# SenseBrain/JPD-SE

Hardware: AMD Instinct MI355X
Metric: training images/sec at 1024x512 (G+D+VGG step) (higher is better)
Workload: dtype bf16; 1 GPU; JPD-SE train step 1024x512, netG=global ngf=64 (39-ch input), num_D=2, VGG19+feat+L1, Adam x2, batch 4/GPU; global_batch=4, parallelism=dp1

## Files before the change

include/jpdse.h:

```cpp
#ifndef JPDSE_H_
#define JPDSE_H_

#include <stddef.h>
#include <stdint.h>

#ifdef __cplusplus
extern "C" {
#endif

#define JPDSE_ABI_VERSION 2

enum { JPDSE_F32 = 0, JPDSE_BF16 = 1 };
enum { JPDSE_PAD_ZERO = 0, JPDSE_PAD_REFLECT = 1 };
enum { JPDSE_ACT_NONE = 0, JPDSE_ACT_RELU = 1, JPDSE_ACT_LRELU = 2, JPDSE_ACT_TANH = 3 };
enum {
  JPDSE_OK = 0,
  JPDSE_EINVAL = -1,
  JPDSE_EWORKSPACE = -2,
  JPDSE_ELAUNCH = -3,
  JPDSE_EARCH = -4
};

#define JPDSE_CPAD(c) (((c) + 7) & ~7)

// ... 9 lines not shown
#define JPDSE_HBM_ADAM 2
int jpdse_prof_hbm_select(int32_t enable, int32_t max_regions);
int jpdse_prof_hbm_collect(int32_t cls, double* total_ms, double* total_bytes, int64_t* regions);

typedef struct jpdse_conv_desc {
  int32_t dtype;
  int32_t N, H, W, C;
  int32_t K;
  int32_t R, S;
  int32_t stride;
  int32_t pad;
  int32_t pad_mode;
  int32_t act;
  float slope;
} jpdse_conv_desc;

int jpdse_conv_out_shape(const jpdse_conv_desc* d, int32_t* OH, int32_t* OW);
int jpdse_conv_plan_query(const jpdse_conv_desc* d, int32_t* out, int32_t n);
size_t jpdse_conv_fwd_pack_size(const jpdse_conv_desc* d);
size_t jpdse_conv_dgrad_pack_size(const jpdse_conv_desc* d);
int jpdse_conv_pack_weights(const jpdse_conv_desc* d, const float* w_krsc, void* fwd_pack,
                            void* dgrad_pack, void* stream);
typedef struct jpdse_pack_entry {
  const float* w;
  void* out;
  int32_t K, Ks, C, Cs, R, S, st, qh, qw, Uh, Uw, Lk, gx, gy;
  int32_t out_f32;
  int32_t reserved_;
  int64_t blocks;
  int64_t block0;
} jpdse_pack_entry;
int jpdse_conv_pack_entries(const jpdse_conv_desc* d, const float* w_krsc, void* dgrad_pack,
                            jpdse_pack_entry* out, int32_t max_entries);
int jpdse_conv_pack_run(const jpdse_pack_entry* table_dev, int32_t n_entries, int64_t total_blocks,
                        void* stream);
size_t jpdse_conv_workspace_size(const jpdse_conv_desc* d);
int jpdse_conv_fwd(const jpdse_conv_desc* d, const void* x, const void* fwd_pack,
                   const float* bias, void* y, void* ws, size_t ws_bytes, void* stream);
int32_t jpdse_conv_moment_slots(const jpdse_conv_desc* d);
int jpdse_conv_fwd_moments(const jpdse_conv_desc* d, const void* x, const void* fwd_pack, void* y, float* moments,
                           void* ws, size_t ws_bytes, void* stream);
int jpdse_conv_fwd_pool(const jpdse_conv_desc* d, const void* x, const void* fwd_pack, const float* bias,
                        void* y, void* y_pool, void* ws, size_t ws_bytes, void* stream);
int jpdse_conv_dgrad(const jpdse_conv_desc* d, const void* dy, const void* dgrad_pack, void* dx,
                     void* ws, size_t ws_bytes, void* stream);
int jpdse_conv_dgrad_relu(const jpdse_conv_desc* d, const void* dy, const void* dgrad_pack,
                          const void* x, void* dx, void* ws, size_t ws_bytes, void* stream);
int jpdse_conv_dgrad_fused(const jpdse_conv_desc* d, const void* dy, const void* dgrad_pack,
                           const void* x, const void* addend, void* dx, void* ws, size_t ws_bytes,
                           void* stream);
int jpdse_conv_dgrad_fused_lrelu(const jpdse_conv_desc* d, const void* dy, const void* dgrad_pack,
                                 const void* x, float slope, const void* addend, void* dx, void* ws,
                                 size_t ws_bytes, void* stream);
int32_t jpdse_conv_dgrad_nsum_slots(const jpdse_conv_desc* d);
int jpdse_conv_dgrad_fused_nsums(const jpdse_conv_desc* d, const void* dy, const void* dgrad_pack, const void* x,
                                 const void* addend, void* dx, const void* norm_x, const float* norm_stats,
                                 int32_t norm_act, float norm_slope, float* sums, void* ws, size_t ws_bytes, void* stream);
int jpdse_conv_wgrad(const jpdse_conv_desc* d, const void* x, const void* dy, float* dw_krsc,
                     void* ws, size_t ws_bytes, void* stream);

int jpdse_convT_fwd(const jpdse_conv_desc* d, const void* x, const void* dgrad_pack, void* y,
                    void* ws, size_t ws_bytes, void* stream);
int32_t jpdse_convT_moment_slots(const jpdse_conv_desc* d);
int jpdse_convT_fwd_moments(const jpdse_conv_desc* d, const void* x, const void* dgrad_pack, void* y, float* moments,
                            void* ws, size_t ws_bytes, void* stream);
int jpdse_convT_dgrad(const jpdse_conv_desc* d, const void* dy, const void* fwd_pack, void* dx,
                      void* ws, size_t ws_bytes, void* stream);
int jpdse_convT_wgrad(const jpdse_conv_desc* d, const void* x, const void* dy, float* dw,
                      void* ws, size_t ws_bytes, void* stream);

typedef struct jpdse_inorm_desc {
  int32_t dtype;
  int32_t N, H, W, C;
  int32_t act;
  float slope;
  float eps;
  int32_t has_residual;
} jpdse_inorm_desc;
size_t jpdse_inorm_workspace_size(const jpdse_inorm_desc* d);
int jpdse_inorm_fwd(const jpdse_inorm_desc* d, const void* x, const void* residual, void* y,
                    float* stats, void* ws, size_t ws_bytes, void* stream);
int jpdse_inorm_fwd_from_moments(const jpdse_inorm_desc* d, const void* x, const float* moments, int32_t slots,
                                 const void* residual, void* y, float* stats, void* stream);
int jpdse_inorm_bwd_from_sums(const jpdse_inorm_desc* d, const void* x, const float* stats, const void* dy,
                              const float* sums, int32_t slots, void* dx, void* ws, size_t ws_bytes, void* stream);
int jpdse_inorm_bwd(const jpdse_inorm_desc* d, const void* x, const float* stats, const void* dy,
                    void* dx, void* ws, size_t ws_bytes, void* stream);

int jpdse_avgpool3s2_fwd(int32_t dtype, int32_t N, int32_t H, int32_t W, int32_t C, const void* x,
                         void* y, void* stream);
int jpdse_avgpool3s2_bwd(int32_t dtype, int32_t N, int32_t H, int32_t W, int32_t C, const void* dy,
                         void* dx, void* stream);
int jpdse_maxpool2_fwd(int32_t dtype, int32_t N, int32_t H, int32_t W, int32_t C, const void* x,
                       void* y, void* stream);
int jpdse_maxpool2_bwd(int32_t dtype, int32_t N, int32_t H, int32_t W, int32_t C, const void* x,
                       const void* dy, void* dx, void* stream);

int jpdse_act_bwd(int32_t dtype, int64_t n, int32_t act, float slope, const void* y, const void* dy,
                  void* dz, void* stream);
int jpdse_add(int32_t dtype, int64_t n, const void* a, const void* b, void* out, void* stream);
size_t jpdse_channel_sum_workspace_size(int64_t npix, int32_t C);
int jpdse_channel_sum(int32_t dtype, int64_t npix, int32_t C, const void* dy, float* out, void* ws,
                      size_t ws_bytes, void* stream);
int jpdse_channel_copy(int32_t dtype, int64_t npix, const void* src, int32_t src_cs, int32_t src_c0,
                       void* dst, int32_t dst_cs, int32_t dst_c0, int32_t nch, void* stream);
int jpdse_concat_channels(int32_t dtype, int64_t npix, const void* base, int32_t cs, const void* img,
                          int32_t img_cs, int32_t c0, int32_t nch, void* out, void* stream);
int jpdse_copy(int64_t nbytes, const void* src, void* dst, void* stream);
int jpdse_zero(int32_t dtype, int64_t n, void* p, void* stream);
int jpdse_cast(int32_t src_dtype, int32_t dst_dtype, int64_t n, const void* src, void* dst, void* stream);

int jpdse_nchw_to_nhwc(int32_t dtype, int32_t N, int32_t C, int32_t H, int32_t W, const float* src,
                       void* dst, void* stream);
int jpdse_nhwc_to_nchw(int32_t dtype, int32_t N, int32_t C, int32_t H, int32_t W, const void* src,
                       float* dst, void* stream);
int jpdse_onehot_edge(int32_t dtype, int32_t N, int32_t H, int32_t W, int32_t num_labels,
                      const float* label, const int64_t* instance, void* dst, int32_t cs,
                      void* stream);

int jpdse_input_builder(int32_t dtype, int32_t N, int32_t H, int32_t W, int32_t num_labels, const float* label,
                        const int64_t* instance, int32_t n_dst, void* const* dst, const void* const* img, int32_t cs,
                        int32_t img_cs, int32_t c0, int32_t nch, void* stream);
int jpdse_input_builder_wide(int32_t dtype, int32_t N, int32_t H, int32_t W, int32_t num_labels, const float* label,
                             const int64_t* instance, int32_t n_dst, void* const* dst, const void* const* img, int32_t cs,
                             int32_t img_cs, int32_t c0, int32_t nch, void*  stream);
int jpdse_insert_channels(int32_t dtype, int64_t npix, void* dst, int32_t cs, const void* img, int32_t img_cs, int32_t c0,
                          int32_t nch, void* stream);

size_t jpdse_loss_workspace_size(int64_t n);
typedef struct jpdse_loss_term {
// ... 426 lines not shown
```

jpd-se_amd/csrc/conv_dispatch_dgrad.h:

```cpp
#pragma once

namespace jpdse {

struct RingFoldArgs {
  bf16_t* dx;
  const float* top; const float* bot; const float* left; const float* right;
  int splits_tb, splits_lr;
  int N, H, W, Cs;
};
__device__ __forceinline__ void ring_acc(float (&acc)[8], const float* slab, int splits, long long slab_elems,
                                         long long row, int Cs, int c0) {
  const float* base = slab + row * Cs + c0;
  int sp = 0;
  for (; sp + 4 <= splits; sp += 4) {
    float4 lo[4], hi[4];
#pragma unroll
    for (int u = 0; u < 4; ++u) {
      const float4* src = reinterpret_cast<const float4*>(base + (sp + u) * slab_elems);
      lo[u] = src[0];
      hi[u] = src[1];
    }
#pragma unroll
    for (int u = 0; u < 4; ++u) {
      acc[0] += lo[u].x; acc[1] += lo[u].y; acc[2] += lo[u].z; acc[3] += lo[u].w;
// ... 80 lines not shown
    cols[1] = left ? 2 : W - 1;
    nc = 2;
  }
  float acc[8];
#pragma unroll
  for (int i = 0; i < 8; ++i) acc[i] = 0.f;
  for (int r = 0; r < nr; ++r)
    for (int c = 0; c < nc; ++c) {
      float v[8];
      Vec16<bf16_t>::load(dy + (((long long)n * H + rows[r]) * W + cols[c]) * Cs + c0, v);
#pragma unroll
      for (int i = 0; i < 8; ++i) acc[i] += v[i];
    }
  Vec16<bf16_t>::store(V + ((long long)n * per_n + e) * Cs + c0, acc);
}

template <typename T>
__global__ void relu_mask_kernel(T* __restrict__ dx, const T* __restrict__ mask, long long total_vec,
                                 const T* __restrict__ addend = nullptr, float slope = 0.f) {
  constexpr int VE = Vec16<T>::N;
  for (long long i = blockIdx.x * (long long)blockDim.x + threadIdx.x; i < total_vec;
       i += (long long)gridDim.x * blockDim.x) {
    float v[VE], m[VE];
    Vec16<T>::load(dx + i * VE, v);
    if (addend != nullptr) {
      Vec16<T>::load(addend + i * VE, m);
#pragma unroll
      for (int e = 0; e < VE; ++e) v[e] += m[e];
    }
    if (mask != nullptr) {
      Vec16<T>::load(mask + i * VE, m);
#pragma unroll
      for (int e = 0; e < VE; ++e) {
        const float r = sizeof(T) == 2 ? bf16_round(v[e]) : v[e];
        v[e] = m[e] > 0.f ? v[e] : (slope == 0.f ? 0.f : r * slope);
      }
    }
    Vec16<T>::store(dx + i * VE, v);
  }
}

struct NormSink {
  const void* x;
  const float* stats;
  float* sums;
  int act;
  float slope;
};

struct DgradCall {
  const jpdse_conv_desc* d; const ConvPlan& p;
  const void* dy; const void* pack; void* dx; void* ws; hipStream_t s;
  const void* mask; const void* addend; float* mom; float mask_slope; const NormSink* sink;
};
static void* dgrad_dxp(const DgradCall& c) { return reinterpret_cast<char*>(c.ws) + c.p.dypad_bytes; }

static ConvView dgrad_view(const DgradCall& c) {
  ConvView v = view_dgrad_phase(c.d, c.p, 0, c.dy, c.pack, c.dx);
  v.mask = reinterpret_cast<const bf16_t*>(c.mask);
  v.addend = reinterpret_cast<const bf16_t*>(c.addend);
  return v;
}
static ConvView ring_view(const DgradCall& c) {
  ConvView r = dgrad_view(c);
  r.OH = c.d->H;
  r.OW = c.d->W;
  r.py = r.px = 1;
  r.out_base = 0;
  r.mask = nullptr;
  return r;
}

static int dgrad_ring_frame(const DgradCall& c, DgradRoute route) {
  const jpdse_conv_desc* d = c.d;
  const ConvPlan& p = c.p;
  const bool taps = route == DgradRoute::ring_taps9_frame;
  ConvView r = ring_view(c);
  bf16_t* frame = reinterpret_cast<bf16_t*>(c.ws);
  const long long fv = (long long)d->N * (2 * (d->W + 2) + 2 * d->H) * (p.Ks / 8);
  if (taps && (size_t)fv * 16 > p.splitk_off) return set_error(JPDSE_EWORKSPACE, "reflect data gradient: no room for the frame in front of the slabs");
  const int pslot = taps ? -1 : prof_begin(c.s, p.Cs, 9LL * p.Ks);
  hipLaunchKernelGGL(ring_frame_kernel, dim3(ew_blocks(fv)), dim3(256), 0, c.s, r.X, frame, d->N, d->H, d->W, p.Ks, fv);
  const int rc = check_launch("ring_frame_kernel");
  prof_end(pslot, 1, 0.0, c.s);
  if (rc) return rc;
  r.frame = frame;
  r.mask = reinterpret_cast<const bf16_t*>(c.mask);
  if (taps) return launch_taps9(r, splitk_slabs(p, c.ws), c.s);
  HaloArgs h = to_halo(r);
  if (c.sink != nullptr) {
    h.nx = reinterpret_cast<const bf16_t*>(c.sink->x);
    h.nstats = c.sink->stats;
    h.nsums = c.sink->sums;
    h.nact = c.sink->act;
    h.nslope = c.sink->slope;
    h.mom_slots = halo_slots(d->H, d->W);
  }
  return p.Cs > 64 ? launch_halo_cfg<2>(h, c.s) : launch_halo_cfg<1>(h, c.s);
}

static int dgrad_ring_strips(const DgradCall& c, DgradRoute route) {
  const jpdse_conv_desc* d = c.d;
  const ConvPlan& p = c.p;
  hipStream_t s = c.s;
  const ConvView r = ring_view(c);
  if (route == DgradRoute::ring_taps9_strips) {
    if (int rc = launch_taps9(r, splitk_slabs(p, c.ws), s)) return rc;
  } else if (int rc = p.Cs > 64 ? launch_halo_cfg<2>(to_halo(r), s) : launch_halo_cfg<1>(to_halo(r), s)) return rc;
  const int H = d->H, W = d->W, Ks = p.Ks, Lk = p.ph[0].Lk;
  const bf16_t* dyb = reinterpret_cast<const bf16_t*>(c.dy);
  const bf16_t* pk = reinterpret_cast<const bf16_t*>(c.pack);
  const int Mtb = d->N * (W + 2), Mlr = d->N * H;
  const int nt = (p.Cs + 127) / 128;
// ... 73 lines not shown
  h.Wp = reinterpret_cast<const bf16_t*>(c.pack);
  h.Y = reinterpret_cast<bf16_t*>(c.dx);
  h.N = d->N; h.H = p.OH; h.W = p.OW; h.OH = d->H; h.OW = d->W;
  h.K = d->C; h.Ks_out = p.Cs;
  h.R = h.S = 3;
  h.pad = 1;
  h.act = JPDSE_ACT_NONE;
  h.tiles_w = (d->W + 63) / 64;
  h.tiles_h = (d->H + kHeadTH - 1) / kHeadTH;
  if (head_rows_ok(64, h.R, h.K, h.Ks_out, h.H, h.W, h.OH, h.OW)) return launch_head_rows<3>(h, c.s);
  return launch_head_fwd<64, 3, 3, 3>(h, c.s);
}

template <typename Args>
static Args phases_rows_args(const DgradCall& c) {
  Args g = {};
  g.DY = reinterpret_cast<const bf16_t*>(c.dy);
  for (int i = 0; i < 4; ++i) g.P[i] = reinterpret_cast<const bf16_t*>(reinterpret_cast<const char*>(c.pack) + c.p.ph[i].pack_off);
  g.DX = reinterpret_cast<bf16_t*>(c.dx);
  g.N = c.d->N; g.OH = c.p.OH; g.OW = c.p.OW;
  return g;
}
static int dgrad_dgrad2_rows(const DgradCall& c) {
  Dgrad2Args g = phases_rows_args<Dgrad2Args>(c);
  g.mom = c.mom;
  return launch_dgrad2_rows(g, c.s);
}
static int dgrad_thin_dgrad2_rows(const DgradCall& c) {
  ThinDgrad2Args g = phases_rows_args<ThinDgrad2Args>(c);
  g.H = c.d->H; g.W = c.d->W; g.K = c.d->C;
  return launch_thin_dgrad2_rows(g, c.s);
}

static int dgrad_thin_in_rows(const DgradCall& c) {
  ThinInArgs g = {};
  g.DY = reinterpret_cast<const bf16_t*>(c.dy);
  g.P = reinterpret_cast<const bf16_t*>(reinterpret_cast<const char*>(c.pack) + c.p.ph[0].pack_off);
  g.DX = reinterpret_cast<bf16_t*>(c.dx);
  g.DXP = reinterpret_cast<bf16_t*>(dgrad_dxp(c));
  g.N = c.d->N; g.H = c.d->H; g.W = c.d->W; g.OH = c.d->H + 6; g.OW = c.d->W + 6;
  g.py = g.px = 6;
  g.act = JPDSE_ACT_NONE;
  return launch_thin_in_rows<7, true>(g, c.s);
}

static int dgrad_thin1(const DgradCall& c) {
  const Phase& f = c.p.ph[0];
  Thin1DgradArgs t = {};
  t.DY = reinterpret_cast<const bf16_t*>(c.dy);
  t.B = reinterpret_cast<const bf16_t*>(reinterpret_cast<const char*>(c.pack) + f.pack_off);
  t.taps = reinterpret_cast<float*>(c.ws);
  t.DX = reinterpret_cast<bf16_t*>(c.dx);
  t.addend = reinterpret_cast<const bf16_t*>(c.addend);
  t.N = c.d->N; t.H = c.d->H; t.W = c.d->W; t.Cs = c.p.Cs; t.OH = c.p.OH; t.OW = c.p.OW;
  t.py = (f.Uh - 1) - f.i0h;
  t.px = (f.Uw - 1) - f.i0w;
  t.Lk = f.Lk;
  t.b_stride = (long long)f.Uh * f.Lk;
  return launch_thin1_dgrad(t, c.s);
}

template <typename Args>
static void phase_out(Args* a, const DgradCall& c, const Phase& f) {
  const jpdse_conv_desc* d = c.d;
  const ConvPlan& p = c.p;
  const bool refl = d->pad_mode == JPDSE_PAD_REFLECT;
  const int st = d->stride, H = refl ? p.Hp : d->H, W = refl ? p.Wp : d->W, off = refl ? 0 : d->pad;
  a->Y = reinterpret_cast<decltype(a->Y)>(refl ? dgrad_dxp(c) : c.dx);
  a->out_sn = (long long)H * W * p.Cs;
  a->out_sh = (long long)st * W * p.Cs;
  a->out_sw = (long long)st * p.Cs;
  a->out_base = ((long long)(st * f.i0h + f.qh - off) * W + (st * f.i0w + f.qw - off)) * p.Cs;
}
template <typename T>
static int dgrad_finish(const DgradCall& c, bool in_epilogue) {
  const jpdse_conv_desc* d = c.d;
  const long long total_vec = (long long)d->N * d->H * d->W * (c.p.Cs / (16 / (int)sizeof(T)));
  int rc = JPDSE_OK;
  if (d->pad_mode == JPDSE_PAD_REFLECT) {
    hipLaunchKernelGGL((reflect_fold_kernel<T>), dim3(ew_blocks(total_vec)), dim3(256), 0, c.s, reinterpret_cast<const T*>(dgrad_dxp(c)),
                       reinterpret_cast<T*>(c.dx), d->N, d->H, d->W, c.p.Cs, d->pad, total_vec);
    rc = check_launch("reflect_fold_kernel");
  }
  if (rc == JPDSE_OK && (c.mask != nullptr || c.addend != nullptr) && !in_epilogue) {
    hipLaunchKernelGGL((relu_mask_kernel<T>), dim3(ew_blocks(total_vec)), dim3(256), 0, c.s, reinterpret_cast<T*>(c.dx),
                       reinterpret_cast<const T*>(c.mask), total_vec, reinterpret_cast<const T*>(c.addend), c.mask_slope);
    rc = check_launch("relu_mask_kernel");
  }
  return rc;
}

static int dgrad_fast(const DgradCall& c) {
  const jpdse_conv_desc* d = c.d;
  const ConvPlan& p = c.p;
  const bool refl = d->pad_mode == JPDSE_PAD_REFLECT;
  const int nlive = live_phases(p);
  FastBatch batch = {};
  for (int i = 0; i < p.nph; ++i) {
    const Phase& f = p.ph[i];
    if (f.cnth <= 0 || f.cntw <= 0) continue;
    FastArgs g = to_fast(view_dgrad_phase(d, p, i, c.dy, c.pack, c.dx));
    phase_out(&g, c, f);
    if (!refl) {
      g.mask = reinterpret_cast<const bf16_t*>(c.mask);
      g.addend = reinterpret_cast<const bf16_t*>(c.addend);
    }
    g.mask_slope = c.mask_slope;
    g.splits = nlive == 1 ? splitk_for(g.M, p.Cs, f.Uh * f.Uw * p.Ks / 64) : 1;
    g.partial = splitk_slabs(p, c.ws);
    batch.p[batch.n++] = g;
  }
  if (int rc = launch_fast_batch(batch, c.s)) return rc;
  return dgrad_finish<bf16_t>(c, !refl);
}

template <typename T>
static int dgrad_generic(const DgradCall& c) {
  const jpdse_conv_desc* d = c.d;
  const ConvPlan& p = c.p;
  if (int rc = launch_pad<T>(c.dy, c.ws, d->N, p.OH, p.OW, p.Ks, p.PT, p.PB, p.PL, p.PR, JPDSE_PAD_ZERO, c.s)) return rc;
  for (int i = 0; i < p.nph; ++i) {
    const Phase& f = p.ph[i];
    if (f.cnth <= 0 || f.cntw <= 0) continue;
    GemmFwdArgs a = {};
    a.A = c.ws;
    a.B = reinterpret_cast<const char*>(c.pack) + f.pack_off;
    a.M = d->N * f.cnth * f.cntw; a.OH = f.cnth; a.OW = f.cntw;
    a.Kout = d->C; a.Ks = a.b_rows = p.Cs;
    a.R = f.Uh; a.cpr = f.Lk / p.BKE; a.b_row_stride = (long long)f.Uh * f.Lk;
    a.in_sn = (long long)p.DH * p.DW * p.Ks; a.in_sh = a.in_sr = (long long)p.DW * p.Ks; a.in_sw = p.Ks;
    a.in_base = ((long long)(f.i0h + p.PT - (f.Uh - 1)) * p.DW + (f.i0w + p.PL - (f.Uw - 1))) * p.Ks;
    phase_out(&a, c, f);
    a.act = JPDSE_ACT_NONE;
    a.partial = splitk_slabs(p, c.ws);
    a.partial_cap = p.splitk_bytes;
    if (int rc = launch_fwd<T>(a, c.s)) return rc;
  }
  return dgrad_finish<T>(c, false);
}

static int convT_fwd_moment_slots(const jpdse_conv_desc* d, const ConvPlan& p) {
  if (!g_moments_fused || select_dgrad(d, p, {false, false, false, true, false}) != DgradRoute::dgrad2_rows) return 0;
  return dgrad2_rows_slots(dgrad2_rows_band(d->N, p.OH, p.OW), p.OH, p.OW);
}
static int dgrad_nsum_slots(const jpdse_conv_desc* d, const ConvPlan& p) {
  if (select_dgrad(d, p, {false, false, false, false, true}) != DgradRoute::ring_halo_frame) return 0;
  return p.Ks >= 128 && p.Cs % 128 == 0 && d->C == p.Cs ? halo_slots(d->H, d->W) : 0;
}

template <typename T>
static int conv_dgrad_t(const jpdse_conv_desc* d, const ConvPlan& p, const void* dy, const void* pack, void* dx,
                        void* ws, hipStream_t s, const void* mask = nullptr, const void* addend = nullptr, float* mom = nullptr,
                        float mask_slope = 0.f, const NormSink* sink = nullptr) {
  const bool lrelu = mask != nullptr && mask_slope != 0.f;
  if (sink != nullptr && (dgrad_nsum_slots(d, p) == 0 || lrelu))
    return set_error(JPDSE_EINVAL, "conv_dgrad: this layer's data-gradient kernel writes no norm-backward sums (jpdse_conv_dgrad_nsum_slots == 0)");
  const DgradCall c = {d, p, dy, pack, dx, ws, s, mask, addend, mom, mask_slope, sink};
  const DgradRoute route = select_dgrad(d, p, {mask != nullptr, addend != nullptr, lrelu, mom != nullptr, sink != nullptr});
  if constexpr (sizeof(T) == 2) {
    switch (route) {
      case DgradRoute::rows: return launch_rows(to_rows(dgrad_view(c)), 1, s);
      case DgradRoute::halo: return p.Cs > 64 ? launch_halo_cfg<2>(to_halo(dgrad_view(c)), s) : launch_halo_cfg<1>(to_halo(dgrad_view(c)), s);
      case DgradRoute::taps9: return launch_taps9(dgrad_view(c), splitk_slabs(p, ws), s);
      case DgradRoute::ring_taps9_frame:
      case DgradRoute::ring_halo_frame: return dgrad_ring_frame(c, route);
      case DgradRoute::ring_taps9_strips:
      case DgradRoute::ring_halo_strips: return dgrad_ring_strips(c, route);
      case DgradRoute::head: return dgrad_head(c);
      case DgradRoute::dgrad2_rows: return dgrad_dgrad2_rows(c);
      case DgradRoute::thin_dgrad2_rows: return dgrad_thin_dgrad2_rows(c);
      case DgradRoute::thin_in_rows: return dgrad_thin_in_rows(c);
      case DgradRoute::taps_dgrad2: return launch_taps_dgrad2(d, p, dy, pack, dx, s, mask, addend, mask_slope);
      case DgradRoute::taps4: return launch_taps4(dgrad_view(c), ws, s);
      case DgradRoute::thin1: return dgrad_thin1(c);
      case DgradRoute::fast: return dgrad_fast(c);
      default: break;
    }
  }
  return dgrad_generic<T>(c);
}

}
```

jpd-se_amd/csrc/conv_gemm.hip:

```cpp
#include "common.h"

#include <vector>


namespace jpdse {

struct GemmFwdArgs {
  const void* A;
  const void* B;
  const float* bias;
  void* Y;
  int M, OH, OW;
  int Kout, Ks;
  int R, cpr;
  int b_rows;
  long long b_row_stride;
  long long in_sn, in_sh, in_sw, in_sr, in_base;
  long long out_sn, out_sh, out_sw, out_base;
  int act;
  float slope;
  int col_mod, k_real;
  int splits;
  float* partial;
  size_t partial_cap;
// ... 443 lines not shown
                           size_t ws_bytes, void* stream) {
  ConvPlan p;
  if (int rc = conv_enter("conv_fwd_moments", d, x && fwd_pack && y && moments, ws, ws_bytes, &p, [d](const ConvPlan& q) {
        JPDSE_REQUIRE(conv_fwd_moment_slots(d, q) > 0, "conv_fwd_moments: this layer has no moment epilogue (jpdse_conv_moment_slots == 0)");
        return (int)JPDSE_OK;
      })) return rc;
  return conv_fwd_t<bf16_t>(d, p, x, fwd_pack, nullptr, y, ws, as_stream(stream), moments);
}

int jpdse_convT_fwd_moments(const jpdse_conv_desc* d, const void* x, const void* dgrad_pack, void* y, float* moments, void* ws,
                            size_t ws_bytes, void* stream) {
  ConvPlan p;
  if (int rc = conv_enter("convT_fwd_moments", d, x && dgrad_pack && y && moments, ws, ws_bytes, &p, [d](const ConvPlan& q) {
        JPDSE_REQUIRE(convT_fwd_moment_slots(d, q) > 0, "convT_fwd_moments: this layer has no moment epilogue (jpdse_convT_moment_slots == 0)");
        return (int)JPDSE_OK;
      })) return rc;
  return conv_dgrad_t<bf16_t>(d, p, x, dgrad_pack, y, ws, as_stream(stream), nullptr, nullptr, moments);
}

int jpdse_conv_dgrad(const jpdse_conv_desc* d, const void* dy, const void* dgrad_pack, void* dx, void* ws,
                     size_t ws_bytes, void* stream) {
  ConvPlan p;
  if (int rc = conv_enter("conv_dgrad", d, dy && dgrad_pack && dx, ws, ws_bytes, &p)) return rc;
  return d->dtype == JPDSE_BF16 ? conv_dgrad_t<bf16_t>(d, p, dy, dgrad_pack, dx, ws, as_stream(stream))
                                : conv_dgrad_t<float>(d, p, dy, dgrad_pack, dx, ws, as_stream(stream));
}

int jpdse_conv_dgrad_relu(const jpdse_conv_desc* d, const void* dy, const void* dgrad_pack, const void* x, void* dx,
                          void* ws, size_t ws_bytes, void* stream) {
  JPDSE_REQUIRE(x != nullptr, "conv_dgrad_relu: null mask tensor");
  return jpdse_conv_dgrad_fused(d, dy, dgrad_pack, x, nullptr, dx, ws, ws_bytes, stream);
}

int jpdse_conv_dgrad_fused(const jpdse_conv_desc* d, const void* dy, const void* dgrad_pack, const void* x,
                           const void* addend, void* dx, void* ws, size_t ws_bytes, void* stream) {
  ConvPlan p;
  if (int rc = conv_enter("conv_dgrad_fused", d, dy && dgrad_pack && dx, ws, ws_bytes, &p)) return rc;
  return d->dtype == JPDSE_BF16 ? conv_dgrad_t<bf16_t>(d, p, dy, dgrad_pack, dx, ws, as_stream(stream), x, addend)
                                : conv_dgrad_t<float>(d, p, dy, dgrad_pack, dx, ws, as_stream(stream), x, addend);
}

int jpdse_conv_dgrad_fused_lrelu(const jpdse_conv_desc* d, const void* dy, const void* dgrad_pack, const void* x,
                                 float slope, const void* addend, void* dx, void* ws, size_t ws_bytes, void* stream) {
  ConvPlan p;
  if (int rc = conv_enter("conv_dgrad_fused_lrelu", d, dy && dgrad_pack && dx && x, ws, ws_bytes, &p, [slope](const ConvPlan&) {
        JPDSE_REQUIRE(slope >= 0.f && slope < 1.f, "conv_dgrad_fused_lrelu: slope %g outside [0, 1)", (double)slope);
        return (int)JPDSE_OK;
      })) return rc;
  return d->dtype == JPDSE_BF16
             ? conv_dgrad_t<bf16_t>(d, p, dy, dgrad_pack, dx, ws, as_stream(stream), x, addend, nullptr, slope)
             : conv_dgrad_t<float>(d, p, dy, dgrad_pack, dx, ws, as_stream(stream), x, addend, nullptr, slope);
}

int32_t jpdse_conv_dgrad_nsum_slots(const jpdse_conv_desc* d) {
  if (validate(d)) return 0;
  ConvPlan p;
  make_plan(d, &p);
  return dgrad_nsum_slots(d, p);
}

int jpdse_conv_dgrad_fused_nsums(const jpdse_conv_desc* d, const void* dy, const void* dgrad_pack, const void* x,
                                 const void* addend, void* dx, const void* norm_x, const float* norm_stats, int32_t norm_act,
                                 float norm_slope, float* sums, void* ws, size_t ws_bytes, void* stream) {
  ConvPlan p;
  if (int rc = conv_enter("conv_dgrad_fused_nsums", d, dy && dgrad_pack && dx && norm_x && norm_stats && sums, ws, ws_bytes, &p,
                          [d, norm_act](const ConvPlan& q) {
        JPDSE_REQUIRE(norm_act == JPDSE_ACT_NONE || norm_act == JPDSE_ACT_RELU || norm_act == JPDSE_ACT_LRELU,
                      "conv_dgrad_fused_nsums: activation %d", norm_act);
        JPDSE_REQUIRE(d->dtype == JPDSE_BF16 && dgrad_nsum_slots(d, q) > 0,
                      "conv_dgrad_fused_nsums: this layer has no norm-backward-sum epilogue (jpdse_conv_dgrad_nsum_slots == 0)");
        return (int)JPDSE_OK;
      })) return rc;
  const NormSink sink = {norm_x, norm_stats, sums, norm_act, norm_slope};
  return conv_dgrad_t<bf16_t>(d, p, dy, dgrad_pack, dx, ws, as_stream(stream), x, addend, nullptr, 0.f, &sink);
}

int jpdse_conv_wgrad(const jpdse_conv_desc* d, const void* x, const void* dy, float* dw, void* ws, size_t ws_bytes,
                     void* stream) {
  ConvPlan p;
  if (int rc = conv_enter("conv_wgrad", d, x && dy && dw, ws, ws_bytes, &p)) return rc;
  return d->dtype == JPDSE_BF16 ? conv_wgrad_t<bf16_t>(d, p, x, dy, dw, ws, as_stream(stream))
                                : conv_wgrad_t<float>(d, p, x, dy, dw, ws, as_stream(stream));
}

int jpdse_convT_fwd(const jpdse_conv_desc* d, const void* x, const void* dgrad_pack, void* y, void* ws,
                    size_t ws_bytes, void* stream) {
  return jpdse_conv_dgrad(d, x, dgrad_pack, y, ws, ws_bytes, stream);
}
int jpdse_convT_dgrad(const jpdse_conv_desc* d, const void* dy, const void* fwd_pack, void* dx, void* ws,
                      size_t ws_bytes, void* stream) {
  return jpdse_conv_fwd(d, dy, fwd_pack, nullptr, dx, ws, ws_bytes, stream);
}
int jpdse_convT_wgrad(const jpdse_conv_desc* d, const void* x, const void* dy, float* dw, void* ws,
                      size_t ws_bytes, void* stream) {
  return jpdse_conv_wgrad(d, dy, x, dw, ws, ws_bytes, stream);
}

}
```

jpd-se_amd/csrc/conv_launch.h:

```cpp
#pragma once

namespace jpdse {

struct GemmProf {
  bool on = false;
  int Ks = 0;
  long long kdim = 0;
  int used = 0;
  std::vector<hipEvent_t> ev;
  std::vector<double> flops;
  std::vector<int> cls;
};
static GemmProf g_prof;
static int check_tile_grid(const char* who, int N, int OH, int OW, int th, int tw, int Cs_in, long long in_elems, long long out_elems) {
  if (N <= 0 || OH <= 0 || OW <= 0 || OH % th != 0 || OW % tw != 0)
    return set_error(JPDSE_EINVAL, "%s: output grid %d x %d x %d does not tile into %d x %d patches", who, N, OH, OW, th, tw);
  if (Cs_in <= 0 || Cs_in % 64 != 0) return set_error(JPDSE_EINVAL, "%s: %d input channels (a multiple of 64 is required)", who, Cs_in);
  if (in_elems >= (1LL << 31) || out_elems >= (1LL << 40))
    return set_error(JPDSE_EINVAL, "%s: tensor too large for the kernel's offsets (%lld input elements)", who, in_elems);
  return JPDSE_OK;
}

template <auto Kernel>
static int opt_in_lds(const char* who, int bytes) {
  static bool configured = false;
  if (configured) return JPDSE_OK;
  const hipError_t e = hipFuncSetAttribute(reinterpret_cast<const void*>(Kernel), hipFuncAttributeMaxDynamicSharedMemorySize, bytes);
  if (e != hipSuccess) return set_error(JPDSE_ELAUNCH, "%s: hipFuncSetAttribute(%d B LDS): %s", who, bytes, hipGetErrorString(e));
  configured = true;
  return JPDSE_OK;
}

static int prof_begin(hipStream_t s, int Ks, long long kdim) {
  if (!g_prof.on || Ks != g_prof.Ks || kdim != g_prof.kdim || (size_t)(2 * g_prof.used + 2) > g_prof.ev.size()) return -1;
  (void)hipEventRecord(g_prof.ev[2 * g_prof.used], s);
  return g_prof.used;
}
static void prof_end(int slot, int cls, double flops, hipStream_t s) {
  if (slot < 0) return;
  (void)hipEventRecord(g_prof.ev[2 * slot + 1], s);
  g_prof.flops[slot] = flops;
  g_prof.cls[slot] = cls;
  g_prof.used = slot + 1;
}

struct ConvView : ConvShape {
  const bf16_t* X; const bf16_t* B; const float* bias; bf16_t* Y;
  int py, px, Kout;
  long long ktot;
  int tap_s;
  long long out_sn, out_sh, out_sw, out_base;
  float slope;
  const bf16_t* mask; float mask_slope; const bf16_t* addend;
  float* mom;
  const bf16_t* frame;
};

static ConvView view_fwd(const jpdse_conv_desc* d, const ConvPlan& p, const void* x, const void* pack, const float* bias, void* y) {
  ConvView v = {};
  static_cast<ConvShape&>(v) = shape_fwd(d, p);
  v.X = reinterpret_cast<const bf16_t*>(x);
  v.B = reinterpret_cast<const bf16_t*>(pack);
  v.bias = bias;
  v.Y = reinterpret_cast<bf16_t*>(y);
  v.py = v.px = d->pad;
  v.Kout = d->K;
  v.ktot = (long long)d->R * p.Lk_fwd; v.tap_s = p.Cs;
  v.out_sn = (long long)p.OH * p.OW * p.Ks; v.out_sh = (long long)p.OW * p.Ks; v.out_sw = p.Ks;
  v.slope = d->slope;
  return v;
}

static ConvView view_dgrad_phase(const jpdse_conv_desc* d, const ConvPlan& p, int i, const void* dy, const void* pack, void* dx) {
  const Phase& f = p.ph[i];
  const int st = d->stride;
  ConvView v = {};
  static_cast<ConvShape&>(v) = shape_dgrad_phase(d, p, i);
  v.X = reinterpret_cast<const bf16_t*>(dy);
  v.B = reinterpret_cast<const bf16_t*>(reinterpret_cast<const char*>(pack) + f.pack_off);
  v.Y = reinterpret_cast<bf16_t*>(dx);
  v.py = (f.Uh - 1) - f.i0h; v.px = (f.Uw - 1) - f.i0w;
  v.Kout = d->C;
  v.ktot = (long long)f.Uh * f.Lk; v.tap_s = p.Ks;
  v.out_sn = (long long)d->H * d->W * p.Cs; v.out_sh = (long long)st * d->W * p.Cs; v.out_sw = (long long)st * p.Cs;
  v.out_base = ((long long)(st * f.i0h + f.qh - d->pad) * d->W + (st * f.i0w + f.qw - d->pad)) * p.Cs;
  return v;
}

template <typename Args>
static Args view_to(const ConvView& v) {
  Args a = {};
  a.X = v.X; a.B = v.B; a.bias = v.bias; a.Y = v.Y;
  a.OH = v.OH; a.OW = v.OW; a.IH = v.IH; a.IW = v.IW; a.py = v.py; a.px = v.px;
  a.Kout = v.Kout; a.Ks = v.Ks_out; a.b_rows = v.Ks_out;
  a.out_sn = v.out_sn; a.out_sh = v.out_sh; a.out_sw = v.out_sw; a.out_base = v.out_base;
  a.act = v.act; a.slope = v.slope;
  a.mask = v.mask; a.addend = v.addend;
  return a;
}
static RowsArgs to_rows(const ConvView& v) {
  RowsArgs r = view_to<RowsArgs>(v);
  r.N = v.N;
  r.mom = v.mom;
  return r;
}
static int halo_slots(int OH, int OW) { return (OH / 4) * (OW / 64); }
static HaloArgs to_halo(const ConvView& v) {
  HaloArgs h = view_to<HaloArgs>(v);
  h.N = v.N; h.Cs = v.Cin_s; h.reflect = v.reflect;
  h.V = v.frame;
  h.mom = v.mom;
  h.mom_slots = v.mom != nullptr ? halo_slots(v.OH, v.OW) : 0;
  return h;
}
static FastArgs to_fast(const ConvView& v) {
  FastArgs f = view_to<FastArgs>(v);
  f.M = v.N * v.OH * v.OW; f.Cs = v.Cin_s;
  f.R = v.R; f.S = v.S; f.sy = f.sx = v.stride; f.reflect = v.reflect;
  f.mask_slope = v.mask_slope;
  return f;
}

template <typename T, int BM, int BN, int WM, int WN>
static int launch_fwd_cfg(const GemmFwdArgs& a_in, hipStream_t s) {
  GemmFwdArgs a = a_in;
  const int tiles_m = (a.M + BM - 1) / BM, tiles_n = (a.Ks + BN - 1) / BN;
  const size_t lds = 2 * (BM + BN) * 64;
  a.splits = (a.col_mod == 0 && a.partial != nullptr) ? generic_splitk_for((int)sizeof(T), a.M, a.Ks, a.R * a.cpr, a.M / (a.OH * a.OW)) : 1;
  if (a.splits > 1 && (size_t)a.splits * a.M * a.Ks * sizeof(float) > a.partial_cap) a.splits = 1;
  const long long kdim = (long long)a.R * a.cpr * (64 / (int)sizeof(T));
  const int pslot = prof_begin(s, a.Ks, kdim);
  hipLaunchKernelGGL((gemm_fwd_kernel<T, BM, BN, WM, WN>), dim3(tiles_m * tiles_n, a.splits > 1 ? a.splits : 1), dim3(64 * WM * WN), lds, s, a);
  int rc = check_launch("gemm_fwd_kernel");
  if (rc == JPDSE_OK && a.splits > 1) {
    const long long total_vec = (long long)a.M * (a.Ks / 4);
    hipLaunchKernelGGL((gemm_splitk_finish_kernel<T>), dim3((unsigned)((total_vec + 255) / 256)), dim3(256), 0, s, a, total_vec);
    rc = check_launch("gemm_splitk_finish_kernel");
  }
  prof_end(pslot, 0, 2.0 * (double)a.M * (double)a.Ks * (double)kdim, s);
  return rc;
}

template <typename T>
static int launch_fwd(const GemmFwdArgs& a, hipStream_t s) {
  if (a.M <= 0) return JPDSE_OK;
  if (a.Ks > 64) return launch_fwd_cfg<T, 128, 128, 2, 2>(a, s);
  if (a.Ks > 32) return launch_fwd_cfg<T, 128, 64, 2, 2>(a, s);
  return launch_fwd_cfg<T, 256, 32, 4, 1>(a, s);
}

template <typename T, int BM, int BN>
static int generic_wgrad_splits(const GemmWgradArgs& a, int* chunks_per_split) {
  const int PIX = WgStage<T>::PIX;
  const int col_tiles = (a.run + BN - 1) / BN, chunks_total = (a.M + PIX - 1) / PIX;
  const int tiles = ((a.K + BM - 1) / BM) * a.R * col_tiles;
  int splits = 1;
  if (tiles < 512) {
    splits = (768 + tiles - 1) / tiles;
    const int max_splits = (chunks_total + 7) / 8;
    if (splits > max_splits) splits = max_splits;
    if (splits > 64) splits = 64;
    if (splits < 1) splits = 1;
  }
  const int cps = (chunks_total + splits - 1) / splits;
  if (chunks_per_split) *chunks_per_split = cps;
  return (chunks_total + cps - 1) / cps;
}

template <typename T, int BM, int BN, int WM, int WN>
static int launch_wgrad_cfg(GemmWgradArgs a, float* slabs, hipStream_t s) {
  const int PIX = WgStage<T>::PIX;
  a.col_tiles_per_r = (a.run + BN - 1) / BN;
  a.chunks_total = (a.M + PIX - 1) / PIX;
  const int tiles = ((a.K + BM - 1) / BM) * a.R * a.col_tiles_per_r;
  const int splits = generic_wgrad_splits<T, BM, BN>(a, &a.chunks_per_split);
  const long long n = (long long)a.K * a.R * a.S * a.C;
  a.partial = splits > 1 ? slabs : nullptr;
  a.slab_stride = (n + 3) / 4 * 4;
  const size_t lds = 2 * (BM + BN) * 64;
  hipLaunchKernelGGL((gemm_wgrad_kernel<T, BM, BN, WM, WN>), dim3(tiles, splits), dim3(64 * WM * WN), lds, s, a);
  if (int rc = check_launch("gemm_wgrad_kernel")) return rc;
  return splits > 1 ? launch_slab_reduce(slabs, a.DW, n, a.slab_stride, splits, s) : JPDSE_OK;
}

template <typename T>
static size_t generic_wgrad_slab_bytes(const GemmWgradArgs& a) {
  const int splits = a.K > 64 ? generic_wgrad_splits<T, 128, 128>(a, nullptr)
                              : (a.K > 32 ? generic_wgrad_splits<T, 64, 128>(a, nullptr) : generic_wgrad_splits<T, 32, 256>(a, nullptr));
  const long long n = (long long)a.K * a.R * a.S * a.C;
  return splits > 1 ? (size_t)splits * ((n + 3) / 4 * 4) * sizeof(float) : 0;
}

template <typename T>
static int launch_wgrad(const GemmWgradArgs& a, float* slabs, hipStream_t s) {
  if (a.K > 64) return launch_wgrad_cfg<T, 128, 128, 2, 2>(a, slabs, s);
  if (a.K > 32) return launch_wgrad_cfg<T, 64, 128, 2, 2>(a, slabs, s);
  return launch_wgrad_cfg<T, 32, 256, 1, 4>(a, slabs, s);
}

template <int WM, int WN, int TM, int TN, int STAGES = 3>
static int launch_fast_cfg(FastBatch& b, hipStream_t s) {
  constexpr int BM = WM * TM * 32, BN = WN * TN * 32;
  constexpr int lds = STAGES * (BM + BN) * 128;
  if (int rc = opt_in_lds<&gemm_fast_kernel<WM, WN, TM, TN, STAGES>>("gemm_fast", lds)) return rc;
  int total = 0;
  for (int i = 0; i < b.n; ++i) {
    const FastArgs& a = b.p[i];
    if ((a.Y == nullptr && !a.no_finish) || ((a.splits > 1 || a.no_finish) && a.partial == nullptr))
      return set_error(JPDSE_EINVAL, "gemm_fast: problem %d has no output buffer", i);
    if ((a.x_sh ? a.x_sh : (long long)a.IW * a.Cs) * a.IH >= (1LL << 31))
      return set_error(JPDSE_EINVAL, "gemm_fast: one image spans >= 2^31 elements (in-image offsets are 32-bit)");
    if (a.x_extent > 0 && a.OH > 0 && a.OW > 0) {
      const long long n_img = a.M / ((long long)a.OH * a.OW);
      const long long sn = a.x_sn ? a.x_sn : (long long)a.IH * a.IW * a.Cs, sh = a.x_sh ? a.x_sh : (long long)a.IW * a.Cs;
      const long long last = (n_img - 1) * sn + (long long)(a.IH - 1) * sh + (long long)(a.IW - 1) * a.Cs + a.Cs;
      if (n_img < 1 || last > a.x_extent)
        return set_error(JPDSE_EINVAL, "gemm_fast: problem %d addresses element %lld of a %lld-element input", i, last, a.x_extent);
    }
    b.first_tile[i] = total;
    b.p[i].xcd_map = 0;
    total += ((a.M + BM - 1) / BM) * ((a.Ks + BN - 1) / BN) * (a.splits > 1 ? a.splits : 1);
  }
  for (int i = b.n; i < 5; ++i) b.first_tile[i] = total;
  const long long kdim = (long long)b.p[0].R * b.p[0].S * b.p[0].Cs;
  const int pslot = b.n == 1 ? prof_begin(s, b.p[0].Ks, kdim) : -1;
  hipLaunchKernelGGL((gemm_fast_kernel<WM, WN, TM, TN, STAGES>), dim3(total), dim3(64 * WM * WN), lds, s, b);
  if (b.n == 1 && b.p[0].splits > 1 && !b.p[0].no_finish) {
    const long long total_vec = (long long)b.p[0].M * (b.p[0].Ks / 8);
    hipLaunchKernelGGL(splitk_finish_kernel, dim3(ew_blocks(total_vec)), dim3(256), 0, s, b.p[0], total_vec);
  }
  prof_end(pslot, 0, 2.0 * (double)b.p[0].M * (double)b.p[0].Ks * (double)kdim, s);
  return check_launch("gemm_fast_kernel");
}

JPDSE_SWITCH(int, g_fast_small, 20);
JPDSE_SWITCH(int, g_fast_fill, 1);
static int launch_fast_batch(FastBatch& b, hipStream_t s) {
  if (b.n <= 0) return JPDSE_OK;
  const int Ks = b.p[0].Ks;
  if (b.n == 1 && b.p[0].splits > 1) {
    if (Ks > 64) return launch_fast_cfg<4, 2, 2, 2>(b, s);
    if (Ks > 32) return launch_fast_cfg<4, 2, 2, 1>(b, s);
    return launch_fast_cfg<8, 1, 1, 1>(b, s);
  }
  for (int i = 0; i < b.n; ++i)
    if (b.n > 1 && !b.p[i].no_finish) b.p[i].splits = 1;
  if (b.small_m) {
    if (Ks > 64) return launch_fast_cfg<2, 2, 2, 2, 2>(b, s);
    if (Ks > 32) return launch_fast_cfg<2, 2, 2, 1, 2>(b, s);
  }
  int kt = 0;
  for (int i = 0; i < b.n; ++i) {
    const int k = b.p[i].R * b.p[i].S * (b.p[i].Cs / 64);
    kt = k > kt ? k : kt;
  }
  if (g_fast_small && kt <= g_fast_small && b.p[0].splits <= 1) {
    if (Ks > 64 && kt <= 16) return launch_fast_cfg<2, 2, 1, 2, 2>(b, s);
    if (Ks > 64) return launch_fast_cfg<2, 2, 2, 2, 2>(b, s);
    if (Ks > 32) return launch_fast_cfg<2, 2, 2, 1, 2>(b, s);
  }
  if (g_fast_fill && Ks > 64 && kt <= 64 && b.p[0].splits <= 1) {
    long long t256 = 0;
    for (int i = 0; i < b.n; ++i) t256 += (long long)((b.p[i].M + 255) / 256) * ((Ks + 127) / 128);
    if (t256 < 224) {
      if (t256 < 160) return launch_fast_cfg<2, 2, 1, 2, 2>(b, s);
      return launch_fast_cfg<2, 2, 2, 2, 2>(b, s);
    }
  }
  if (b.n == 1 && prefer_320(b.p[0].M, Ks)) return launch_fast_cfg<2, 4, 5, 1, 2>(b, s);
  if (Ks > 64) return launch_fast_cfg<4, 2, 2, 2>(b, s);
  if (Ks > 32) return launch_fast_cfg<4, 2, 2, 1>(b, s);
  return launch_fast_cfg<8, 1, 1, 1>(b, s);
}

static int launch_fast(const FastArgs& a, hipStream_t s) {
  if (a.M <= 0) return JPDSE_OK;
// ... 239 lines not shown
          ++t;
        }
    }
  }
  const int bn = p.Cs % 128 == 0 ? 128 : 64;
  a.nblk0 = d->N * (a.OH / 4) * (a.OW / 64) * ((p.Cs + bn - 1) / bn);
  return bn == 128 ? launch_taps_dgrad2_cfg<2>(a, 2 * a.nblk0, s) : launch_taps_dgrad2_cfg<1>(a, 2 * a.nblk0, s);
}

static int taps4_fringe_splits(int N, int OH, int OW, int Ks_out, int k_tiles) {
  const int OHc = OH / 8 * 8, OWc = OW / 32 * 32;
  const long long m_bot = (long long)N * (OH - OHc) * OW, m_right = (long long)N * OHc * (OW - OWc);
  const long long nt = (Ks_out + 127) / 128;
  const long long tiles = ((m_bot + 255) / 256 + (m_right + 255) / 256) * nt;
  if (tiles <= 0) return 0;
  long long sp = 256 / tiles;
  if (sp > k_tiles / 8) sp = k_tiles / 8;
  if (sp > 8) sp = 8;
  return sp < 1 ? 1 : (int)sp;
}

static size_t taps4_fringe_bytes(int N, int OH, int OW, int Ks_out, int k_tiles) {
  const int OHc = OH / 8 * 8, OWc = OW / 32 * 32;
  const long long m = (long long)N * (OH - OHc) * OW + (long long)N * OHc * (OW - OWc);
  return (size_t)taps4_fringe_splits(N, OH, OW, Ks_out, k_tiles) * m * Ks_out * sizeof(float);
}

template <int TN>
static int launch_taps4_cfg(const TapsArgs& a, int total, hipStream_t s) {
  constexpr int PH = 11, PW = 35;
  constexpr int lds = 2 * ((PH * PW + 7) / 8) * 1024 + 3 * (2 * TN * 32) * 128;
  if (int rc = opt_in_lds<&gemm_taps_kernel<TN, 16, 0, 0, 0, 2, PH, PW>>("gemm_taps(4x4)", lds)) return rc;
  if (int rc = check_tile_grid("gemm_taps(4x4)", a.N, a.OH, a.OW, 8, 32, a.Cs, (long long)a.N * a.IH * a.IW * a.Cs,
                               (long long)a.N * a.OH * a.OW * a.Ks)) return rc;
  if (total != a.N * (a.OH / 8) * (a.OW / 32) * ((a.Ks + 2 * TN * 32 - 1) / (2 * TN * 32)))
    return set_error(JPDSE_EINVAL, "gemm_taps(4x4): %d blocks do not match the tile grid", total);
  hipLaunchKernelGGL((gemm_taps_kernel<TN, 16, 0, 0, 0, 2, PH, PW>), dim3(total), dim3(512), lds, s, a);
  return check_launch("gemm_taps_kernel(4x4)");
}

static TapsArgs to_taps(const ConvView& v, int patch_w) {
  TapsArgs a = {};
  a.X = v.X;
  a.Y = v.Y;
  a.bias = v.bias;
  a.N = v.N; a.OH = v.OH; a.OW = v.OW; a.IH = v.IH; a.IW = v.IW; a.Cs = v.Cin_s;
  a.py = v.py; a.px = v.px;
  a.Kout = v.Kout; a.Ks = v.Ks_out; a.b_rows = v.Ks_out;
  a.out_sn = v.out_sn; a.out_sh = v.out_sh; a.out_sw = v.out_sw;
  a.act = v.act;
  a.slope = v.slope;
  a.addend = v.addend;
  a.mask = v.mask;
  a.prog[0].B[0] = v.B;
  a.prog[0].ktot[0] = v.ktot;
  a.prog[0].out_base[0] = v.out_base;
  for (int r = 0; r < v.R; ++r)
    for (int c = 0; c < v.S; ++c) {
      a.prog[0].tap_off[r * v.S + c] = r * patch_w + c;
      a.prog[0].tap_koff[r * v.S + c] = r * v.tap_r + c * v.tap_s;
    }
  return a;
}

static int launch_taps4(const ConvView& v, void* ws, hipStream_t s) {
  const int OHc = v.OH / 8 * 8, OWc = v.OW / 32 * 32;
  TapsArgs a = to_taps(v, 35);
  a.OH = OHc;
  a.OW = OWc;
  const int bn = v.Ks_out % 128 == 0 ? 128 : 64;
  a.nblk0 = v.N * (OHc / 8) * (OWc / 32) * ((v.Ks_out + bn - 1) / bn);
  if (int rc = bn == 128 ? launch_taps4_cfg<2>(a, a.nblk0, s) : launch_taps4_cfg<1>(a, a.nblk0, s)) return rc;
  const int k_tiles = 16 * v.Cin_s / 64;
  const int sp = taps4_fringe_splits(v.N, v.OH, v.OW, v.Ks_out, k_tiles);
  if (sp == 0) return JPDSE_OK;
  FastBatch fb = {};
  float* slab = reinterpret_cast<float*>(ws);
  const int rect[2][4] = {{OHc, 0, v.OH - OHc, v.OW}, {0, OWc, OHc, v.OW - OWc}};
  for (int q = 0; q < 2; ++q) {
    const int oh0 = rect[q][0], ow0 = rect[q][1], rows = rect[q][2], cols = rect[q][3];
    if (rows <= 0 || cols <= 0) continue;
    FastArgs g = to_fast(v);
    g.M = v.N * rows * cols;
    g.OH = rows;
    g.OW = cols;
    g.py = v.py - oh0;
    g.px = v.px - ow0;
    g.out_base = v.out_base + oh0 * v.out_sh + ow0 * v.out_sw;
    g.splits = sp;
    g.no_finish = 1;
    g.partial = slab;
    g.b_stride = v.ktot;
    g.b_tap_r = v.tap_r;
    g.b_tap_s = v.tap_s;
    slab += (size_t)sp * g.M * v.Ks_out;
    fb.p[fb.n++] = g;
  }
  if (int rc = launch_fast_batch(fb, s)) return rc;
  for (int q = 0; q < fb.n; ++q) {
    const long long total_vec = (long long)fb.p[q].M * (fb.p[q].Ks / 8);
    hipLaunchKernelGGL(splitk_finish_kernel, dim3(ew_blocks(total_vec)), dim3(256), 0, s, fb.p[q], total_vec);
  }
  return check_launch("taps4 fringe finish");
}

static int taps9_splits(int N, int OH, int OW, int Cin_s, int Ks_out) {
// ... 105 lines not shown
```

jpd-se_amd/csrc/gemm_fast.h:

```cpp
#pragma once
#include "common.h"
#include "lds_ops.h"

namespace jpdse {

__device__ __attribute__((aligned(256))) uint32_t g_zero_page[64];

struct FastArgs {
  const bf16_t* X;
  const bf16_t* B;
  const float* bias;
  bf16_t* Y;
  int M, OH, OW;
  int IH, IW, Cs;
  int R, S;
  int sy, sx;
  int py, px;
  int reflect;
  int Kout, Ks, b_rows;
  long long out_sn, out_sh, out_sw, out_base;
  int act;
  float slope;
  int splits;
  float* partial;
  const bf16_t* mask;
  const bf16_t* addend;
  float mask_slope;
  long long x_sn, x_sh;
  long long b_stride;
  int b_tap_r, b_tap_s;
  int no_finish;
  long long x_extent;
  int xcd_map;
};

struct FastBatch {
  FastArgs p[4];
  int first_tile[5];
  int n;
  int small_m;
};

__device__ __forceinline__ int swz128(int row, int slot) { return (row << 7) + (((slot ^ (row >> 1)) & 7) << 4); }

__device__ __forceinline__ float pair_swap(float v) {
  return __builtin_bit_cast(float, __builtin_amdgcn_update_dpp(0, __builtin_bit_cast(int, v), 0xB1, 0xF, 0xF, false));
}

template <int TM, int TN, int ACT>
__device__ __forceinline__ void acc_tile_to_lds_ct(char* tile, int pitch, int wrow0, int wcol0, int n0, int lane,
                                                   const f32x16 (&acc)[TM][TN], const float* bias, int Kout, float slope) {
  const int odd = lane & 1;
#pragma unroll
  for (int j = 0; j < TN; ++j) {
    const int lcol = wcol0 + j * 32 + (lane & 31);
    const int col = n0 + lcol;
    const bool live = col < Kout;
    const float bv = (bias != nullptr && live) ? bias[col] : 0.f;
#pragma unroll
    for (int i = 0; i < TM; ++i) {
#pragma unroll
      for (int ep = 0; ep < 8; ++ep) {
        const int e = 2 * ep;
        const float v0 = live ? act_ct<ACT>(acc[i][j][e] + bv, slope) : 0.f;
        const float v1 = live ? act_ct<ACT>(acc[i][j][e + 1] + bv, slope) : 0.f;
        const float recv = pair_swap(odd ? v0 : v1);
        const float lo = odd ? recv : v0, hi = odd ? v1 : recv;
        const uint32_t word = (uint32_t)f2bf(lo) | ((uint32_t)f2bf(hi) << 16);
        const int row = wrow0 + i * 32 + (e & 3) + 8 * (e >> 2) + 4 * (lane >> 5) + odd;
        *reinterpret_cast<uint32_t*>(tile + row * pitch + (lcol - odd) * 2) = word;
      }
    }
  }
}
template <int TM, int TN>
__device__ __forceinline__ void acc_tile_to_lds(char* tile, int pitch, int wrow0, int wcol0, int n0, int lane,
                                                const f32x16 (&acc)[TM][TN], const float* bias, int Kout, int act,
                                                float slope) {
  if (act == JPDSE_ACT_RELU) acc_tile_to_lds_ct<TM, TN, JPDSE_ACT_RELU>(tile, pitch, wrow0, wcol0, n0, lane, acc, bias, Kout, slope);
  else if (act == JPDSE_ACT_LRELU) acc_tile_to_lds_ct<TM, TN, JPDSE_ACT_LRELU>(tile, pitch, wrow0, wcol0, n0, lane, acc, bias, Kout, slope);
  else if (act == JPDSE_ACT_TANH) acc_tile_to_lds_ct<TM, TN, JPDSE_ACT_TANH>(tile, pitch, wrow0, wcol0, n0, lane, acc, bias, Kout, slope);
  else acc_tile_to_lds_ct<TM, TN, JPDSE_ACT_NONE>(tile, pitch, wrow0, wcol0, n0, lane, acc, bias, Kout, slope);
}

__device__ __forceinline__ u32x4 add_bf16x8(u32x4 v, u32x4 w) {
#pragma unroll
  for (int i = 0; i < 4; ++i) {
    const float lo = __uint_as_float(v[i] << 16) + __uint_as_float(w[i] << 16);
    const float hi = __uint_as_float(v[i] & 0xffff0000u) + __uint_as_float(w[i] & 0xffff0000u);
    v[i] = (uint32_t)f2bf(lo) | ((uint32_t)f2bf(hi) << 16);
  }
  return v;
}

__device__ __forceinline__ u32x4 max_bf16x8(u32x4 a, u32x4 b) {
#pragma unroll
  for (int i = 0; i < 4; ++i) {
    const float alo = __uint_as_float(a[i] << 16), blo = __uint_as_float(b[i] << 16);
    const float ahi = __uint_as_float(a[i] & 0xffff0000u), bhi = __uint_as_float(b[i] & 0xffff0000u);
    a[i] = (__float_as_uint(fmaxf(alo, blo)) >> 16) | (__float_as_uint(fmaxf(ahi, bhi)) & 0xffff0000u);
  }
  return a;
}

__device__ __forceinline__ u32x4 relu_mask8(u32x4 v, u32x4 m) {
#pragma unroll
  for (int i = 0; i < 4; ++i) {
    const uint32_t lo = m[i] & 0xffffu, hi = m[i] >> 16;
    const uint32_t klo = (lo - 1u) < 0x7f80u ? 0xffffu : 0u;
    const uint32_t khi = (hi - 1u) < 0x7f80u ? 0xffff0000u : 0u;
    v[i] &= (klo | khi);
  }
  return v;
}

__device__ __forceinline__ u32x4 lrelu_mask8(u32x4 v, u32x4 m, float slope) {
  if (slope == 0.f) return relu_mask8(v, m);
#pragma unroll
  for (int i = 0; i < 4; ++i) {
    const uint32_t lo = m[i] & 0xffffu, hi = m[i] >> 16;
    const uint32_t slo = f2bf(__uint_as_float(v[i] << 16) * slope);
    const uint32_t shi = f2bf(__uint_as_float(v[i] & 0xffff0000u) * slope);
    const uint32_t rlo = (lo - 1u) < 0x7f80u ? (v[i] & 0xffffu) : slo;
    const uint32_t rhi = (hi - 1u) < 0x7f80u ? (v[i] >> 16) : shi;
    v[i] = rlo | (rhi << 16);
  }
  return v;
}

template <int WM, int WN, int TM, int TN, int STAGES>
__global__ __launch_bounds__(64 * WM * WN) void gemm_fast_kernel(const FastBatch batch) {
  int q = 0;
#pragma unroll
  for (int i = 1; i < 4; ++i)
    if (i < batch.n && (int)blockIdx.x >= batch.first_tile[i]) q = i;
  const FastArgs& a = batch.p[q];
  const int block_id = (int)blockIdx.x - batch.first_tile[q];
  constexpr int NW = WM * WN;
  constexpr int BM = WM * TM * 32, BN = WN * TN * 32;
  constexpr int A_TILE = BM * 128, B_TILE = BN * 128;
  constexpr int STAGE_BYTES = A_TILE + B_TILE;
  constexpr int A_UNITS = BM / 8, B_UNITS = BN / 8;
  constexpr int AU = (A_UNITS + NW - 1) / NW, BU = (B_UNITS + NW - 1) / NW;
  static_assert(A_UNITS % NW == 0, "every wave stages the same number of A units");
  extern __shared__ __attribute__((aligned(16))) char smem[];

  const int tid = threadIdx.x, lane = tid & 63;
  const int wid = __builtin_amdgcn_readfirstlane(tid >> 6);
  const int wm = wid / WN, wn = wid % WN;
  const int tiles_m = (a.M + BM - 1) / BM;
  const int ntiles = tiles_m * ((a.Ks + BN - 1) / BN);
  const int split = a.splits > 1 ? block_id / ntiles : 0;
  const int tile_id = a.splits > 1 ? block_id - split * ntiles : block_id;
  int tile_m = tile_id % tiles_m, tile_n = tile_id / tiles_m;
  if (a.xcd_map) {
    const int tiles_n = ntiles / tiles_m;
    const int m8 = tiles_m & ~7, head = m8 * tiles_n;
    if (tile_id < head) {
      const int x = tile_id & 7, j = tile_id >> 3;
      tile_n = j % tiles_n;
      tile_m = (j / tiles_n) * 8 + x;
    } else {
      const int rem = tiles_m - m8, t = tile_id - head;
      tile_m = m8 + t % rem;
      tile_n = t / rem;
    }
  }
  const int m0 = tile_m * BM, n0 = tile_n * BN;
  const int lrow = lane >> 3, lslot = lane & 7;

  const bf16_t* a_xb[AU];
  int a_oh[AU], a_ow[AU], a_lds[AU];
#pragma unroll
  for (int i = 0; i < AU; ++i) {
    const int u = wid + i * NW;
    const int row = u * 8 + lrow;
    int m = m0 + row;
    m = m < a.M ? m : a.M - 1;
    const int ow = m % a.OW, t = m / a.OW, oh = t % a.OH, n = t / a.OH;
    a_xb[i] = a.X + (long long)n * (a.x_sn ? a.x_sn : (long long)a.IH * a.IW * a.Cs) + ((lslot ^ (row >> 1)) & 7) * 8;
    a_oh[i] = oh * a.sy - a.py;
    a_ow[i] = ow * a.sx - a.px;
    a_lds[i] = u * 1024;
  }
  const bf16_t* b_ptr[BU];
  int b_lds[BU];
  bool b_on[BU];
// ... 193 lines not shown
      }
    }
    return;
  }
  for (int idx = tid; idx < BM * VPR; idx += 64 * NW) {
    const int row = idx / VPR, v = idx - row * VPR;
    const long long off = row_off[row];
    if (off < 0 || n0 + v * 8 >= a.Ks) continue;
    *reinterpret_cast<u32x4*>(a.Y + off + n0 + v * 8) = *reinterpret_cast<const u32x4*>(tile + row * PITCH + v * 16);
  }
}

__global__ __launch_bounds__(256) void splitk_finish_kernel(const FastArgs a, long long total_vec) {
  const long long v = (long long)blockIdx.x * 256 + threadIdx.x;
  if (v >= total_vec) return;
  const int vpr = a.Ks >> 3;
  const int m = (int)(v / vpr), c0 = (int)(v % vpr) * 8;
  float acc[8];
#pragma unroll
  for (int e = 0; e < 8; ++e) acc[e] = 0.f;
  const float* const base = a.partial + (long long)m * a.Ks + c0;
  const long long slab_elems = (long long)a.M * a.Ks;
  int sidx = 0;
  for (; sidx + 4 <= a.splits; sidx += 4) {
    float4 lo[4], hi[4];
#pragma unroll
    for (int u = 0; u < 4; ++u) {
      const float4* src = reinterpret_cast<const float4*>(base + (sidx + u) * slab_elems);
      lo[u] = src[0];
      hi[u] = src[1];
    }
#pragma unroll
    for (int u = 0; u < 4; ++u) {
      acc[0] += lo[u].x; acc[1] += lo[u].y; acc[2] += lo[u].z; acc[3] += lo[u].w;
      acc[4] += hi[u].x; acc[5] += hi[u].y; acc[6] += hi[u].z; acc[7] += hi[u].w;
    }
  }
  for (; sidx < a.splits; ++sidx) {
    const float4* src = reinterpret_cast<const float4*>(base + sidx * slab_elems);
    const float4 lo = src[0], hi = src[1];
    acc[0] += lo.x; acc[1] += lo.y; acc[2] += lo.z; acc[3] += lo.w;
    acc[4] += hi.x; acc[5] += hi.y; acc[6] += hi.z; acc[7] += hi.w;
  }
  const int ow = m % a.OW, t = m / a.OW, oh = t % a.OH, n = t / a.OH;
  const long long off = a.out_base + n * a.out_sn + oh * a.out_sh + ow * a.out_sw;
  float o[8];
#pragma unroll
  for (int e = 0; e < 8; ++e) {
    const int col = c0 + e;
    const bool live = col < a.Kout;
    const float bv = (a.bias != nullptr && live) ? a.bias[col] : 0.f;
    o[e] = live ? apply_act(acc[e] + bv, a.act, a.slope) : 0.f;
  }
  if (a.addend != nullptr) {
    float ad[8];
    Vec16<bf16_t>::load(a.addend + off + c0, ad);
#pragma unroll
    for (int e = 0; e < 8; ++e) o[e] += ad[e];
  }
  if (a.mask != nullptr) {
    float mk[8];
    Vec16<bf16_t>::load(a.mask + off + c0, mk);
#pragma unroll
    for (int e = 0; e < 8; ++e) o[e] = mk[e] > 0.f ? o[e] : (a.mask_slope == 0.f ? 0.f : bf16_round(o[e]) * a.mask_slope);
  }
  Vec16<bf16_t>::store(a.Y + off + c0, o);
}

}
```

jpd-se_amd/csrc/gemm_taps.h:

```cpp
#pragma once
#include "common.h"
#include "gemm_fast.h"
#include "gemm_halo.h"

namespace jpdse {

constexpr int kTapsMax = 16;

struct TapsProg {
  const bf16_t* B[2];
  long long ktot[2];
  long long out_base[2];
  int tap_off[kTapsMax];
  int tap_koff[kTapsMax];
};

struct TapsArgs {
  const bf16_t* X;
  bf16_t* Y;
  const float* bias;
  int N, OH, OW;
  int IH, IW, Cs;
  int py, px;
  int Kout, Ks, b_rows;
  long long out_sn, out_sh, out_sw;
  int act;
  float slope;
  const bf16_t* addend;
  const bf16_t* mask;
  float mask_slope;
  int reflect;
  int splits;
  float* partial;
  const bf16_t* V;
  int nblk0;
  TapsProg prog[2];
};

template <int TN, int T0, int T1, int WROWS, int PH, int PW, bool VIRT = false>
__device__ __forceinline__ void gemm_taps_body(const TapsArgs& a, const TapsProg& pr, int bid, char* smem) {
  constexpr int NT = T0 + T1, NSETS = T1 > 0 ? 2 : 1;
  constexpr int NW = 8, WN = 2;
  constexpr int TH = 4 * WROWS, TW = 64 / WROWS;
  constexpr int BN = WN * TN * 32;
  constexpr int NP = PH * PW;
  constexpr int UH = (NP + 7) / 8;
  constexpr int HALO = UH * 1024;
  constexpr int B_STAGE = BN * 128;
  constexpr int B_UNITS = BN / 8, BU = B_UNITS / NW;
  static_assert(B_UNITS % NW == 0, "every wave issues exactly BU weight pieces per tile");
  constexpr int HU = (UH + NW - 1) / NW;
  constexpr int UPT = (HU + NT - 1) / NT;
  static_assert(NT <= kTapsMax && NT >= 2, "tap program length");
  constexpr int PZ = UH * 8 - 1;
  static_assert(!VIRT || (T0 == 9 && T1 == 0 && PZ - 1 >= NP && (PZ & 1) == 1 && (PW & 1) == 0 && PH == TH + 2 && PW == TW + 2), "VIRT: nine taps, one set, two slack pixels");
  char* const bring = smem;
  char* const halo0 = smem + 3 * B_STAGE;

  const int tid = threadIdx.x, lane = tid & 63;
  const int wid = __builtin_amdgcn_readfirstlane(tid >> 6);
  const int wm = wid / WN, wn = wid % WN;
  const int tiles_w = a.OW / TW, tiles_h = a.OH / TH;
  const int tiles_m = a.N * tiles_h * tiles_w;
  const int ntiles = tiles_m * ((a.Ks + BN - 1) / BN);
  const int split = a.splits > 1 ? bid / ntiles : 0;
  if (a.splits > 1) bid -= split * ntiles;
  const int tile_m = bid % tiles_m, tile_n = bid / tiles_m;
  const int tw_i = tile_m % tiles_w, t1 = tile_m / tiles_w;
  const int th_i = t1 % tiles_h, n = t1 / tiles_h;
  const int oh0 = th_i * TH, ow0 = tw_i * TW, n0 = tile_n * BN;
  const int lrow = lane >> 3, lslot = lane & 7;
  const bf16_t* const zero = reinterpret_cast<const bf16_t*>(g_zero_page);

  int h_off[HU];
  int h_lds[HU];
  int n_hu = 0;
#pragma unroll
  for (int i = 0; i < HU; ++i) {
    const int u = wid + i * NW;
    const bool on = u < UH;
    n_hu += on ? 1 : 0;
    const int ug = on ? u : 0;
    int p = ug * 8 + lrow;
    const int swz_p = p;
    const bool slack = p >= NP;
    p = p < NP ? p : NP - 1;
    const int hr = p / PW, wc = p - hr * PW;
    int ih = oh0 - a.py + hr, iw = ow0 - a.px + wc;
// ... 131 lines not shown
    }
    __builtin_amdgcn_s_setprio(1);
#pragma unroll
    for (int ks = 0; ks < 4; ++ks) {
      s16x8 af[2], bf[TN];
#pragma unroll
      for (int i = 0; i < 2; ++i)
        af[i] = *reinterpret_cast<const s16x8*>(hb + a_base[i] + (((2 * ks + hsel) << 4) ^ a_sw[i]));
#pragma unroll
      for (int j = 0; j < TN; ++j) bf[j] = *reinterpret_cast<const s16x8*>(st + b_rd[j][ks]);
#pragma unroll
      for (int i = 0; i < 2; ++i)
#pragma unroll
        for (int j = 0; j < TN; ++j)
          acc[q][i][j] = __builtin_amdgcn_mfma_f32_32x32x16_bf16(af[i], bf[j], acc[q][i][j], 0, 0, 0);
    }
    __builtin_amdgcn_s_setprio(0);
  };

  for (int slab0 = s_begin; slab0 < CC; slab0 += 3) {
#pragma unroll
    for (int sm = 0; sm < 3; ++sm) {
      const int slab = slab0 + sm;
      if (slab >= CC) break;
      const bool more = slab + 1 < CC;
      const char* const hb = halo0 + (slab & 1) * HALO;
#pragma unroll
      for (int tap = 0; tap < NT; ++tap) step(sm, tap, slab, more, hb);
    }
  }

  if (a.splits > 1) {
    float* const slab = a.partial + (long long)split * ((long long)a.N * a.OH * a.OW) * a.Ks;
#pragma unroll
    for (int j = 0; j < TN; ++j) {
      const int col = n0 + wn * TN * 32 + j * 32 + (lane & 31);
      if (col >= a.Ks) continue;
#pragma unroll
      for (int i = 0; i < 2; ++i) {
#pragma unroll
        for (int e = 0; e < 16; ++e) {
          const int rl = i * 32 + (e & 3) + 8 * (e >> 2) + 4 * (lane >> 5);
          const int r = WROWS == 1 ? wm : 2 * wm + (rl >> 5), c = WROWS == 1 ? rl : (rl & 31);
          const long long m = ((long long)n * a.OH + oh0 + r) * a.OW + ow0 + c;
          slab[m * a.Ks + col] = acc[0][i][j][e];
        }
      }
    }
    return;
  }
  constexpr int PITCH = BN * 2 + 64;
  static_assert(TH * TW * PITCH <= 2 * HALO + 3 * B_STAGE, "epilogue tile fits the pipeline LDS");
  constexpr int VPR = BN / 8;
#pragma unroll
  for (int q = 0; q < NSETS; ++q) {
    __syncthreads();
    acc_tile_to_lds<2, TN>(smem, PITCH, WROWS == 1 ? wm * 64 : wm * 64, wn * TN * 32, n0, lane, acc[q], a.bias, a.Kout, a.act, a.slope);
    __syncthreads();
    const long long blk_base = pr.out_base[q] + n * a.out_sn + (long long)oh0 * a.out_sh + (long long)ow0 * a.out_sw;
    if (a.addend != nullptr || a.mask != nullptr) {
      constexpr int NV = TH * TW * VPR / 512;
      static_assert(TH * TW * VPR % 512 == 0, "every thread owns the same number of output vectors");
      u32x4 addv[NV], mskv[NV];
#pragma unroll
      for (int it = 0; it < NV; ++it) {
        const int idx = tid + 512 * it;
        const int row = idx / VPR, v = idx - row * VPR;
        const int r = row / TW, c = row - r * TW;
        const long long off = blk_base + (long long)r * a.out_sh + (long long)c * a.out_sw + n0 + v * 8;
        const bool on = n0 + v * 8 < a.Ks;
        if (on && a.addend != nullptr) addv[it] = *reinterpret_cast<const u32x4*>(a.addend + off);
        if (on && a.mask != nullptr) mskv[it] = *reinterpret_cast<const u32x4*>(a.mask + off);
      }
#pragma unroll
      for (int it = 0; it < NV; ++it) {
        const int idx = tid + 512 * it;
        const int row = idx / VPR, v = idx - row * VPR;
        if (n0 + v * 8 >= a.Ks) continue;
        const int r = row / TW, c = row - r * TW;
        const long long off = blk_base + (long long)r * a.out_sh + (long long)c * a.out_sw + n0 + v * 8;
        u32x4 val = *reinterpret_cast<const u32x4*>(smem + row * PITCH + v * 16);
        if (a.addend != nullptr) val = add_bf16x8(val, addv[it]);
        if (a.mask != nullptr) val = lrelu_mask8(val, mskv[it], a.mask_slope);
        *reinterpret_cast<u32x4*>(a.Y + off) = val;
      }
      continue;
    }
    for (int idx = tid; idx < TH * TW * VPR; idx += 512) {
      const int row = idx / VPR, v = idx - row * VPR;
      if (n0 + v * 8 >= a.Ks) continue;
      const int r = row / TW, c = row - r * TW;
      const long long off = blk_base + (long long)r * a.out_sh + (long long)c * a.out_sw;
      *reinterpret_cast<u32x4*>(a.Y + off + n0 + v * 8) = *reinterpret_cast<const u32x4*>(smem + row * PITCH + v * 16);
    }
  }
}

template <int TN, int T0A, int T1A, int T0B, int T1B, int WROWS, int PH, int PW, bool VIRT = false>
__global__ __launch_bounds__(512) void gemm_taps_kernel(const TapsArgs a) {
  extern __shared__ __attribute__((aligned(16))) char smem[];
  if constexpr (T0B > 0) {
    const int b = (int)blockIdx.x;
    int prog, local;
    if ((a.nblk0 & 7) == 0) {
      prog = (b >> 3) & 1;
      local = ((b >> 4) << 3) | (b & 7);
    } else {
      prog = b >= a.nblk0 ? 1 : 0;
      local = prog ? b - a.nblk0 : b;
    }
    if (prog) {
      gemm_taps_body<TN, T0B, T1B, WROWS, PH, PW>(a, a.prog[1], local, smem);
      return;
    }
    gemm_taps_body<TN, T0A, T1A, WROWS, PH, PW>(a, a.prog[0], local, smem);
  } else {
    gemm_taps_body<TN, T0A, T1A, WROWS, PH, PW, VIRT>(a, a.prog[0], (int)blockIdx.x, smem);
  }
}

}
```

jpd-se_amd/csrc/norm.hip:

```cpp
#include "common.h"

namespace jpdse {

struct MomentGeom {
  int N, HW, Cs, cv;
  int TX, TY;
  int tx_shift;
  int splits, pix_per_split;
};

static MomentGeom moment_geom(int N, int HW, int Cs, int VE) {
  MomentGeom g;
  g.N = N; g.HW = HW; g.Cs = Cs; g.cv = Cs / VE;
  int tx = 1;
  while (tx < g.cv && tx < 256) tx <<= 1;
  g.TX = tx; g.TY = 256 / tx;
  g.tx_shift = 0;
  while ((1 << g.tx_shift) < tx) ++g.tx_shift;
  const int col_blocks = (g.cv + g.TX - 1) / g.TX;
  long long want = 2048 / ((long long)N * col_blocks);
  if (want < 1) want = 1;
  long long max_splits = HW / ((long long)g.TY * 8);
  if (max_splits < 1) max_splits = 1;
  if (want > max_splits) want = max_splits;
  if (want > 256) want = 256;
  g.splits = (int)want;
  g.pix_per_split = (HW + g.splits - 1) / g.splits;
  g.splits = (HW + g.pix_per_split - 1) / g.pix_per_split;
  return g;
}

#ifndef JPDSE_NORM_ILP
#define JPDSE_NORM_ILP 2
#endif

template <typename T> struct FwdMoments {
  const T* x;
  __device__ __forceinline__ void prep(int n, int HW, int Cs, int c0, float (&aux)[8]) const {
    float v[Vec16<T>::N];
    Vec16<T>::load(x + (long long)n * HW * Cs + c0, v);
#pragma unroll
    for (int e = 0; e < Vec16<T>::N; ++e) aux[e] = v[e];
  }
  __device__ __forceinline__ void acc(const float (&v)[Vec16<T>::N], const float (&aux)[8], float (&s1)[8], float (&s2)[8]) const {
#pragma unroll
    for (int e = 0; e < Vec16<T>::N; ++e) {
      const float d = v[e] - aux[e];
      s1[e] += d;
      s2[e] += d * d;
    }
  }
  __device__ __forceinline__ void at(long long off, const float (&aux)[8], float (&s1)[8], float (&s2)[8]) const {
    float v[Vec16<T>::N];
    Vec16<T>::load(x + off, v);
    acc(v, aux, s1, s2);
  }
};

__device__ __forceinline__ float act_grad(float yhat, int act, float slope) {
  if (act == JPDSE_ACT_RELU) return yhat > 0.f ? 1.f : 0.f;
  if (act == JPDSE_ACT_LRELU) return yhat > 0.f ? 1.f : slope;
  return 1.f;
}

template <typename T> struct BwdMoments {
  const T* x;
  const T* dy;
  const float* stats;
  int act;
  float slope;
  __device__ __forceinline__ void acc2(const float (&v)[Vec16<T>::N], const float (&g)[Vec16<T>::N], const float (&mean)[Vec16<T>::N],
                                       const float (&rstd)[Vec16<T>::N], float (&s1)[8], float (&s2)[8]) const {
#pragma unroll
    for (int e = 0; e < Vec16<T>::N; ++e) {
      const float yh = (v[e] - mean[e]) * rstd[e];
      const float dz = g[e] * act_grad(yh, act, slope);
      s1[e] += dz;
      s2[e] += dz * yh;
    }
  }
};

template <typename T, bool BWD>
__global__ __launch_bounds__(256) void moment_kernel(const T* __restrict__ x, const T* __restrict__ dy,
                                                    const float* __restrict__ stats, int act, float slope,
                                                    float* __restrict__ partial, MomentGeom g) {
  constexpr int VE = Vec16<T>::N;
  __shared__ float red[256 * 2 * VE];
  const int tx = threadIdx.x & (g.TX - 1), ty = threadIdx.x >> g.tx_shift;
  const int col_blocks = (g.cv + g.TX - 1) / g.TX;
  const int cb = blockIdx.x % col_blocks;
  const int split = (blockIdx.x / col_blocks) % g.splits;
  const int n = blockIdx.x / (col_blocks * g.splits);
  const int col = cb * g.TX + tx;
  const bool on = col < g.cv;
  const int c0 = col * VE;
  float s1[8], s2[8], aux[8];
#pragma unroll
  for (int e = 0; e < 8; ++e) { s1[e] = 0.f; s2[e] = 0.f; aux[e] = 0.f; }
  if (on) {
    const int p0 = split * g.pix_per_split;
    int p1 = p0 + g.pix_per_split;
    p1 = p1 < g.HW ? p1 : g.HW;
    const long long base = (long long)n * g.HW * g.Cs + c0;
    if (!BWD) {
      FwdMoments<T> f{x};
      f.prep(n, g.HW, g.Cs, c0, aux);
      int p = p0 + ty;
      for (; p + (JPDSE_NORM_ILP - 1) * g.TY < p1; p += JPDSE_NORM_ILP * g.TY) {
        float v[JPDSE_NORM_ILP][VE];
#pragma unroll
        for (int u = 0; u < JPDSE_NORM_ILP; ++u) Vec16<T>::load(x + base + (long long)(p + u * g.TY) * g.Cs, v[u]);
#pragma unroll
        for (int u = 0; u < JPDSE_NORM_ILP; ++u) f.acc(v[u], aux, s1, s2);
      }
      for (; p < p1; p += g.TY) f.at(base + (long long)p * g.Cs, aux, s1, s2);
    } else {
      BwdMoments<T> f{x, dy, stats, act, slope};
      float mean[VE], rstd[VE];
      {
        const float* st = stats + ((long long)n * g.Cs + c0) * 2;
#pragma unroll
        for (int e = 0; e < VE; ++e) { mean[e] = st[2 * e]; rstd[e] = st[2 * e + 1]; }
      }
      int p = p0 + ty;
      for (; p + (JPDSE_NORM_ILP - 1) * g.TY < p1; p += JPDSE_NORM_ILP * g.TY) {
        float v[JPDSE_NORM_ILP][VE], gr[JPDSE_NORM_ILP][VE];
#pragma unroll
        for (int u = 0; u < JPDSE_NORM_ILP; ++u) {
          const long long off = base + (long long)(p + u * g.TY) * g.Cs;
          Vec16<T>::load(x + off, v[u]);
          Vec16<T>::load(dy + off, gr[u]);
        }
#pragma unroll
        for (int u = 0; u < JPDSE_NORM_ILP; ++u) f.acc2(v[u], gr[u], mean, rstd, s1, s2);
      }
      for (; p < p1; p += g.TY) {
        float v[VE], gr[VE];
        Vec16<T>::load(x + base + (long long)p * g.Cs, v);
        Vec16<T>::load(dy + base + (long long)p * g.Cs, gr);
        f.acc2(v, gr, mean, rstd, s1, s2);
      }
    }
  }
#pragma unroll
  for (int e = 0; e < VE; ++e) {
    red[(threadIdx.x * VE + e) * 2] = s1[e];
    red[(threadIdx.x * VE + e) * 2 + 1] = s2[e];
  }
  __syncthreads();
  if (ty == 0 && on) {
    float* out = partial + (((long long)n * g.splits + split) * g.Cs + c0) * 2;
#pragma unroll
    for (int e = 0; e < VE; ++e) {
      float a = 0.f, b = 0.f;
      for (int y = 0; y < g.TY; ++y) {
        a += red[((y * g.TX + tx) * VE + e) * 2];
        b += red[((y * g.TX + tx) * VE + e) * 2 + 1];
      }
      out[2 * e] = a;
      out[2 * e + 1] = b;
    }
  }
}

__device__ __forceinline__ void reduce_splits(const float* __restrict__ partial, int n, int c, int Cs, int splits,
                                              int sub, float& a, float& b) {
  a = 0.f;
  b = 0.f;
  const long long stride = (long long)Cs * 2;
  const float* p = partial + (((long long)n * splits + sub) * Cs + c) * 2;
  int s = sub;
  for (; s + 24 < splits; s += 32, p += 32 * stride) {
    const float2 v0 = *reinterpret_cast<const float2*>(p);
    const float2 v1 = *reinterpret_cast<const float2*>(p + 8 * stride);
    const float2 v2 = *reinterpret_cast<const float2*>(p + 16 * stride);
    const float2 v3 = *reinterpret_cast<const float2*>(p + 24 * stride);
    a += v0.x; b += v0.y;
    a += v1.x; b += v1.y;
    a += v2.x; b += v2.y;
    a += v3.x; b += v3.y;
  }
  for (; s < splits; s += 8, p += 8 * stride) {
    const float2 v = *reinterpret_cast<const float2*>(p);
    a += v.x;
    b += v.y;
  }
#pragma unroll
  for (int off = 4; off > 0; off >>= 1) {
    a += __shfl_xor(a, off, 64);
    b += __shfl_xor(b, off, 64);
  }
// ... 51 lines not shown
  const int n = blockIdx.x / (col_blocks * g.splits);
  const int col = cb * g.TX + tx;
  if (col >= g.cv) return;
  const int c0 = col * VE;
  float mean[VE], rstd[VE];
  const float* st = stats + ((long long)n * g.Cs + c0) * 2;
#pragma unroll
  for (int e = 0; e < VE; ++e) { mean[e] = st[2 * e]; rstd[e] = st[2 * e + 1]; }
  const int p0 = split * g.pix_per_split;
  int p1 = p0 + g.pix_per_split;
  p1 = p1 < g.HW ? p1 : g.HW;
  const long long base = (long long)n * g.HW * g.Cs + c0;
  for (int p = p0 + ty; p < p1; p += JPDSE_NORM_ILP * g.TY) {
    float v[JPDSE_NORM_ILP][VE], r[JPDSE_NORM_ILP][VE];
#pragma unroll
    for (int u = 0; u < JPDSE_NORM_ILP; ++u) {
      const int pu = p + u * g.TY;
      if (pu < p1) {
        const long long off = base + (long long)pu * g.Cs;
        JPDSE_LOAD_LAST(T, x + off, v[u]);
        if (res != nullptr) Vec16<T>::load(res + off, r[u]);
      }
    }
#pragma unroll
    for (int u = 0; u < JPDSE_NORM_ILP; ++u) {
      const int pu = p + u * g.TY;
      if (pu >= p1) break;
#pragma unroll
      for (int e = 0; e < VE; ++e) {
        float t = norm_act(v[u][e], mean[e], rstd[e], act, slope);
        if (res != nullptr) t += r[u][e];
        v[u][e] = t;
      }
      Vec16<T>::store(y + base + (long long)pu * g.Cs, v[u]);
    }
  }
}

template <typename T>
__global__ __launch_bounds__(256) void inorm_apply_bwd_kernel(const T* __restrict__ x, const T* __restrict__ dy,
                                                            T* __restrict__ dx, const float* __restrict__ stats,
                                                            const float* __restrict__ sums, int act, float slope,
                                                            MomentGeom g) {
  constexpr int VE = Vec16<T>::N;
  const int tx = threadIdx.x & (g.TX - 1), ty = threadIdx.x >> g.tx_shift;
  const int col_blocks = (g.cv + g.TX - 1) / g.TX;
  const int cb = blockIdx.x % col_blocks;
  const int split = (blockIdx.x / col_blocks) % g.splits;
  const int n = blockIdx.x / (col_blocks * g.splits);
  const int col = cb * g.TX + tx;
  if (col >= g.cv) return;
  const int c0 = col * VE;
  float mean[VE], rstd[VE], s1[VE], s2[VE];
  const long long sidx = ((long long)n * g.Cs + c0) * 2;
#pragma unroll
  for (int e = 0; e < VE; ++e) {
    mean[e] = stats[sidx + 2 * e];
    rstd[e] = stats[sidx + 2 * e + 1];
    s1[e] = sums[sidx + 2 * e];
    s2[e] = sums[sidx + 2 * e + 1];
  }
  const int p0 = split * g.pix_per_split;
  int p1 = p0 + g.pix_per_split;
  p1 = p1 < g.HW ? p1 : g.HW;
  const long long base = (long long)n * g.HW * g.Cs + c0;
  for (int p = p0 + ty; p < p1; p += JPDSE_NORM_ILP * g.TY) {
    float v[JPDSE_NORM_ILP][VE], gr[JPDSE_NORM_ILP][VE];
#pragma unroll
    for (int u = 0; u < JPDSE_NORM_ILP; ++u) {
      const int pu = p + u * g.TY;
      if (pu < p1) {
        const long long off = base + (long long)pu * g.Cs;
        JPDSE_LOAD_LAST(T, x + off, v[u]);
        JPDSE_LOAD_LAST(T, dy + off, gr[u]);
      }
    }
#pragma unroll
    for (int u = 0; u < JPDSE_NORM_ILP; ++u) {
      const int pu = p + u * g.TY;
      if (pu >= p1) break;
#pragma unroll
      for (int e = 0; e < VE; ++e) {
        const float yh = (v[u][e] - mean[e]) * rstd[e];
        const float dz = gr[u][e] * act_grad(yh, act, slope);
        v[u][e] = rstd[e] * (dz - s1[e] - yh * s2[e]);
      }
      Vec16<T>::store(dx + base + (long long)pu * g.Cs, v[u]);
    }
  }
}


static inline int norm_form() {
#ifdef JPDSE_DEV
  return g_norm_fused;
#else
  return 1;
#endif
}
#ifdef JPDSE_DEV
int g_norm_fused = 1;
#endif

struct FusedGeom {
  int N, HW, Cs, cv;
  int TX, TY, tx_shift;
  int col_blocks, splits, span;
  int nv;
};

static FusedGeom fused_geom(int N, int HW, int Cs, int VE, int P) {
  FusedGeom g;
  g.N = N; g.HW = HW; g.Cs = Cs; g.cv = Cs / VE;
  int tx = 1;
  while (tx < g.cv && tx < 16) tx <<= 1;
  g.TX = tx; g.TY = 256 / tx;
  g.tx_shift = 0;
  while ((1 << g.tx_shift) < tx) ++g.tx_shift;
  g.col_blocks = (g.cv + g.TX - 1) / g.TX;
  g.span = g.TY * P;
  g.splits = (HW + g.span - 1) / g.span;
  g.nv = g.TX * VE * 2;
  return g;
}

template <int VE>
__device__ __forceinline__ float block_row(float* red, const float (&s1)[8], const float (&s2)[8], const FusedGeom& g) {
  const int tid = threadIdx.x;
  const int tx = tid & (g.TX - 1), ty = tid >> g.tx_shift;
#pragma unroll
  for (int e = 0; e < VE; ++e) {
    red[ty * g.nv + (tx * VE + e) * 2] = s1[e];
    red[ty * g.nv + (tx * VE + e) * 2 + 1] = s2[e];
  }
  __syncthreads();
  float tsum = 0.f;
  if (tid < g.nv)
    for (int yy = 0; yy < g.TY; ++yy) tsum += red[yy * g.nv + tid];
  __syncthreads();
  return tsum;
}

__device__ __forceinline__ float sum_rows(const float* rows, int splits, int nv) {
  float total = 0.f;
  for (int s0 = 0; s0 < splits; s0 += 16) {
    float v[16];
#pragma unroll
    for (int k = 0; k < 16; ++k) {
      const float* q = rows + (long long)(s0 + k) * nv;
      v[k] = 0.f;
      if (s0 + k < splits) v[k] = *q;
    }
#pragma unroll
    for (int k = 0; k < 16; ++k) total += v[k];
  }
  return total;
}

__device__ __forceinline__ void group_totals(float* red, const float* partial, int grp, const FusedGeom& g) {
  const int tid = threadIdx.x;
  const float* rows = partial + (long long)grp * g.splits * g.nv;
  const float total = tid < g.nv ? sum_rows(rows + tid, g.splits, g.nv) : 0.f;
  if (tid < g.nv) red[tid] = total;
  __syncthreads();
}

// ... 79 lines not shown
#pragma unroll
  for (int e = 0; e < VE; ++e) {
    if constexpr (PHASE == 3) {
      mean[e] = red[(tx * VE + e) * 2];
      rstd[e] = rsqrtf(red[(tx * VE + e) * 2 + 1] + eps);
    } else {
      const float dm = red[(tx * VE + e) * 2] * inv;
      float var = red[(tx * VE + e) * 2 + 1] * inv - dm * dm;
      var = var > 0.f ? var : 0.f;
      mean[e] = aux[e] + dm;
      rstd[e] = rsqrtf(var + eps);
    }
  }
  if (on && split == 0 && ty == 0) {
    float* st = stats + ((long long)n * g.Cs + c0) * 2;
#pragma unroll
    for (int e = 0; e < VE; ++e) { st[2 * e] = mean[e]; st[2 * e + 1] = rstd[e]; }
  }
#pragma unroll
  for (int i = 0; i < P; ++i) {
    const int p = p0 + i * g.TY;
    if (on && p < g.HW) {
      const long long off = base + (long long)p * g.Cs;
      float v[VE], r[VE];
      Vec16<T>::unpack(xv[i], v);
      if (res != nullptr) Vec16<T>::load(res + off, r);
#pragma unroll
      for (int e = 0; e < VE; ++e) {
        float t = norm_act(v[e], mean[e], rstd[e], act, slope);
        if (res != nullptr) t += r[e];
        v[e] = t;
      }
      Vec16<T>::store(y + off, v);
    }
  }
}

template <typename T, int P, int PHASE>
__global__ __launch_bounds__(256, (P == 8 ? 3 : 2)) void inorm_reg_bwd_kernel(const T* __restrict__ x, const T* __restrict__ dy,
                                                                             T* __restrict__ dx,
                                                                             const float* __restrict__ stats, float* partial,
                                                                             unsigned* unused, int act, float slope,
                                                                             FusedGeom g, int mslots = 0) {
  static_assert(PHASE >= 1 && PHASE <= 3, "PHASE 0 (in-launch exchange) is retired");
  constexpr int VE = Vec16<T>::N;
  __shared__ float red[256 * VE * 2];
  const int tid = threadIdx.x;
  const int tx = tid & (g.TX - 1), ty = tid >> g.tx_shift;
  const int split = blockIdx.x % g.splits, grp = blockIdx.x / g.splits;
  const int cb = grp % g.col_blocks, n = grp / g.col_blocks;
  const int col = cb * g.TX + tx;
  const bool on = col < g.cv;
  const int c0 = (on ? col : 0) * VE;
  const long long base = (long long)n * g.HW * g.Cs + c0;
  const int p0 = split * g.span + ty;
  u32x4 xv[P], gv[P];
#pragma unroll
  for (int i = 0; i < P; ++i) {
    const int p = p0 + i * g.TY;
    if (on && p < g.HW) {
      xv[i] = *reinterpret_cast<const u32x4*>(x + base + (long long)p * g.Cs);
      gv[i] = *reinterpret_cast<const u32x4*>(dy + base + (long long)p * g.Cs);
    }
  }
  float mean[VE], rstd[VE], s1[8], s2[8];
#pragma unroll
  for (int e = 0; e < 8; ++e) { s1[e] = 0.f; s2[e] = 0.f; }
  {
    const float* st = stats + ((long long)n * g.Cs + c0) * 2;
#pragma unroll
    for (int e = 0; e < VE; ++e) { mean[e] = st[2 * e]; rstd[e] = st[2 * e + 1]; }
  }
  if constexpr (PHASE == 3) {
    const int nch = g.TX * VE;
    if (tid < nch) {
      const int ch = cb * nch + tid;
      float a = 0.f, b = 0.f;
      if (ch < g.Cs) {
        const float2* const src = reinterpret_cast<const float2*>(partial) + ((long long)n * g.Cs + ch) * mslots;
        for (int q = 0; q < mslots; ++q) {
          const float2 v = src[q];
          a += v.x;
          b += v.y;
        }
      }
      red[tid * 2] = a;
      red[tid * 2 + 1] = b;
    }
    __syncthreads();
  } else if constexpr (PHASE == 2) {
    group_totals(red, partial, grp, g);
  } else {
#pragma unroll
    for (int i = 0; i < P; ++i) {
      const int p = p0 + i * g.TY;
      if (on && p < g.HW) {
        float v[VE], gr[VE];
        Vec16<T>::unpack(xv[i], v);
        Vec16<T>::unpack(gv[i], gr);
#pragma unroll
        for (int e = 0; e < VE; ++e) {
          const float yh = (v[e] - mean[e]) * rstd[e];
          const float dz = gr[e] * act_grad(yh, act, slope);
          s1[e] += dz;
          s2[e] += dz * yh;
        }
      }
    }
    const float tsum = block_row<VE>(red, s1, s2, g);
    if (tid < g.nv) partial[((long long)grp * g.splits + split) * g.nv + tid] = tsum;
    return;
  }
  float m1[VE], m2[VE];
  const float inv = 1.f / (float)g.HW;
#pragma unroll
  for (int e = 0; e < VE; ++e) {
    m1[e] = red[(tx * VE + e) * 2] * inv;
    m2[e] = red[(tx * VE + e) * 2 + 1] * inv;
  }
#pragma unroll
  for (int i = 0; i < P; ++i) {
    const int p = p0 + i * g.TY;
// ... 38 lines not shown
    a += v1.x;
    a += v2.x;
    a += v3.x;
  }
  for (; s < slots; s += 64) a += src[s].x;
  const float mean = wave_sum(a) / (float)slots;
  const float ns = (float)HW / (float)slots;
  float b = 0.f;
  for (s = lane; s < slots; s += 64) {
    const float2 v = src[s];
    const float dm = v.x - mean;
    b += v.y + ns * dm * dm;
  }
  b = wave_sum(b);
  if (lane == 0) {
    float var = b / (float)HW;
    var = var > 0.f ? var : 0.f;
    stats[2 * pair] = mean;
    stats[2 * pair + 1] = rsqrtf(var + eps);
  }
}

__global__ __launch_bounds__(256) void finalize_bwd_slots_kernel(const float* __restrict__ slots_in, float* __restrict__ sums, int NC,
                                                                int slots, int HW) {
  const int gid = blockIdx.x * blockDim.x + threadIdx.x;
  const int idx = gid >> 3, sub = gid & 7;
  float a = 0.f, b = 0.f;
  if (idx < NC) {
    const float2* const src = reinterpret_cast<const float2*>(slots_in) + (long long)idx * slots;
    for (int q = sub; q < slots; q += 8) {
      const float2 v = src[q];
      a += v.x;
      b += v.y;
    }
  }
#pragma unroll
  for (int off = 1; off < 8; off <<= 1) {
    a += __shfl_xor(a, off, 64);
    b += __shfl_xor(b, off, 64);
  }
  if (idx >= NC || sub != 0) return;
  const float inv = 1.f / (float)HW;
  sums[2 * idx] = a * inv;
  sums[2 * idx + 1] = b * inv;
}

struct NormCall {
  const jpdse_inorm_desc* d;
  const void* x;
  const void* in2;
  void* out;
  float* stats;
  void* stream;
};

static MomentGeom moment_geom(const jpdse_inorm_desc* d) {
  return moment_geom(d->N, d->H * d->W, cpad(d->C), vec_elems(d->dtype));
}
static dim3 moment_grid(const MomentGeom& g) { return dim3(g.N * g.splits * ((g.cv + g.TX - 1) / g.TX)); }
static dim3 lanes8_grid(const jpdse_inorm_desc* d) { return dim3((d->N * cpad(d->C) * 8 + 255) / 256); }
static dim3 fused_grid(const FusedGeom& g) { return dim3((unsigned)((size_t)g.N * g.col_blocks * g.splits)); }

static size_t ws_sums_bytes(const jpdse_inorm_desc* d) { return align_up((size_t)d->N * cpad(d->C) * 2 * sizeof(float), 256); }
static size_t ws_sums_offset(const jpdse_inorm_desc* d, const MomentGeom& g) {
  return align_up((size_t)d->N * g.splits * g.Cs * 2 * sizeof(float), 256);
}
static size_t ws_bytes_for(const jpdse_inorm_desc* d) {
  const size_t three = ws_sums_offset(d, moment_geom(d)) + ws_sums_bytes(d), reg = reg_ws_bytes(d);
  return three > reg ? three : reg;
}

template <typename T, int PHASE, bool BWD>
static int launch_reg(const NormCall& c, const FusedGeom& fg, float* part, int mslots = 0) {
  static const char* const what[2][3] = {{"inorm rows fwd", "inorm apply-from-rows fwd", "inorm apply-from-slots fwd"},
                                         {"inorm rows bwd", "inorm apply-from-rows bwd", "inorm apply-from-slots bwd"}};
  const jpdse_inorm_desc* d = c.d;
  if constexpr (BWD)
    return launch256(what[1][PHASE - 1], inorm_reg_bwd_kernel<T, 8, PHASE>, fused_grid(fg), c.stream, cptr<T>(c.x), cptr<T>(c.in2),
                     mptr<T>(c.out), c.stats, part, (unsigned*)nullptr, d->act, d->slope, fg, mslots);
  else
    return launch256(what[0][PHASE - 1], inorm_reg_fwd_kernel<T, 8, PHASE>, fused_grid(fg), c.stream, cptr<T>(c.x), cptr<T>(c.in2),
                     mptr<T>(c.out), c.stats, part, (unsigned*)nullptr, d->act, d->slope, d->eps, fg, mslots);
}

constexpr int kNoRegForm = 1;

template <typename T, bool BWD> static int try_reg(const NormCall& c, void* ws) {
  FusedGeom fg;
  if (norm_form() == 0 || !reg_geom<T>(c.d, &fg)) return kNoRegForm;
  float* part = mptr<float>(ws);
  if (int rc = launch_reg<T, 1, BWD>(c, fg, part)) return rc;
  return launch_reg<T, 2, BWD>(c, fg, part);
}

template <typename T, bool BWD> static int try_reg_from_slots(const NormCall& c, const float* slots_in, int slots) {
  FusedGeom fg;
  if (norm_form() == 0 || slots > 64 || !reg_geom<T>(c.d, &fg)) return kNoRegForm;
  return launch_reg<T, 3, BWD>(c, fg, const_cast<float*>(slots_in), slots);
}

template <typename T, bool BWD> static int launch_apply(const NormCall& c, const MomentGeom& g, const float* sums = nullptr) {
  if constexpr (BWD)
    return launch256("inorm apply bwd", inorm_apply_bwd_kernel<T>, moment_grid(g), c.stream, cptr<T>(c.x), cptr<T>(c.in2),
                     mptr<T>(c.out), c.stats, sums, c.d->act, c.d->slope, g);
  else
    return launch256("inorm apply fwd", inorm_apply_fwd_kernel<T>, moment_grid(g), c.stream, cptr<T>(c.x), cptr<T>(c.in2),
                     mptr<T>(c.out), c.stats, c.d->act, c.d->slope, g);
}

template <typename T> static int inorm_fwd_t(const NormCall& c, void* ws) {
  if (const int r = try_reg<T, false>(c, ws); r != kNoRegForm) return r;
  const jpdse_inorm_desc* d = c.d;
  const MomentGeom g = moment_geom(d);
  float* partial = mptr<float>(ws);
  if (int rc = launch256("inorm moment fwd", moment_kernel<T, false>, moment_grid(g), c.stream, cptr<T>(c.x), nullptr, nullptr, 0,
                         0.f, partial, g))
    return rc;
  if (int rc = launch256("inorm finalize fwd", finalize_fwd_kernel<T>, lanes8_grid(d), c.stream, cptr<T>(c.x), partial, c.stats,
                         d->N, g.HW, g.Cs, g.splits, d->eps))
    return rc;
  return launch_apply<T, false>(c, g);
}

template <typename T> static int inorm_bwd_t(const NormCall& c, void* ws) {
  if (const int r = try_reg<T, true>(c, ws); r != kNoRegForm) return r;
  const jpdse_inorm_desc* d = c.d;
  const MomentGeom g = moment_geom(d);
  float* partial = mptr<float>(ws);
  float* sums = reinterpret_cast<float*>(mptr<char>(ws) + ws_sums_offset(d, g));
  if (int rc = launch256("inorm moment bwd", moment_kernel<T, true>, moment_grid(g), c.stream, cptr<T>(c.x), cptr<T>(c.in2),
                         c.stats, d->act, d->slope, partial, g))
    return rc;
  if (int rc = launch256("inorm finalize bwd", finalize_bwd_kernel, lanes8_grid(d), c.stream, partial, sums, d->N, g.HW, g.Cs,
                         g.splits))
    return rc;
  return launch_apply<T, true>(c, g, sums);
}

template <typename T> static int inorm_bwd_from_sums_t(const NormCall& c, const float* slot_sums, int slots, void* ws) {
  if (const int r = try_reg_from_slots<T, true>(c, slot_sums, slots); r != kNoRegForm) return r;
  const jpdse_inorm_desc* d = c.d;
  float* const sums = mptr<float>(ws);
  if (int rc = launch256("inorm finalize bwd from slots", finalize_bwd_slots_kernel, lanes8_grid(d), c.stream, slot_sums, sums,
                         d->N * cpad(d->C), slots, d->H * d->W))
    return rc;
  return launch_apply<T, true>(c, moment_geom(d), sums);
}

template <typename T> static int inorm_from_moments_t(const NormCall& c, const float* mom, int slots) {
  if (const int r = try_reg_from_slots<T, false>(c, mom, slots); r != kNoRegForm) return r;
  const jpdse_inorm_desc* d = c.d;
  const int NC = d->N * cpad(d->C);
  if (int rc = launch256("inorm finalize from moments", finalize_slots_kernel, dim3((NC + 3) / 4), c.stream, mom, c.stats, NC,
                         slots, d->H * d->W, d->eps))
    return rc;
  return launch_apply<T, false>(c, moment_geom(d));
}

static int validate(const jpdse_inorm_desc* d) {
  JPDSE_REQUIRE(d != nullptr, "inorm: null descriptor");
  JPDSE_REQUIRE(d->dtype == JPDSE_F32 || d->dtype == JPDSE_BF16, "inorm: bad dtype");
  JPDSE_REQUIRE(d->N > 0 && d->H > 0 && d->W > 0 && d->C > 0, "inorm: non-positive shape");
  JPDSE_REQUIRE(d->act == JPDSE_ACT_NONE || d->act == JPDSE_ACT_RELU || d->act == JPDSE_ACT_LRELU,
                "inorm: unsupported activation %d", d->act);
  return JPDSE_OK;
}

enum NormWs { WS_NONE, WS_FULL, WS_SUMS };
static int inorm_enter(const char* name, const jpdse_inorm_desc* d, bool args_ok, const char* args_what, const void** residual,
                       NormWs kind, const void* ws, size_t ws_bytes) {
  if (int rc = validate(d)) return rc;
  JPDSE_REQUIRE(args_ok, "%s: %s", name, args_what);
  if (residual != nullptr) {
    JPDSE_REQUIRE(!d->has_residual || *residual, "%s: has_residual set but residual is null", name);
    if (!d->has_residual) *residual = nullptr;
  }
  if (kind != WS_NONE) {
    const size_t need = kind == WS_FULL ? ws_bytes_for(d) : ws_sums_bytes(d);
    if (ws == nullptr || ws_bytes < need) return set_error(JPDSE_EWORKSPACE, "%s: workspace %zu < %zu", name, ws_bytes, need);
  }
  return JPDSE_OK;
}

template <typename F> static int timed_by_dtype(const jpdse_inorm_desc* d, void* stream, int cls, double tensors, F&& run) {
  const int pslot = hbm_prof_begin(as_stream(stream));
  const int rc = by_dtype(d->dtype, run);
  hbm_prof_end(pslot, cls, (double)d->N * d->H * d->W * cpad(d->C) * (double)esize(d->dtype) * tensors, as_stream(stream));
  return rc;
}

}

using namespace jpdse;

extern "C" {

size_t jpdse_inorm_workspace_size(const jpdse_inorm_desc* d) {
  if (jpdse::validate(d)) return 0;
  return ws_bytes_for(d);
}

int jpdse_inorm_fwd(const jpdse_inorm_desc* d, const void* x, const void* residual, void* y, float* stats, void* ws,
                    size_t ws_bytes, void* stream) {
  if (int rc = inorm_enter("inorm_fwd", d, x && y && stats, "null pointer", &residual, WS_FULL, ws, ws_bytes)) return rc;
  const NormCall c = {d, x, residual, y, stats, stream};
  return timed_by_dtype(d, stream, JPDSE_HBM_INORM_FWD, d->has_residual ? 4.0 : 3.0,
                        [&](auto tag) { return inorm_fwd_t<decltype(tag)>(c, ws); });
}

int jpdse_inorm_bwd(const jpdse_inorm_desc* d, const void* x, const float* stats, const void* dy, void* dx, void* ws,
                    size_t ws_bytes, void* stream) {
  if (int rc = inorm_enter("inorm_bwd", d, x && stats && dy && dx, "null pointer", nullptr, WS_FULL, ws, ws_bytes)) return rc;
  const NormCall c = {d, x, dy, dx, const_cast<float*>(stats), stream};
  return timed_by_dtype(d, stream, JPDSE_HBM_INORM_BWD, 5.0, [&](auto tag) { return inorm_bwd_t<decltype(tag)>(c, ws); });
}

int jpdse_inorm_bwd_from_sums(const jpdse_inorm_desc* d, const void* x, const float* stats, const void* dy, const float* sums,
                              int32_t slots, void* dx, void* ws, size_t ws_bytes, void* stream) {
  if (int rc = inorm_enter("inorm_bwd_from_sums", d, x && stats && dy && dx && sums && slots > 0, "null pointer / no slots",
                           nullptr, WS_SUMS, ws, ws_bytes))
    return rc;
  const NormCall c = {d, x, dy, dx, const_cast<float*>(stats), stream};
  return timed_by_dtype(d, stream, JPDSE_HBM_INORM_BWD, 3.0,
                        [&](auto tag) { return inorm_bwd_from_sums_t<decltype(tag)>(c, sums, slots, ws); });
}

int jpdse_inorm_fwd_from_moments(const jpdse_inorm_desc* d, const void* x, const float* moments, int32_t slots,
                                 const void* residual, void* y, float* stats, void* stream) {
  if (int rc = inorm_enter("inorm_fwd_from_moments", d, x && y && stats && moments && slots > 0, "null pointer / no slots",
                           &residual, WS_NONE, nullptr, 0))
    return rc;
  const NormCall c = {d, x, residual, y, stats, stream};
  return timed_by_dtype(d, stream, JPDSE_HBM_INORM_FWD, d->has_residual ? 3.0 : 2.0,
                        [&](auto tag) { return inorm_from_moments_t<decltype(tag)>(c, moments, slots); });
}

}
```

jpd-se_amd/csrc/thin_out1.h:

```cpp
#pragma once
#include "common.h"

namespace jpdse {

struct Thin1DgradArgs {
  const bf16_t* DY;
  const bf16_t* B;
  float* taps;
  bf16_t* DX;
  const bf16_t* addend;
  int N, H, W, Cs, OH, OW;
  int py, px;
  long long b_stride;
  int Lk;
  int nseg, segw;
};

typedef float f32x2 __attribute__((ext_vector_type(2)));

constexpr int kThin1Run = 64;

__global__ __launch_bounds__(256) void thin1_taps_kernel(const bf16_t* __restrict__ B, float* __restrict__ taps, int Cs, long long b_stride,
                                                         int Lk, int S, int ntaps) {
  const int i = blockIdx.x * 256 + threadIdx.x;
  if (i >= ntaps * Cs) return;
  const int t = i / Cs, c = i - t * Cs;
  taps[i] = bf2f(B[(long long)c * b_stride + (t / S) * Lk + (t % S) * 8]);
}

template <int R, int S>
__global__ __launch_bounds__(256) void thin1_dgrad_kernel(const Thin1DgradArgs a) {
  __shared__ float dyw[32][R][kThin1Run + S];
  const int cv = a.Cs >> 3;
  const int cg = threadIdx.x & (cv - 1);
  const int pl = threadIdx.x / cv, PL = 256 / cv;
  f32x2 w[R * S][4];
#pragma unroll
  for (int t = 0; t < R * S; ++t) {
    const float4 lo = *reinterpret_cast<const float4*>(a.taps + t * a.Cs + cg * 8);
    const float4 hi = *reinterpret_cast<const float4*>(a.taps + t * a.Cs + cg * 8 + 4);
    w[t][0] = (f32x2){lo.x, lo.y};
    w[t][1] = (f32x2){lo.z, lo.w};
    w[t][2] = (f32x2){hi.x, hi.y};
    w[t][3] = (f32x2){hi.z, hi.w};
  }
  const int items = a.N * a.H * a.nseg;
  const int rounds = (items + gridDim.x * PL - 1) / (gridDim.x * PL);
  for (int k = 0; k < rounds; ++k) {
    const int it = (k * gridDim.x + blockIdx.x) * PL + pl;
    const bool live = it < items;
    const int itc = live ? it : 0;
    const int seg = itc % a.nseg, row = itc / a.nseg;
    const int ih = row % a.H, n = row / a.H;
    const int w0 = seg * a.segw;
    int wn = a.W - w0;
    wn = wn < a.segw ? wn : a.segw;
    wn = live ? wn : 0;
    __syncthreads();
    for (int j = cg; j < R * (kThin1Run + S); j += cv) {
      const int u = j / (kThin1Run + S), c = j - u * (kThin1Run + S);
      const int oh = ih - a.py + u, ow = w0 - a.px + c;
      const bool ok = live && c < wn + S - 1 && ((unsigned)oh < (unsigned)a.OH) & ((unsigned)ow < (unsigned)a.OW);
      dyw[pl][u][c] = ok ? bf2f(a.DY[(((long long)n * a.OH + oh) * a.OW + ow) * 8]) : 0.f;
    }
    __syncthreads();
    float win[S][R];
#pragma unroll
    for (int v = 1; v < S; ++v)
#pragma unroll
      for (int u = 0; u < R; ++u) win[v][u] = dyw[pl][u][v - 1];
    bf16_t* __restrict__ out = a.DX + (((long long)n * a.H + ih) * a.W + w0) * a.Cs + cg * 8;
    const bf16_t* __restrict__ add = a.addend != nullptr ? a.addend + (out - a.DX) : nullptr;
    for (int i0 = 0; i0 < wn; i0 += 4) {
      u32x4 adv[4];
      if (add != nullptr) {
#pragma unroll
        for (int q = 0; q < 4; ++q)
          if (i0 + q < wn) adv[q] = *reinterpret_cast<const u32x4*>(add + (long long)(i0 + q) * a.Cs);
      }
#pragma unroll
      for (int q = 0; q < 4; ++q) {
        const int i = i0 + q;
        if (i >= wn) break;
#pragma unroll
        for (int v = 0; v + 1 < S; ++v)
#pragma unroll
          for (int u = 0; u < R; ++u) win[v][u] = win[v + 1][u];
#pragma unroll
        for (int u = 0; u < R; ++u) win[S - 1][u] = dyw[pl][u][i + S - 1];
        f32x2 acc[4];
#pragma unroll
        for (int e = 0; e < 4; ++e) acc[e] = (f32x2){0.f, 0.f};
#pragma unroll
        for (int u = 0; u < R; ++u)
#pragma unroll
          for (int v = 0; v < S; ++v) {
            const f32x2 g = {win[v][u], win[v][u]};
#pragma unroll
            for (int e = 0; e < 4; ++e) acc[e] += g * w[u * S + v][e];
          }
        float o[8];
#pragma unroll
        for (int e = 0; e < 4; ++e) { o[2 * e] = acc[e].x; o[2 * e + 1] = acc[e].y; }
        if (add != nullptr) {
          float ad[8];
          Vec16<bf16_t>::unpack(adv[q], ad);
#pragma unroll
          for (int e = 0; e < 8; ++e) o[e] = bf16_round(o[e]) + ad[e];
        }
        Vec16<bf16_t>::store(out + (long long)i * a.Cs, o);
      }
    }
  }
}

struct Thin1WgradArgs {
  const bf16_t* X;
  const bf16_t* DY;
  float* partial;
  int N, H, W, Cs, OH, OW, pad;
  int nseg, segw;
  int items_per_strip;
};

constexpr int kThin1SegW = 32;
// ... 170 lines not shown
```

jpd-se_amd/ctu/models/pix2pixHD_model.py:

```python
import contextlib
import os

import torch
import torch.distributed as dist

from jpdse_hip import F32, JpdseError, require_gpu
from jpdse_hip import ops
from jpdse_hip.ops import Act
from jpdse_hip.optim import FusedAdam
from jpdse_hip.layers import PackBatcher
from ctu.utils.image_pool import ImagePool
from ctu.models.codec import CODECS
from ctu.models.coded_calls import CodedCalls
from ctu.models.model_options import add_model_options, parse_class_distortion_weights, resolve_model_options
from ctu.models.pix2pixHD_networks.base_model import BaseModel
from ctu.models.pix2pixHD_networks import networks

LOSS_NAMES = ('G_GAN', 'G_GAN_Feat', 'G_VGG', 'G_Distortion', 'D_real', 'D_fake')
FORWARD_MODES = {m: (m, {}) for m in ('get_img', 'get_train_loss', 'get_eval_loss', 'get_code', 'get_eval_rate',
                                      'get_eval_metrics', 'get_rate_map', 'get_class_rates')}
FORWARD_MODES['get_eval_metrics_per_class'] = ('get_eval_metrics', dict(per_class=True))


class Pix2PixHDModel(CodedCalls, BaseModel):
# ... 307 lines not shown
    s = lambda i: slots[i:i + 1]
    gw = grad_w or {}
    d_feat, d_vgg, d_dist = None, None, None
    with ops.deferred_loss_finals():
      for i in range(nD if run_d else 0):
        p = pred[i][-1]
        ops.mse_const_fwd(p.batch_slice(0, B), 0.0, s(layout['D_fake'][i]))
        ops.mse_const_fwd(p.batch_slice(B, 2 * B), 1.0, s(layout['D_real'][i]))
        ops.mse_const_fwd(p.batch_slice(0, B), 1.0, s(layout['G_GAN'][i]))
        for j in range(nF):
          f = pred[i][j]
          ff, fr = f.batch_slice(0, B), f.batch_slice(B, 2 * B)
          if gw.get('feat') and j < nF - 1:
            d_feat = d_feat if d_feat is not None else [[None] * nF for _ in range(nD)]
            d_feat[i][j] = ops.l1_fwd_bwd(ff, fr, s(layout['feat'][i][j]), gw['feat'] / nD)
          else:
            ops.l1_fwd(ff, fr, s(layout['feat'][i][j]))
      wk = networks.VGGLoss.weights
      for k in range(len(vf)):
        if gw.get('vgg') and v_ctx is not None:
          d_vgg = d_vgg if d_vgg is not None else [None] * len(vf)
          d_vgg[k] = ops.l1_fwd_bwd(vf[k], vr[k], s(layout['vgg'][k]), gw['vgg'] * wk[k], relu_a=True)
        else:
          ops.l1_fwd(vf[k], vr[k], s(layout['vgg'][k]))
      d_dist = self._distortion(fake, real, label, pre['inst_raw'], s(layout['dist']), gw.get('dist'))
    state = dict(B=B, fake=fake, real=real, g_ctx=g_ctx, e_ctx=e_ctx, pred=pred, d_ctx=d_ctx, vf=vf, vr=vr, v_ctx=v_ctx,
                 d_feat=d_feat, d_vgg=d_vgg, d_dist=d_dist, label=label, inst_raw=pre['inst_raw'])
    return state, slots, layout

  def _reduce_losses(self, vals, layout):
    nD = self.opt.num_D
    w = networks.VGGLoss.weights
    L = dict(
        G_GAN=sum(vals[i] for i in layout['G_GAN']),
        G_GAN_Feat=sum((1.0 / nD) * vals[i] for row in layout['feat'] for i in row),
        G_VGG=sum(w[k] * vals[i] for k, i in enumerate(layout['vgg'])),
        G_Distortion=vals[layout['dist']],
        D_real=sum(vals[i] for i in layout['D_real']),
        D_fake=sum(vals[i] for i in layout['D_fake']))
    if 'rate' in layout:
      L['G_Rate'] = vals[layout['rate']]
    return L

  def get_train_loss(self, x_dict):
    state, slots, layout = self._forward_losses(x_dict)
    L = self._reduce_losses(slots.cpu().tolist(), layout)
    return tuple(torch.tensor(L[k], device=slots.device) for k in LOSS_NAMES)

  def _ones(self, dev):
    if self._one is None or self._one.device != dev:
      self._one = torch.ones(1, dtype=torch.float32, device=dev)
    return self._one

  def backward_G(self, state, w_gan, w_feat, w_vgg, w_dist):
    opt, B = self.opt, state['B']
    one = self._ones(state['fake'].t.device)
    fake, real = state['fake'], state['real']
    d_fake = None
    if (w_gan != 0.0 or w_feat != 0.0) and state['pred'] is not None:
      dres = []
      for i in range(opt.num_D):
        row = []
        for j, f in enumerate(state['pred'][i]):
          ff, fr = f.batch_slice(0, B), f.batch_slice(B, 2 * B)
          if j == len(state['pred'][i]) - 1:
            row.append(ops.mse_const_bwd(ff, 1.0, one, w_gan) if w_gan != 0.0 else None)
          elif w_feat == 0.0:
            row.append(None)
          elif state.get('d_feat') is not None and state['d_feat'][i][j] is not None:
            row.append(state['d_feat'][i][j])
          else:
            row.append(ops.l1_bwd(ff, fr, one, w_feat / opt.num_D))
        dres.append(row)
      d_fake = self.netD.bwd(state['d_ctx'], dres, need_dx=True, need_dw=False, batch=(0, B),
                             dx_channels=(self.label_nc, self.label_nc + fake.C))
    if w_vgg != 0.0 and state['v_ctx'] is not None:
      wk = networks.VGGLoss.weights
      dmaps = state.get('d_vgg') or [ops.l1_bwd(state['vf'][k], state['vr'][k], one, w_vgg * wk[k], relu_a=True)
                                     for k in range(len(wk))]
      dv = self.criterionVGG.vgg.bwd(state['v_ctx'], dmaps)
      d_fake = dv if d_fake is None else ops.add_(d_fake, dv)
    if w_dist != 0.0:
      if state.get('d_dist') is not None:
        dd = state['d_dist']
      elif opt.distortion_loss_fn == 'ms_ssim' or self.sem_weights is not None:
        dd = self._distortion(fake, real, state['label'], state['inst_raw'],
                              torch.empty(1, dtype=torch.float32, device=fake.t.device), w_dist)
      else:
        fn = ops.l1_bwd if opt.distortion_loss_fn == 'l1' else ops.mse_bwd
        dd = fn(fake, real, one, w_dist)
      d_fake = dd if d_fake is None else ops.add_(d_fake, dd)
    if d_fake is None:
      return False
    if state['e_ctx'] is None:
      self.netG.bwd(state['g_ctx'], d_fake, need_dx=False, need_dw=True)
      return True
    d_feat_map = self.netG.bwd(state['g_ctx'], d_fake, need_dx=True, need_dw=True,
                               dx_channels=(self.label_nc, self.label_nc + self.feat_nc))
    self.netE.bwd(state['e_ctx'], d_feat_map)
    return True

  def g_nets(self):
    if self.netE is None:
      return self.netG
    if getattr(self, '_g_nets', None) is None:
      self.__dict__['_g_nets'] = torch.nn.ModuleList([self.netG, self.netE])
    return self._g_nets

  def _repack(self, which):
    if not hasattr(self, '_pack_batchers'):
      self._pack_batchers = {}
    b = self._pack_batchers.get(which)
    if b is None:
      b = self._pack_batchers[which] = PackBatcher(self.g_nets() if which == 'G' else self.netD)
    b.run()

  def backward_D(self, state, w_d):
    if w_d == 0.0 or state['pred'] is None:
      return False
    opt, B = self.opt, state['B']
    one = self._ones(state['fake'].t.device)
    dres = []
    for i in range(opt.num_D):
      p = state['pred'][i][-1]
      dp = p.empty_like()
      ops.mse_const_bwd(p.batch_slice(0, B), 0.0, one, w_d, out=dp.batch_slice(0, B))
      ops.mse_const_bwd(p.batch_slice(B, 2 * B), 1.0, one, w_d, out=dp.batch_slice(B, 2 * B))
      dres.append([None] * (len(state['pred'][i]) - 1) + [dp])
    self.netD.bwd(state['d_ctx'], dres, need_dx=False, need_dw=True)
    return True

  def train_step(self, x_dict, optimizer_G, optimizer_D, lambda_distortion_weight=1.0):
    opt = self.opt
    w_gan = 0.0 if opt.no_g_gan_loss else 1.0
    w_feat = 0.0 if opt.no_gan_feat_loss else opt.lambda_feat
    w_vgg = 0.0 if opt.no_vgg_loss else opt.lambda_feat
    w_dist = 0.0 if opt.no_distortion_loss else opt.lambda_distortion * lambda_distortion_weight
    state, slots, layout = self._forward_losses(x_dict, grad_w=dict(feat=w_feat, vgg=w_vgg, dist=w_dist))
    early = getattr(self, 'early_loss_readback', True)
    if early:
      loss_host, loss_ready = self._queue_loss_readback(slots)
    bg, bd = self.grad_buckets.get('G'), self.grad_buckets.get('D')
    tl = getattr(self, 'ddp_timeline', None)
    marks = {} if tl is not None else None

    def mark(name):
      if marks is not None:
        ev = torch.cuda.Event(enable_timing=True)
        ev.record()
        marks[name] = ev

    did_G = self.backward_G(state, w_gan, w_feat, w_vgg, w_dist)
    mark('g_bwd_end')
    if did_G and bg is not None:
      bg.launch_all()
    did_D = self.backward_D(state, 0.0 if opt.no_d_gan_loss else 0.5)
    mark('d_bwd_end')
    if did_G:
      if bg is not None:
        bg.finish()
      mark('g_reduced')
      optimizer_G.step()
      self._repack('G')
      mark('adam_g_end')
    if did_D:
      if bd is not None:
        bd.finish()
      mark('d_reduced')
      optimizer_D.step()
      self._repack('D')
    mark('step_end')
    if tl is not None:
      marks['stats_G'] = dict(bg.stats) if bg is not None and bg.stats else None
      marks['stats_D'] = dict(bd.stats) if bd is not None and bd.stats else None
      tl.append(marks)
    if not early:
      loss_host, loss_ready = self._queue_loss_readback(slots)
    loss_ready.synchronize()
    return self._reduce_losses(loss_host.tolist(), layout)

  def _queue_loss_readback(self, slots):
    n = slots.numel()
    buf = getattr(self, '_loss_pinned', None)
    if buf is None or buf.numel() < n:
      buf = self._loss_pinned = torch.empty(max(n, 64), dtype=torch.float32).pin_memory()
    host = buf[:n]
    host.copy_(slots, non_blocking=True)
    ev = torch.cuda.Event()
    ev.record(torch.cuda.current_stream(slots.device))
    return host, ev

  def save(self):
    self.save_network(self.netG, 'G', self.opt)
    self.save_network(self.netD, 'D', self.opt)
    if self.netE is not None:
      self.save_network(self.netE, 'E', self.opt)

  def update_fixed_params(self, optimizer_G):
    for p in self.netG.parameters():
      p.requires_grad_(True)
    for m in self.netG.modules():
      if hasattr(m, 'ensure_grads'):
        m.ensure_grads()
    params = list(self.netG.parameters())
    if self.netE is not None:
      params += list(self.netE.parameters())
    return FusedAdam(params, lr=self.opt.lr, betas=(self.opt.beta1, 0.999),
                     grad_scale=getattr(optimizer_G, 'grad_scale', 1.0))
```

jpd-se_amd/ctu/models/pix2pixHD_networks/networks.py:

```python
import torch
import torch.nn as nn

from jpdse_hip import (ACT_NONE, ACT_RELU, ACT_LRELU, ACT_TANH, PAD_ZERO, PAD_REFLECT, F32, BF16, JpdseError,
                       require_gpu)
from jpdse_hip import ops
from jpdse_hip.ops import Act
from jpdse_hip.layers import (HipConv2d, HipResnetBlock, HipBinarizer, HipVQBottleneck, vq_bottleneck_check, InstNormAct,
                              ConvNormAct, Ctx, _Slot,
                              run_chain_fwd, run_chain_bwd)

ResnetBlock = HipResnetBlock

VGG_CFG = (64, 64, 'M', 128, 128, 'M', 256, 256, 256, 256, 'M', 512, 512, 512, 512, 'M', 512)
VGG_TAPS = (0, 2, 4, 8, 12)


def dtype_code(name):
  if name in (F32, BF16):
    return name
  table = {'fp32': F32, 'float32': F32, 'f32': F32, 'bf16': BF16, 'bfloat16': BF16}
  if name not in table:
    raise ValueError('compute dtype must be fp32 or bf16, got %r' % (name,))
  return table[name]

# ... 337 lines not shown
    nf = ndf
    for _ in range(1, n_layers):
      nf = min(nf * 2, 512)
      chans.append(nf)
    chans.append(min(nf * 2, 512))
    chans.append(1)
    self._stages = []
    for j in range(n_layers + 2):
      stride = 2 if j < n_layers else 1
      if j == 0:
        conv = HipConv2d(chans[0], chans[1], 4, stride, 2, PAD_ZERO, act=ACT_LRELU, slope=0.2, **kw)
        seq, stage = nn.Sequential(conv, _Slot()), conv
      elif j <= n_layers:
        conv = HipConv2d(chans[j], chans[j + 1], 4, stride, 2, PAD_ZERO, apply_bias=False, **kw)
        seq, stage = nn.Sequential(conv, _Slot(), _Slot()), ConvNormAct(conv, InstNormAct(ACT_LRELU, 0.2))
      else:
        conv = HipConv2d(chans[j], 1, 4, 1, 2, PAD_ZERO, **kw)
        seq, stage = nn.Sequential(conv), conv
      setattr(self, 'model' + str(j), seq)
      self._stages.append(stage)

  def fwd(self, x):
    feats, ctxs = [], []
    for st in self._stages:
      x, c = st.fwd(x)
      feats.append(x)
      ctxs.append(c)
    return feats, ctxs

  def bwd(self, ctxs, dfeats, need_dx=False, need_dw=True, dx_channels=None):
    d = None
    fused = False
    dz0 = False
    for j in range(len(self._stages) - 1, -1, -1):
      if dfeats[j] is not None and not fused:
        d = dfeats[j] if d is None else ops.add_(d, dfeats[j])
      fused = False
      if d is None:
        continue
      lrelu0 = dict(relu_input=True, input_slope=self._stages[0].slope) if (j == 1 and self.fuse_lrelu0) else {}
      if j == 0 and dx_channels is not None and need_dx and not need_dw:
        d = self._stages[0].bwd_input_slice(ctxs[0], d, dx_channels[0], dx_channels[1], dy_is_dz=dz0)
      elif j == 0:
        d = self._stages[0].bwd(ctxs[0], d, need_dx, need_dw, dy_is_dz=dz0)
      elif dfeats[j - 1] is not None:
        d = self._stages[j].bwd(ctxs[j], d, True, need_dw, addend=dfeats[j - 1], **lrelu0)
        fused = True
      else:
        d = self._stages[j].bwd(ctxs[j], d, True, need_dw, **lrelu0)
      dz0 = bool(lrelu0)
    return d


class MultiscaleDiscriminator(nn.Module):

  def __init__(self, input_nc, ndf=64, n_layers=3, norm_layer=None, use_sigmoid=False, num_D=3,
               getIntermFeat=True, compute_dtype='fp32', device=None):
    super(MultiscaleDiscriminator, self).__init__()
    if not getIntermFeat:
      raise NotImplementedError('the JPD-SE model always requests intermediate features')
    self.num_D, self.n_layers, self.getIntermFeat = num_D, n_layers, True
    self.cdtype = dtype_code(compute_dtype)
    self._scales = []
    for i in range(num_D):
      netD = NLayerDiscriminator(input_nc, ndf, n_layers, norm_layer, use_sigmoid, True, compute_dtype, device)
      for j in range(n_layers + 2):
        setattr(self, 'scale' + str(i) + '_layer' + str(j), getattr(netD, 'model' + str(j)))
      self._scales.append(netD)

  def fwd(self, x):
    result, ctxs, h = [], [], x
    for i in range(self.num_D):
      feats, c = self._scales[self.num_D - 1 - i].fwd(h)
      result.append(feats)
      ctxs.append((c, h.H, h.W))
      if i != self.num_D - 1:
        h = ops.avgpool3s2_fwd(h)
    return result, ctxs

  def bwd(self, ctxs, dresult, need_dx=False, need_dw=True, batch=None, dx_channels=None):
    dx = None
    for i in range(self.num_D - 1, -1, -1):
      c, H, W = ctxs[i]
      if batch is not None:
        c = [ci.slice(batch[0], batch[1]) for ci in c]
      d = self._scales[self.num_D - 1 - i].bwd(c, dresult[i], need_dx, need_dw, dx_channels)
      if need_dx:
        if dx is not None:
          d = ops.add_(d, ops.avgpool3s2_bwd(dx, H, W))
        dx = d
    return dx

  def forward(self, input, keep_input=False):
    if keep_input:
      raise NotImplementedError('--match_raw_feat is outside the JPD-SE hot path')
    result, _ = self.fwd(_to_act(input, self.cdtype))
    return [[ops.nhwc_to_nchw(f) for f in scale] for scale in result]


def define_D(input_nc, ndf, n_layers_D, norm='instance', use_sigmoid=False, num_D=1, getIntermFeat=False,
             gpu_ids=[], compute_dtype='fp32'):
  get_norm_layer(norm)
  device = torch.device('cuda', gpu_ids[0]) if len(gpu_ids) > 0 else None
  if device is not None:
    require_gpu(gpu_ids[0])
  return MultiscaleDiscriminator(input_nc, ndf, n_layers_D, None, use_sigmoid, num_D, getIntermFeat,
                                 compute_dtype, device)


class Vgg19(nn.Module):

  def __init__(self, requires_grad=False, compute_dtype='fp32', device=None, seed=20):
    super(Vgg19, self).__init__()
    self.cdtype = dtype_code(compute_dtype)
    convs, cin = [], 3
    g = torch.Generator().manual_seed(seed)
    for item in VGG_CFG:
      if item == 'M':
        continue
      conv = HipConv2d(cin, item, 3, 1, 1, PAD_ZERO, act=ACT_RELU, dtype=self.cdtype, device=device)
      std = (2.0 / (cin * 9)) ** 0.5
      with torch.no_grad():
        conv.weight.copy_(torch.randn(item, cin, 3, 3, generator=g) * std)
        conv.bias.copy_(torch.randn(item, generator=g) * 0.01)
      convs.append(conv)
      cin = item
    self.convs = nn.ModuleList(convs)
    for p in self.parameters():
      p.requires_grad = requires_grad

  def load_torchvision_state_dict(self, sd):
    idx, ci = 0, 0
    with torch.no_grad():
      for item in VGG_CFG:
        if item == 'M':
          idx += 1
          continue
        self.convs[ci].weight.copy_(sd['features.%d.weight' % idx])
        self.convs[ci].bias.copy_(sd['features.%d.bias' % idx])
        idx, ci = idx + 2, ci + 1

  def fwd(self, x, save=True):
    maps, ctxs, ci = [], [], 0
    pooled = None
# ... 80 lines not shown
```

jpd-se_amd/jpdse_hip/__init__.py:

```python
import ctypes
import os

_HERE = os.path.dirname(os.path.abspath(__file__))
LIB_PATH = os.environ.get('JPDSE_HIP_LIB') or os.path.join(_HERE, 'libjpdse_hip.so')

F32, BF16 = 0, 1
PAD_ZERO, PAD_REFLECT = 0, 1
ACT_NONE, ACT_RELU, ACT_LRELU, ACT_TANH = 0, 1, 2, 3


class JpdseError(RuntimeError):
  pass


class ConvDesc(ctypes.Structure):
  _fields_ = [('dtype', ctypes.c_int32), ('N', ctypes.c_int32), ('H', ctypes.c_int32),
              ('W', ctypes.c_int32), ('C', ctypes.c_int32), ('K', ctypes.c_int32),
              ('R', ctypes.c_int32), ('S', ctypes.c_int32), ('stride', ctypes.c_int32),
              ('pad', ctypes.c_int32), ('pad_mode', ctypes.c_int32), ('act', ctypes.c_int32),
              ('slope', ctypes.c_float)]


class InormDesc(ctypes.Structure):
  _fields_ = [('dtype', ctypes.c_int32), ('N', ctypes.c_int32), ('H', ctypes.c_int32),
              ('W', ctypes.c_int32), ('C', ctypes.c_int32), ('act', ctypes.c_int32),
              ('slope', ctypes.c_float), ('eps', ctypes.c_float), ('has_residual', ctypes.c_int32)]


class PackEntry(ctypes.Structure):
  _fields_ = [('w', ctypes.c_void_p), ('out', ctypes.c_void_p)] + \
             [(n, ctypes.c_int32) for n in ('K', 'Ks', 'C', 'Cs', 'R', 'S', 'st', 'qh', 'qw', 'Uh', 'Uw', 'Lk', 'gx', 'gy',
                                            'out_f32', 'reserved_')] + \
             [('blocks', ctypes.c_int64), ('block0', ctypes.c_int64)]


class LossTerm(ctypes.Structure):
  _fields_ = [('partial', ctypes.c_void_p), ('n', ctypes.c_int32), ('inv_count', ctypes.c_float), ('out', ctypes.c_void_p)]


class AdamEntry(ctypes.Structure):
  _fields_ = [('p', ctypes.c_void_p), ('g', ctypes.c_void_p), ('m', ctypes.c_void_p),
              ('v', ctypes.c_void_p), ('n', ctypes.c_int64), ('block0', ctypes.c_int64),
              ('cast_bf16', ctypes.c_void_p)]


class EvalMetricsSemArgs(ctypes.Structure):
  _fields_ = [(n, ctypes.c_int32) for n in ('dtype_fake', 'dtype_real', 'N', 'H', 'W', 'C')] + \
             [('fake', ctypes.c_void_p), ('real', ctypes.c_void_p), ('label', ctypes.c_void_p), ('n_classes', ctypes.c_int32),
              ('mean', ctypes.POINTER(ctypes.c_double)), ('std', ctypes.POINTER(ctypes.c_double)), ('out', ctypes.c_void_p),
              ('cls', ctypes.c_void_p), ('ws', ctypes.c_void_p), ('ws_bytes', ctypes.c_size_t), ('stream', ctypes.c_void_p)]


class MsssimLossArgs(ctypes.Structure):
  _fields_ = [(n, ctypes.c_int32) for n in ('dtype', 'N', 'H', 'W', 'C')] + \
             [('fake', ctypes.c_void_p), ('real', ctypes.c_void_p), ('mean', ctypes.POINTER(ctypes.c_double)),
              ('std', ctypes.POINTER(ctypes.c_double)), ('out', ctypes.c_void_p), ('stats', ctypes.c_void_p),
              ('dfake', ctypes.c_void_p), ('scale', ctypes.c_float), ('ws', ctypes.c_void_p), ('ws_bytes', ctypes.c_size_t),
              ('stream', ctypes.c_void_p)]


class CodeRateArgs(ctypes.Structure):
  _fields_ = [(n, ctypes.c_int32) for n in ('dtype', 'N', 'H', 'W', 'C')] + \
             [('pixels', ctypes.c_int64), ('b', ctypes.c_void_p), ('t', ctypes.c_void_p), ('grad', ctypes.c_void_p),
              ('scale', ctypes.c_float), ('out', ctypes.c_void_p), ('per_image', ctypes.c_void_p), ('counts', ctypes.c_void_p),
              ('ws', ctypes.c_void_p), ('ws_bytes', ctypes.c_size_t), ('stream', ctypes.c_void_p)]


class SemLossArgs(ctypes.Structure):
  _fields_ = [(n, ctypes.c_int32) for n in ('dtype', 'N', 'H', 'W', 'C', 'kind')] + \
             [('fake', ctypes.c_void_p), ('real', ctypes.c_void_p), ('label', ctypes.c_void_p), ('inst', ctypes.c_void_p),
              ('table', ctypes.POINTER(ctypes.c_float)), ('n_table', ctypes.c_int32), ('edge_w', ctypes.c_float),
              ('scale', ctypes.c_float), ('out', ctypes.c_void_p), ('dfake', ctypes.c_void_p), ('ws', ctypes.c_void_p),
              ('ws_bytes', ctypes.c_size_t), ('stream', ctypes.c_void_p)]


class CodeCostArgs(ctypes.Structure):
  _fields_ = [(n, ctypes.c_int32) for n in ('dtype', 'N', 'h', 'w', 'C')] + \
             [('b', ctypes.c_void_p), ('H', ctypes.c_int32), ('W', ctypes.c_int32), ('label', ctypes.c_void_p),
              ('n_classes', ctypes.c_int32), ('symbol', ctypes.c_void_p), ('cell', ctypes.c_void_p), ('channel', ctypes.c_void_p),
# ... 103 lines not shown

class VqRateFwdArgs(ctypes.Structure):
  _fields_ = [(n, ctypes.c_int32) for n in ('dtype', 'M', 'D', 'L', 'G')] + \
             [('sigma', ctypes.c_float), ('hard', ctypes.c_int32), ('x', ctypes.c_void_p), ('code_book', ctypes.c_void_p),
              ('scale', ctypes.c_float), ('denom', ctypes.c_float), ('hist', ctypes.c_void_p), ('rate', ctypes.c_void_p),
              ('dhist', ctypes.c_void_p), ('ws', ctypes.c_void_p), ('ws_bytes', ctypes.c_size_t), ('stream', ctypes.c_void_p)]


class VqQuantizeBwdGroupedArgs(ctypes.Structure):
  _fields_ = [(n, ctypes.c_int32) for n in ('dtype', 'M', 'D', 'L', 'G')] + \
             [('sigma', ctypes.c_float), ('dy', ctypes.c_void_p), ('x', ctypes.c_void_p), ('code_book', ctypes.c_void_p),
              ('dhist', ctypes.c_void_p), ('dx', ctypes.c_void_p), ('dcode_book', ctypes.c_void_p), ('ws', ctypes.c_void_p),
              ('ws_bytes', ctypes.c_size_t), ('stream', ctypes.c_void_p)]


class VqLloydAccumArgs(ctypes.Structure):
  _fields_ = [(n, ctypes.c_int32) for n in ('dtype', 'M', 'D', 'L', 'first')] + \
             [(n, ctypes.c_void_p) for n in ('x', 'code_book', 'counts', 'sums', 'sse', 'far_dist', 'far_vec', 'ws')] + \
             [('ws_bytes', ctypes.c_size_t), ('stream', ctypes.c_void_p)]


class VqLloydUpdateArgs(ctypes.Structure):
  _fields_ = [(n, ctypes.c_int32) for n in ('D', 'L', 'reseed')] + \
             [(n, ctypes.c_void_p) for n in ('code_book', 'counts', 'sums', 'sse', 'far_dist', 'far_vec', 'report', 'stream')]


_P, _I32, _I64, _F, _SZ = (ctypes.c_void_p, ctypes.c_int32, ctypes.c_int64, ctypes.c_float,
                           ctypes.c_size_t)
_CD, _ND = ctypes.POINTER(ConvDesc), ctypes.POINTER(InormDesc)

SIGNATURES = {
    'jpdse_version': (_I32, []),
    'jpdse_last_error': (ctypes.c_char_p, []),
    'jpdse_arch_check': (_I32, [_I32]),
    'jpdse_prof_select': (_I32, [_I32, _I32, _I64, _I32]),
    'jpdse_prof_collect': (_I32, [ctypes.POINTER(ctypes.c_double), ctypes.POINTER(ctypes.c_double), ctypes.POINTER(_I64)]),
    'jpdse_prof_collect_class': (_I32, [_I32, ctypes.POINTER(ctypes.c_double), ctypes.POINTER(ctypes.c_double), ctypes.POINTER(_I64)]),
    'jpdse_prof_hbm_select': (_I32, [_I32, _I32]),
    'jpdse_prof_hbm_collect': (_I32, [_I32, ctypes.POINTER(ctypes.c_double), ctypes.POINTER(ctypes.c_double), ctypes.POINTER(_I64)]),
    'jpdse_conv_out_shape': (_I32, [_CD, ctypes.POINTER(_I32), ctypes.POINTER(_I32)]),
    'jpdse_conv_plan_query': (_I32, [_CD, ctypes.POINTER(_I32), _I32]),
    'jpdse_conv_fwd_pack_size': (_SZ, [_CD]),
    'jpdse_conv_dgrad_pack_size': (_SZ, [_CD]),
    'jpdse_conv_pack_entries': (_I32, [_CD, _P, _P, ctypes.POINTER(PackEntry), _I32]),
    'jpdse_conv_pack_run': (_I32, [_P, _I32, _I64, _P]),
    'jpdse_conv_pack_weights': (_I32, [_CD, _P, _P, _P, _P]),
    'jpdse_conv_workspace_size': (_SZ, [_CD]),
    'jpdse_conv_fwd': (_I32, [_CD, _P, _P, _P, _P, _P, _SZ, _P]),
    'jpdse_conv_fwd_pool': (_I32, [_CD, _P, _P, _P, _P, _P, _P, _SZ, _P]),
    'jpdse_conv_dgrad': (_I32, [_CD, _P, _P, _P, _P, _SZ, _P]),
    'jpdse_conv_dgrad_relu': (_I32, [_CD, _P, _P, _P, _P, _P, _SZ, _P]),
    'jpdse_conv_dgrad_fused': (_I32, [_CD, _P, _P, _P, _P, _P, _P, _SZ, _P]),
    'jpdse_conv_dgrad_fused_lrelu': (_I32, [_CD, _P, _P, _P, _F, _P, _P, _P, _SZ, _P]),
    'jpdse_conv_dgrad_nsum_slots': (_I32, [_CD]),
    'jpdse_conv_dgrad_fused_nsums': (_I32, [_CD, _P, _P, _P, _P, _P, _P, _P, _I32, _F, _P, _P, _SZ, _P]),
    'jpdse_conv_wgrad': (_I32, [_CD, _P, _P, _P, _P, _SZ, _P]),
    'jpdse_convT_fwd': (_I32, [_CD, _P, _P, _P, _P, _SZ, _P]),
    'jpdse_conv_moment_slots': (_I32, [_CD]),
    'jpdse_convT_moment_slots': (_I32, [_CD]),
    'jpdse_conv_fwd_moments': (_I32, [_CD, _P, _P, _P, _P, _P, _SZ, _P]),
    'jpdse_convT_fwd_moments': (_I32, [_CD, _P, _P, _P, _P, _P, _SZ, _P]),
    'jpdse_inorm_fwd_from_moments': (_I32, [_ND, _P, _P, _I32, _P, _P, _P, _P]),
    'jpdse_convT_dgrad': (_I32, [_CD, _P, _P, _P, _P, _SZ, _P]),
    'jpdse_convT_wgrad': (_I32, [_CD, _P, _P, _P, _P, _SZ, _P]),
    'jpdse_inorm_workspace_size': (_SZ, [_ND]),
    'jpdse_inorm_fwd': (_I32, [_ND, _P, _P, _P, _P, _P, _SZ, _P]),
    'jpdse_inorm_bwd': (_I32, [_ND, _P, _P, _P, _P, _P, _SZ, _P]),
    'jpdse_inorm_bwd_from_sums': (_I32, [_ND, _P, _P, _P, _P, _I32, _P, _P, _SZ, _P]),
    'jpdse_avgpool3s2_fwd': (_I32, [_I32, _I32, _I32, _I32, _I32, _P, _P, _P]),
    'jpdse_avgpool3s2_bwd': (_I32, [_I32, _I32, _I32, _I32, _I32, _P, _P, _P]),
    'jpdse_maxpool2_fwd': (_I32, [_I32, _I32, _I32, _I32, _I32, _P, _P, _P]),
    'jpdse_maxpool2_bwd': (_I32, [_I32, _I32, _I32, _I32, _I32, _P, _P, _P, _P]),
    'jpdse_act_bwd': (_I32, [_I32, _I64, _I32, _F, _P, _P, _P, _P]),
    'jpdse_add': (_I32, [_I32, _I64, _P, _P, _P, _P]),
    'jpdse_channel_sum_workspace_size': (_SZ, [_I64, _I32]),
    'jpdse_channel_sum': (_I32, [_I32, _I64, _I32, _P, _P, _P, _SZ, _P]),
    'jpdse_channel_copy': (_I32, [_I32, _I64, _P, _I32, _I32, _P, _I32, _I32, _I32, _P]),
    'jpdse_concat_channels': (_I32, [_I32, _I64, _P, _I32, _P, _I32, _I32, _I32, _P, _P]),
    'jpdse_copy': (_I32, [_I64, _P, _P, _P]),
    'jpdse_zero': (_I32, [_I32, _I64, _P, _P]),
    'jpdse_cast': (_I32, [_I32, _I32, _I64, _P, _P, _P]),
    'jpdse_quant_loss_workspace_size': (_SZ, []),
    'jpdse_quant_loss': (_I32, [_I32, _I32, _I64, _I32, _P, _P, ctypes.POINTER(ctypes.c_double),
                                ctypes.POINTER(ctypes.c_double), _I32, _P, _P, _SZ, _P]),
    'jpdse_nchw_to_nhwc': (_I32, [_I32, _I32, _I32, _I32, _I32, _P, _P, _P]),
    'jpdse_nhwc_to_nchw': (_I32, [_I32, _I32, _I32, _I32, _I32, _P, _P, _P]),
    'jpdse_onehot_edge': (_I32, [_I32, _I32, _I32, _I32, _I32, _P, _P, _P, _I32, _P]),
    'jpdse_input_builder': (_I32, [_I32, _I32, _I32, _I32, _I32, _P, _P, _I32, ctypes.POINTER(_P), ctypes.POINTER(_P), _I32, _I32,
                                   _I32, _I32, _P]),
    'jpdse_input_builder_wide': (_I32, [_I32, _I32, _I32, _I32, _I32, _P, _P, _I32, ctypes.POINTER(_P), ctypes.POINTER(_P), _I32,
                                        _I32, _I32, _I32, _P]),
    'jpdse_insert_channels': (_I32, [_I32, _I64, _P, _I32, _P, _I32, _I32, _I32, _P]),
    'jpdse_loss_workspace_size': (_SZ, [_I64]),
    'jpdse_loss_partial_count': (_I32, [_I64]),
    'jpdse_loss_finalize': (_I32, [_P, _I32, _P]),
    'jpdse_l1_fwd': (_I32, [_I32, _I64, _I64, _P, _P, _P, _P, _SZ, _P]),
    'jpdse_l1_bwd': (_I32, [_I32, _I64, _I64, _P, _P, _P, _F, _P, _P]),
    'jpdse_l1_bwd_relu': (_I32, [_I32, _I64, _I64, _P, _P, _P, _F, _P, _P]),
    'jpdse_l1_fwd_bwd': (_I32, [_I32, _I64, _I64, _P, _P, _P, _F, _I32, _P, _P, _SZ, _P]),
    'jpdse_mse_fwd': (_I32, [_I32, _I64, _I64, _P, _P, _P, _P, _SZ, _P]),
    'jpdse_mse_bwd': (_I32, [_I32, _I64, _I64, _P, _P, _P, _F, _P, _P]),
    'jpdse_mse_const_fwd': (_I32, [_I32, _I64, _I32, _F, _P, _P, _P, _SZ, _P]),
    'jpdse_mse_const_bwd': (_I32, [_I32, _I64, _I32, _F, _P, _P, _F, _P, _P]),
    'jpdse_adam_step': (_I32, [_P, _I32, _I64, _F, _F, _F, _F, _I32, _F, _P]),
    'jpdse_binarize_fwd': (_I32, [_I32, _I32, _I32, _I32, _I32, _P, _P, _I32, ctypes.c_uint64, ctypes.c_uint64, _I64, _P, _P]),
    'jpdse_code_stats_workspace_size': (_SZ, [_I32, _I32, _I32, _I32, _I32]),
# ... 139 lines not shown
```

jpd-se_amd/jpdse_hip/layers.py:

```python
import math

import torch
import torch.nn as nn

from . import ACT_NONE, ACT_RELU, ACT_LRELU, ACT_TANH, PAD_ZERO, PAD_REFLECT, F32, BF16, binding_epoch
from . import ops
from .ops import Act
from .panels import WeightPanels, ALIAS, CAST, PACKED, bump_weights_epoch


class Ctx(object):
  __slots__ = ('items',)

  def __init__(self, *items):
    self.items = items

  def slice(self, b0, b1):
    out = []
    for it in self.items:
      if isinstance(it, Act):
        out.append(it.batch_slice(b0, b1))
      elif torch.is_tensor(it):
        out.append(it[b0:b1])
      elif isinstance(it, Ctx):
# ... 105 lines not shown
    if self.apply_bias or self.act != ACT_NONE or self.cdtype != BF16:
      return None
    dims = (x.N, 2 * x.H, 2 * x.W) if self.transposed else (x.N, x.H, x.W)
    slots = self._route_answer(ops.conv_moment_slots, dims, self.transposed)
    if slots <= 0:
      return None
    fwd_pack, dgrad_pack = self.packs()
    y, mom = ops.conv_fwd_moments(self._desc(*dims), x, dgrad_pack if self.transposed else fwd_pack, slots, self.transposed)
    return y, (Ctx(x) if self.transposed else Ctx(x, None)), mom, slots

  def nsum_slots(self, N, H, W):
    if self.transposed or self.cdtype != BF16:
      return 0
    return self._route_answer(ops.conv_dgrad_nsum_slots, (N, H, W))

  def _route_answer(self, query, dims, *args):
    key = (query, binding_epoch(), dims)
    if key not in self._route_answers:
      self._route_answers[key] = query(self._desc(*dims), *args)
    return self._route_answers[key]

  def bwd(self, ctx, dy, need_dx=True, need_dw=True, dy_is_dz=False, relu_input=False, addend=None, input_slope=0.0, sink=None):
    fwd_pack, dgrad_pack = self.packs()
    need_dw = need_dw and self.weight.requires_grad
    if self.transposed:
      (x,) = ctx.items
      d = self._desc(x.N, 2 * x.H, 2 * x.W)
      if need_dw:
        ops.conv_wgrad(d, dy, x, self._wgrad_buffer())
        self._bgrad_buffer()
        self._fire()
      return ops.conv_fwd(d, dy, fwd_pack, None) if need_dx else None
    x, y = ctx.items
    d = self._desc(x.N, x.H, x.W)
    dz = dy if (self.act == ACT_NONE or dy_is_dz) else ops.act_bwd(y, dy, self.act, self.slope)
    if need_dw:
      ops.conv_wgrad(d, x, dz, self._wgrad_buffer())
      store = self._bgrad_buffer()
      if self.apply_bias:
        ops.channel_sum(dz, store)
        if self.bias.grad.data_ptr() != store.data_ptr():
          self.bias.grad.copy_(store[:self.cout])
      self._fire()
    if not need_dx:
      return None
    if sink is not None and input_slope == 0.0:
      slots = self.nsum_slots(x.N, x.H, x.W)
      if slots > 0:
        sx, sstats, sact, sslope = sink
        return ops.conv_dgrad_nsums(d, dz, dgrad_pack, slots, sx, sstats, sact, sslope,
                                    relu_input=x if relu_input else None, addend=addend)
    return ops.conv_dgrad(d, dz, dgrad_pack, relu_input=x if relu_input else None, addend=addend, mask_slope=input_slope)

  def bwd_input_slice(self, ctx, dy, c0, c1, dy_is_dz=False):
    assert not self.transposed
    x, y = ctx.items
    dz = dy if (self.act == ACT_NONE or dy_is_dz) else ops.act_bwd(y, dy, self.act, self.slope)
    w = self._master()
    d = ops.conv_desc(self.cdtype, x.N, x.H, x.W, c1 - c0, self.cout, self.k, self.k, self.stride, self.pad,
                      self.pad_mode, ACT_NONE, self.slope)
    if self._slice[0] != (c0, c1):
      self._slice = ((c0, c1), WeightPanels(PACKED, d))
    _, dgrad_pack = self._slice[1].get(w, lambda: w.detach()[:, c0:c1].contiguous(memory_format=torch.channels_last))
    return ops.conv_dgrad(d, dz, dgrad_pack)

  def _fire(self):
    if self.grad_ready_hook is not None:
      self.grad_ready_hook(self)


class HipBinarizer(nn.Module):

  def __init__(self, cin, cout, dtype=F32, device=None):
    super(HipBinarizer, self).__init__()
    self.conv = HipConv2d(cin, cout, 1, act=ACT_TANH, apply_bias=False, bias=False, dtype=dtype, device=device)
    self.seed, self.draw, self.n_global0 = 0, 0, 0
    self.noise_override = None
    self.rate_scale, self.rate_denom, self.rate_value = None, 0, None

  def fwd(self, x):
    t, ctx = self.conv.fwd(x)
    u, self.noise_override = self.noise_override, None
    b = ops.binarize_fwd(t, self.training, self.seed, self.draw, self.n_global0, u)
    if self.rate_scale is not None:
      self.rate_value, _, d_rate, _ = ops.code_rate_loss(b, t, self.rate_denom, self.rate_scale)
      ctx = Ctx(ctx, d_rate)
    return b, ctx

  def bwd(self, ctx, db, need_dx=True, need_dw=True):
    if len(ctx.items) == 2 and isinstance(ctx.items[0], Ctx):
      ctx, d_rate = ctx.items
      db = ops.add(db, d_rate)
    return self.conv.bwd(ctx, db, need_dx, need_dw)


def vq_bottleneck_check(cout, n_center, center_size, sigma, who='HipVQBottleneck'):
  if center_size < 1 or cout % center_size != 0:
    raise ValueError('%s: center_size %d does not divide the bottleneck\'s %d channels' % (who, center_size, cout))
  if ops.cpad(cout) != cout:
    raise ValueError('%s: %d channels are no multiple of 8: the NHWC tensor would carry padding lanes between the vectors'
                     % (who, cout))
  if not 1 <= center_size <= ops.VQ_MAX_D or not 2 <= n_center <= ops.VQ_MAX_L:
    raise ValueError('%s: center_size %d / n_center %d, the kernels take 1 .. %d and 2 .. %d'
                     % (who, center_size, n_center, ops.VQ_MAX_D, ops.VQ_MAX_L))
  if not (float(sigma) > 0.0 and float(sigma) != float('inf')):
    raise ValueError('%s: sigma must be a finite number > 0, got %r' % (who, sigma))
# ... 112 lines not shown
    ops.conv_pack_run(*ops.device_table(self._table, 0, sig, lambda: ops.conv_pack_table(entries), layers[0].weight.device))
    for m in layers:
      m._panels.mark_fresh(m.weight)
    return len(layers)


class InstNormAct(object):

  def __init__(self, act=ACT_NONE, slope=0.2, eps=1e-5):
    self.act, self.slope, self.eps = act, slope, eps

  def fwd(self, x, residual=None):
    y, stats = ops.inorm_fwd(x, self.act, self.slope, self.eps, residual)
    return y, Ctx(x, stats)

  def fwd_from_moments(self, x, mom, slots, residual=None):
    y, stats = ops.inorm_fwd_from_moments(x, mom, slots, self.act, self.slope, self.eps, residual)
    return y, Ctx(x, stats)

  def bwd(self, ctx, dy, need_dx=True, need_dw=True):
    x, stats = ctx.items
    return ops.inorm_bwd(x, stats, dy, self.act, self.slope, self.eps)

  def sink(self, ctx):
    x, stats = ctx.items
    return (x, stats, self.act, self.slope)


def conv_norm_fwd(conv, norm, x, residual=None):
  fused = conv.fwd_moments(x)
  if fused is not None:
    h, c, mom, slots = fused
    y, n = norm.fwd_from_moments(h, mom, slots, residual=residual)
    return y, c, n
  h, c = conv.fwd(x)
  y, n = norm.fwd(h, residual=residual)
  return y, c, n


class ConvNormAct(object):

  def __init__(self, conv, norm):
    self.conv, self.norm = conv, norm

  def fwd(self, x):
    y, c1, c2 = conv_norm_fwd(self.conv, self.norm, x)
    return y, Ctx(c1, c2)

  def bwd(self, ctx, dy, need_dx=True, need_dw=True, addend=None, **conv_kw):
    c1, c2 = ctx.items
    dh = self.norm.bwd(c2, dy)
    return self.conv.bwd(c1, dh, need_dx, need_dw, addend=addend, **conv_kw)

  def dy_sink(self, ctx):
    return self.norm.sink(ctx.items[1])


class _Slot(nn.Module):

  def forward(self, x):
    return x


class HipResnetBlock(nn.Module):

  def __init__(self, dim, dtype=F32, device=None):
    super(HipResnetBlock, self).__init__()
    mk = lambda: HipConv2d(dim, dim, 3, 1, 1, PAD_REFLECT, apply_bias=False, dtype=dtype, device=device)
    self.conv_block = nn.Sequential(_Slot(), mk(), _Slot(), _Slot(), _Slot(), mk(), _Slot())
    self.norm1 = InstNormAct(ACT_RELU)
    self.norm2 = InstNormAct(ACT_NONE)

  recompute = False

  def _fwd(self, x):
    h, c1, n1 = conv_norm_fwd(self.conv_block[1], self.norm1, x)
    y, c2, n2 = conv_norm_fwd(self.conv_block[5], self.norm2, h, residual=x)
    return y, Ctx(c1, n1, c2, n2)

  def fwd(self, x):
    y, ctx = self._fwd(x)
    return (y, Ctx(x)) if self.recompute else (y, ctx)

  accepts_dx_sink = True

  def bwd(self, ctx, dy, need_dx=True, need_dw=True, dx_sink=None):
    ctx = self.materialize(ctx)
    c1, n1, c2, n2 = ctx.items
    d = self.norm2.bwd(n2, dy)
    d = self.conv_block[5].bwd(c2, d, True, need_dw, sink=self.norm1.sink(n1) if self.fuse_norm_sums else None)
    d = self.norm1.bwd(n1, d)
    return self.conv_block[1].bwd(c1, d, need_dx, need_dw, addend=dy if need_dx else None,
                                  sink=dx_sink if self.fuse_norm_sums else None)

  fuse_norm_sums = True

  def materialize(self, ctx):
    if len(ctx.items) == 1:
      _, ctx = self._fwd(ctx.items[0])
    return ctx

  def dy_sink(self, ctx):
    if len(ctx.items) == 1:
      return None
    return self.norm2.sink(ctx.items[3])

# ... 24 lines not shown
```

jpd-se_amd/jpdse_hip/ops.py:

```python
import ctypes

import torch

from . import (lib, check, JpdseError, F32, BF16, ConvDesc, PackEntry, InormDesc, EvalMetricsSemArgs, MsssimLossArgs, CodeRateArgs, SemLossArgs, CodeCostArgs, ACT_NONE, PAD_ZERO, PAD_REFLECT)
from . import (VqSoftFwdArgs, VqHardFwdArgs, VqSoftBwdArgs, VqDecodeArgs, VqDecodeBwdArgs, VqArgmaxArgs, VqPmfArgs, VqPmfBwdArgs,
               VqQuantizeFwdArgs, VqQuantizeBwdArgs, VqRateFwdArgs, VqQuantizeBwdGroupedArgs, VqLloydAccumArgs, VqLloydUpdateArgs)


def cpad(c):
  return (c + 7) & ~7


def code_of(tdtype):
  if tdtype == torch.float32:
    return F32
  if tdtype == torch.bfloat16:
    return BF16
  raise TypeError('unsupported compute dtype %r' % (tdtype,))


def tdtype_of(code):
  return torch.bfloat16 if code == BF16 else torch.float32


# ... 90 lines not shown
  check(lib().jpdse_conv_pack_run(_p(table), n, total_blocks, _stream()), 'conv_pack_run')


def device_table(cache, slot, sig, build, device):
  if cache.get(slot, (None,))[0] != sig:
    arr, rest = build()
    cache[slot] = (sig, torch.frombuffer(bytearray(bytes(arr)), dtype=torch.uint8).to(device)) + rest
  return cache[slot][1:]


def _conv_ws(d, device):
  n = lib().jpdse_conv_workspace_size(ctypes.byref(d))
  return workspace(n, device), n


def conv_fwd(d, x, fwd_pack, bias, out=None):
  oh, ow = conv_out_shape(d)
  y = out if out is not None else Act.empty(d.N, oh, ow, d.K, d.dtype, x.t.device)
  ws, n = _conv_ws(d, x.t.device)
  check(lib().jpdse_conv_fwd(ctypes.byref(d), _p(x.t), _p(fwd_pack), _p(bias), _p(y.t), _p(ws), ws.numel(), _stream()),
        'conv_fwd')
  return y


def conv_fwd_pool(d, x, fwd_pack, bias):
  oh, ow = conv_out_shape(d)
  y = Act.empty(d.N, oh, ow, d.K, d.dtype, x.t.device)
  yp = Act.empty(d.N, oh // 2, ow // 2, d.K, d.dtype, x.t.device)
  ws, n = _conv_ws(d, x.t.device)
  check(lib().jpdse_conv_fwd_pool(ctypes.byref(d), _p(x.t), _p(fwd_pack), _p(bias), _p(y.t), _p(yp.t), _p(ws), ws.numel(),
                                  _stream()), 'conv_fwd_pool')
  return y, yp


def conv_dgrad(d, dy, dgrad_pack, relu_input=None, addend=None, mask_slope=0.0):
  dx = Act.empty(d.N, d.H, d.W, d.C, d.dtype, dy.t.device)
  ws, n = _conv_ws(d, dy.t.device)
  if relu_input is not None and mask_slope != 0.0:
    check(lib().jpdse_conv_dgrad_fused_lrelu(ctypes.byref(d), _p(dy.t), _p(dgrad_pack), _p(relu_input.t), float(mask_slope),
                                             _p(addend.t if addend is not None else None), _p(dx.t), _p(ws),
                                             ws.numel(), _stream()), 'conv_dgrad_fused_lrelu')
    return dx
  if relu_input is not None or addend is not None:
    check(lib().jpdse_conv_dgrad_fused(ctypes.byref(d), _p(dy.t), _p(dgrad_pack),
                                       _p(relu_input.t if relu_input is not None else None),
                                       _p(addend.t if addend is not None else None), _p(dx.t), _p(ws),
                                       ws.numel(), _stream()), 'conv_dgrad_fused')
    return dx
  check(lib().jpdse_conv_dgrad(ctypes.byref(d), _p(dy.t), _p(dgrad_pack), _p(dx.t), _p(ws), ws.numel(), _stream()),
        'conv_dgrad')
  return dx


def conv_dgrad_nsum_slots(d):
  return int(lib().jpdse_conv_dgrad_nsum_slots(ctypes.byref(d)))


def conv_dgrad_nsums(d, dy, dgrad_pack, slots, norm_x, norm_stats, norm_act, norm_slope, relu_input=None, addend=None):
  dx = Act.empty(d.N, d.H, d.W, d.C, d.dtype, dy.t.device)
  assert tuple(norm_x.t.shape) == tuple(dx.t.shape) and norm_x.dtype == dx.dtype
  sums = torch.empty((d.N, dx.Cs, slots, 2), dtype=torch.float32, device=dy.t.device)
  ws, n = _conv_ws(d, dy.t.device)
  check(lib().jpdse_conv_dgrad_fused_nsums(ctypes.byref(d), _p(dy.t), _p(dgrad_pack),
                                           _p(relu_input.t if relu_input is not None else None),
                                           _p(addend.t if addend is not None else None), _p(dx.t), _p(norm_x.t), _p(norm_stats),
                                           int(norm_act), float(norm_slope), _p(sums), _p(ws), ws.numel(), _stream()),
        'conv_dgrad_fused_nsums')
  dx.nsums = (sums, slots, norm_x.t.data_ptr())
  return dx


def conv_wgrad(d, x, dy, dw):
  ws, n = _conv_ws(d, x.t.device)
  check(lib().jpdse_conv_wgrad(ctypes.byref(d), _p(x.t), _p(dy.t), _p(dw), _p(ws), ws.numel(), _stream()), 'conv_wgrad')


def conv_moment_slots(d, transposed=False):
  fn = lib().jpdse_convT_moment_slots if transposed else lib().jpdse_conv_moment_slots
  return int(fn(ctypes.byref(d)))


def conv_fwd_moments(d, x, pack, slots, transposed=False):
  if transposed:
    y = Act.empty(d.N, d.H, d.W, d.C, d.dtype, x.t.device)
  else:
    oh, ow = conv_out_shape(d)
    y = Act.empty(d.N, oh, ow, d.K, d.dtype, x.t.device)
  mom = torch.empty((d.N, y.Cs, slots, 2), dtype=torch.float32, device=x.t.device)
  ws, n = _conv_ws(d, x.t.device)
  fn = lib().jpdse_convT_fwd_moments if transposed else lib().jpdse_conv_fwd_moments
  check(fn(ctypes.byref(d), _p(x.t), _p(pack), _p(y.t), _p(mom), _p(ws), ws.numel(), _stream()), 'conv_fwd_moments')
  return y, mom


def inorm_fwd_from_moments(x, mom, slots, act, slope=0.2, eps=1e-5, residual=None):
  d = InormDesc(x.dtype, x.N, x.H, x.W, x.C, act, slope, eps, 1 if residual is not None else 0)
  y = x.empty_like()
  stats = torch.empty((x.N, x.Cs, 2), dtype=torch.float32, device=x.t.device)
  check(lib().jpdse_inorm_fwd_from_moments(ctypes.byref(d), _p(x.t), _p(mom), slots,
                                           _p(residual.t if residual is not None else None), _p(y.t), _p(stats), _stream()),
        'inorm_fwd_from_moments')
  return y, stats


def inorm_fwd(x, act, slope=0.2, eps=1e-5, residual=None):
  d = InormDesc(x.dtype, x.N, x.H, x.W, x.C, act, slope, eps, 1 if residual is not None else 0)
  y = x.empty_like()
  stats = torch.empty((x.N, x.Cs, 2), dtype=torch.float32, device=x.t.device)
  n = lib().jpdse_inorm_workspace_size(ctypes.byref(d))
  ws = workspace(n, x.t.device)
  check(lib().jpdse_inorm_fwd(ctypes.byref(d), _p(x.t), _p(residual.t if residual is not None else None), _p(y.t),
                              _p(stats), _p(ws), ws.numel(), _stream()), 'inorm_fwd')
  return y, stats


def inorm_bwd(x, stats, dy, act, slope=0.2, eps=1e-5):
  d = InormDesc(x.dtype, x.N, x.H, x.W, x.C, act, slope, eps, 0)
  dx = x.empty_like()
  n = lib().jpdse_inorm_workspace_size(ctypes.byref(d))
  ws = workspace(n, x.t.device)
  if dy.nsums is not None and dy.nsums[2] == x.t.data_ptr():
    sums, slots, _ = dy.nsums
    check(lib().jpdse_inorm_bwd_from_sums(ctypes.byref(d), _p(x.t), _p(stats), _p(dy.t), _p(sums), slots, _p(dx.t), _p(ws),
                                          ws.numel(), _stream()), 'inorm_bwd_from_sums')
    return dx
  check(lib().jpdse_inorm_bwd(ctypes.byref(d), _p(x.t), _p(stats), _p(dy.t), _p(dx.t), _p(ws), ws.numel(), _stream()),
        'inorm_bwd')
  return dx


def avgpool3s2_fwd(x):
  y = Act.empty(x.N, (x.H - 1) // 2 + 1, (x.W - 1) // 2 + 1, x.C, x.dtype, x.t.device)
  check(lib().jpdse_avgpool3s2_fwd(x.dtype, x.N, x.H, x.W, x.C, _p(x.t), _p(y.t), _stream()), 'avgpool3s2_fwd')
  return y


def avgpool3s2_bwd(dy, H, W):
  dx = Act.empty(dy.N, H, W, dy.C, dy.dtype, dy.t.device)
  check(lib().jpdse_avgpool3s2_bwd(dy.dtype, dy.N, H, W, dy.C, _p(dy.t), _p(dx.t), _stream()), 'avgpool3s2_bwd')
  return dx


def maxpool2_fwd(x):
  y = Act.empty(x.N, x.H // 2, x.W // 2, x.C, x.dtype, x.t.device)
  check(lib().jpdse_maxpool2_fwd(x.dtype, x.N, x.H, x.W, x.C, _p(x.t), _p(y.t), _stream()), 'maxpool2_fwd')
  return y


def maxpool2_bwd(x, dy):
  dx = x.empty_like()
  check(lib().jpdse_maxpool2_bwd(x.dtype, x.N, x.H, x.W, x.C, _p(x.t), _p(dy.t), _p(dx.t), _stream()), 'maxpool2_bwd')
  return dx


def act_bwd(y, dy, act, slope=0.2):
  dz = y.empty_like()
  check(lib().jpdse_act_bwd(y.dtype, y.t.numel(), act, slope, _p(y.t), _p(dy.t), _p(dz.t), _stream()), 'act_bwd')
  return dz


def add(a, b):
  out = a.empty_like()
  check(lib().jpdse_add(a.dtype, a.t.numel(), _p(a.t), _p(b.t), _p(out.t), _stream()), 'add')
  return out


def add_(a, b):
  check(lib().jpdse_add(a.dtype, a.t.numel(), _p(a.t), _p(b.t), _p(a.t), _stream()), 'add')
  return a


def copy_(src, dst):
  nb = src.numel() * src.element_size()
  assert src.is_contiguous() and dst.is_contiguous() and nb == dst.numel() * dst.element_size()
  check(lib().jpdse_copy(nb, _p(src), _p(dst), _stream()), 'copy')
  return dst


def zero_(t):
  check(lib().jpdse_zero(code_of(t.dtype), t.numel(), _p(t), _stream()), 'zero')
# ... 659 lines not shown
```

Baseline: 156.9 images/sec.

## Batch discriminator backward for generator and D losses into one pass with aliased inputs

Runs the discriminator backward for the generator's fake-as-real gradient and the D loss's fake/real gradients together as one 3B-sized batch. Data-gradient convs and instance-norm backward read the saved forward activations through an alias offset, so the fake images are not duplicated. Weight gradients for the D update are deferred as closures over the D-loss slice. This cuts the number of kernel launches and lets each GEMM run with a larger M. In exchange it adds complexity: fast-batch capacity grows to 8 problems, per-image addend and mask handling is added, and several routes are restricted.

```diff
diff --git a/include/jpdse.h b/include/jpdse.h
--- a/include/jpdse.h
+++ b/include/jpdse.h
@@ -85,6 +85,9 @@
 int jpdse_conv_dgrad_fused_lrelu(const jpdse_conv_desc* d, const void* dy, const void* dgrad_pack,
                                  const void* x, float slope, const void* addend, void* dx, void* ws,
                                  size_t ws_bytes, void* stream);
+int jpdse_conv_dgrad_batched(const jpdse_conv_desc* d, const void* dy, const void* dgrad_pack, const void* x, float slope,
+                             const void* addend, int32_t alias, int32_t addend_n, void* dx, void* ws, size_t ws_bytes,
+                             void* stream);
 int32_t jpdse_conv_dgrad_nsum_slots(const jpdse_conv_desc* d);
 int jpdse_conv_dgrad_fused_nsums(const jpdse_conv_desc* d, const void* dy, const void* dgrad_pack, const void* x,
                                  const void* addend, void* dx, const void* norm_x, const float* norm_stats,
@@ -109,6 +112,7 @@
   float slope;
   float eps;
   int32_t has_residual;
+  int32_t alias;
 } jpdse_inorm_desc;
 size_t jpdse_inorm_workspace_size(const jpdse_inorm_desc* d);
 int jpdse_inorm_fwd(const jpdse_inorm_desc* d, const void* x, const void* residual, void* y,
diff --git a/jpd-se_amd/csrc/conv_dispatch_dgrad.h b/jpd-se_amd/csrc/conv_dispatch_dgrad.h
--- a/jpd-se_amd/csrc/conv_dispatch_dgrad.h
+++ b/jpd-se_amd/csrc/conv_dispatch_dgrad.h
@@ -156,6 +156,7 @@
   const jpdse_conv_desc* d; const ConvPlan& p;
   const void* dy; const void* pack; void* dx; void* ws; hipStream_t s;
   const void* mask; const void* addend; float* mom; float mask_slope; const NormSink* sink;
+  int alias, addend_n;
 };
 static void* dgrad_dxp(const DgradCall& c) { return reinterpret_cast<char*>(c.ws) + c.p.dypad_bytes; }
 
@@ -163,6 +164,8 @@
   ConvView v = view_dgrad_phase(c.d, c.p, 0, c.dy, c.pack, c.dx);
   v.mask = reinterpret_cast<const bf16_t*>(c.mask);
   v.addend = reinterpret_cast<const bf16_t*>(c.addend);
+  v.alias = c.mask != nullptr ? c.alias : 0;
+  v.addend_n = c.addend != nullptr ? c.addend_n : 0;
   return v;
 }
 static ConvView ring_view(const DgradCall& c) {
@@ -342,6 +345,7 @@
   t.taps = reinterpret_cast<float*>(c.ws);
   t.DX = reinterpret_cast<bf16_t*>(c.dx);
   t.addend = reinterpret_cast<const bf16_t*>(c.addend);
+  t.addend_n = c.addend_n;
   t.N = c.d->N; t.H = c.d->H; t.W = c.d->W; t.Cs = c.p.Cs; t.OH = c.p.OH; t.OW = c.p.OW;
   t.py = (f.Uh - 1) - f.i0h;
   t.px = (f.Uw - 1) - f.i0w;
@@ -373,9 +377,21 @@
     rc = check_launch("reflect_fold_kernel");
   }
   if (rc == JPDSE_OK && (c.mask != nullptr || c.addend != nullptr) && !in_epilogue) {
-    hipLaunchKernelGGL((relu_mask_kernel<T>), dim3(ew_blocks(total_vec)), dim3(256), 0, c.s, reinterpret_cast<T*>(c.dx),
-                       reinterpret_cast<const T*>(c.mask), total_vec, reinterpret_cast<const T*>(c.addend), c.mask_slope);
-    rc = check_launch("relu_mask_kernel");
+    const int cuts[4] = {0, c.addend != nullptr ? c.addend_n : 0, c.mask != nullptr ? c.alias : 0, d->N};
+    const long long img = (long long)d->H * d->W * c.p.Cs, img_vec = total_vec / d->N;
+    for (int n0 = 0; n0 < d->N && rc == JPDSE_OK;) {
+      int n1 = d->N;
+      for (int q = 1; q < 3; ++q) if (cuts[q] > n0 && cuts[q] < n1) n1 = cuts[q];
+      const T* addend = c.addend != nullptr && (c.addend_n == 0 || n0 < c.addend_n) ? reinterpret_cast<const T*>(c.addend) + n0 * img : nullptr;
+      const T* mask = c.mask != nullptr ? reinterpret_cast<const T*>(c.mask) + (n0 >= c.alias ? n0 - c.alias : n0) * img : nullptr;
+      if (addend != nullptr || mask != nullptr) {
+        const long long nvec = (n1 - n0) * img_vec;
+        hipLaunchKernelGGL((relu_mask_kernel<T>), dim3(ew_blocks(nvec)), dim3(256), 0, c.s, reinterpret_cast<T*>(c.dx) + n0 * img, mask, nvec,
+                           addend, c.mask_slope);
+        rc = check_launch("relu_mask_kernel");
+      }
+      n0 = n1;
+    }
   }
   return rc;
 }
@@ -394,10 +410,31 @@
     if (!refl) {
       g.mask = reinterpret_cast<const bf16_t*>(c.mask);
       g.addend = reinterpret_cast<const bf16_t*>(c.addend);
+      g.alias = c.mask != nullptr ? c.alias : 0;
+      g.addend_n = c.addend != nullptr ? c.addend_n : 0;
     }
     g.mask_slope = c.mask_slope;
     g.splits = nlive == 1 ? splitk_for(g.M, p.Cs, f.Uh * f.Uw * p.Ks / 64) : 1;
     g.partial = splitk_slabs(p, c.ws);
+    if ((g.alias != 0 || g.addend_n != 0) && g.splits <= 1) {
+      const int cuts[2] = {g.addend_n, g.alias};
+      const long long x_img = (long long)g.IH * g.IW * g.Cs;
+      for (int n0 = 0; n0 < d->N;) {
+        int n1 = d->N;
+        for (int q = 0; q < 2; ++q) if (cuts[q] > n0 && cuts[q] < n1) n1 = cuts[q];
+        if (batch.n >= kFastBatchMax) return set_error(JPDSE_EINVAL, "conv_dgrad_batched: more than %d problems in one launch", kFastBatchMax);
+        FastArgs r = g;
+        r.alias = r.addend_n = 0;
+        r.X = g.X + n0 * x_img;
+        r.Y = g.Y + n0 * g.out_sn;
+        r.M = (n1 - n0) * g.OH * g.OW;
+        r.addend = g.addend != nullptr && (g.addend_n == 0 || n0 < g.addend_n) ? g.addend + n0 * g.out_sn : nullptr;
+        r.mask = g.mask != nullptr ? g.mask + (long long)(n0 >= g.alias ? n0 - g.alias : n0) * g.out_sn : nullptr;
+        batch.p[batch.n++] = r;
+        n0 = n1;
+      }
+      continue;
+    }
     batch.p[batch.n++] = g;
   }
   if (int rc = launch_fast_batch(batch, c.s)) return rc;
@@ -441,12 +478,15 @@
 template <typename T>
 static int conv_dgrad_t(const jpdse_conv_desc* d, const ConvPlan& p, const void* dy, const void* pack, void* dx,
                         void* ws, hipStream_t s, const void* mask = nullptr, const void* addend = nullptr, float* mom = nullptr,
-                        float mask_slope = 0.f, const NormSink* sink = nullptr) {
+                        float mask_slope = 0.f, const NormSink* sink = nullptr, int alias = 0, int addend_n = 0) {
   const bool lrelu = mask != nullptr && mask_slope != 0.f;
   if (sink != nullptr && (dgrad_nsum_slots(d, p) == 0 || lrelu))
     return set_error(JPDSE_EINVAL, "conv_dgrad: this layer's data-gradient kernel writes no norm-backward sums (jpdse_conv_dgrad_nsum_slots == 0)");
-  const DgradCall c = {d, p, dy, pack, dx, ws, s, mask, addend, mom, mask_slope, sink};
+  const DgradCall c = {d, p, dy, pack, dx, ws, s, mask, addend, mom, mask_slope, sink, alias, addend_n};
   const DgradRoute route = select_dgrad(d, p, {mask != nullptr, addend != nullptr, lrelu, mom != nullptr, sink != nullptr});
+  if ((alias != 0 || addend_n != 0) && route != DgradRoute::fast && route != DgradRoute::taps4 && route != DgradRoute::thin1 &&
+      route != DgradRoute::generic)
+    return set_error(JPDSE_EINVAL, "conv_dgrad_batched: this layer's data-gradient kernel does not take a batched call");
   if constexpr (sizeof(T) == 2) {
     switch (route) {
       case DgradRoute::rows: return launch_rows(to_rows(dgrad_view(c)), 1, s);
diff --git a/jpd-se_amd/csrc/conv_gemm.hip b/jpd-se_amd/csrc/conv_gemm.hip
--- a/jpd-se_amd/csrc/conv_gemm.hip
+++ b/jpd-se_amd/csrc/conv_gemm.hip
@@ -519,6 +519,24 @@
              : conv_dgrad_t<float>(d, p, dy, dgrad_pack, dx, ws, as_stream(stream), x, addend, nullptr, slope);
 }
 
+int jpdse_conv_dgrad_batched(const jpdse_conv_desc* d, const void* dy, const void* dgrad_pack, const void* x, float slope,
+                             const void* addend, int32_t alias, int32_t addend_n, void* dx, void* ws, size_t ws_bytes, void* stream) {
+  ConvPlan p;
+  if (int rc = conv_enter("conv_dgrad_batched", d, dy && dgrad_pack && dx, ws, ws_bytes, &p, [=](const ConvPlan&) {
+        JPDSE_REQUIRE(slope >= 0.f && slope < 1.f, "conv_dgrad_batched: slope %g outside [0, 1)", (double)slope);
+        JPDSE_REQUIRE(alias >= 0 && 2 * (long long)alias <= d->N && addend_n >= 0 && addend_n <= d->N,
+                      "conv_dgrad_batched: alias %d (at most N / 2) / addend_n %d outside the batch of %d", alias, addend_n, d->N);
+        JPDSE_REQUIRE(x == nullptr || addend == nullptr || alias == 0 || addend_n == alias,
+                      "conv_dgrad_batched: addend_n %d differs from alias %d", addend_n, alias);
+        return (int)JPDSE_OK;
+      })) return rc;
+  if (x == nullptr) alias = 0;
+  if (addend == nullptr || addend_n == d->N) addend_n = 0;
+  return d->dtype == JPDSE_BF16
+             ? conv_dgrad_t<bf16_t>(d, p, dy, dgrad_pack, dx, ws, as_stream(stream), x, addend, nullptr, slope, nullptr, alias, addend_n)
+             : conv_dgrad_t<float>(d, p, dy, dgrad_pack, dx, ws, as_stream(stream), x, addend, nullptr, slope, nullptr, alias, addend_n);
+}
+
 int32_t jpdse_conv_dgrad_nsum_slots(const jpdse_conv_desc* d) {
   if (validate(d)) return 0;
   ConvPlan p;
diff --git a/jpd-se_amd/csrc/conv_launch.h b/jpd-se_amd/csrc/conv_launch.h
--- a/jpd-se_amd/csrc/conv_launch.h
+++ b/jpd-se_amd/csrc/conv_launch.h
@@ -52,6 +52,7 @@
   long long out_sn, out_sh, out_sw, out_base;
   float slope;
   const bf16_t* mask; float mask_slope; const bf16_t* addend;
+  int alias, addend_n;
   float* mom;
   const bf16_t* frame;
 };
@@ -118,6 +119,7 @@
   f.M = v.N * v.OH * v.OW; f.Cs = v.Cin_s;
   f.R = v.R; f.S = v.S; f.sy = f.sx = v.stride; f.reflect = v.reflect;
   f.mask_slope = v.mask_slope;
+  f.alias = v.alias; f.addend_n = v.addend_n;
   return f;
 }
 
@@ -221,7 +223,7 @@
     b.p[i].xcd_map = 0;
     total += ((a.M + BM - 1) / BM) * ((a.Ks + BN - 1) / BN) * (a.splits > 1 ? a.splits : 1);
   }
-  for (int i = b.n; i < 5; ++i) b.first_tile[i] = total;
+  for (int i = b.n; i <= kFastBatchMax; ++i) b.first_tile[i] = total;
   const long long kdim = (long long)b.p[0].R * b.p[0].S * b.p[0].Cs;
   const int pslot = b.n == 1 ? prof_begin(s, b.p[0].Ks, kdim) : -1;
   hipLaunchKernelGGL((gemm_fast_kernel<WM, WN, TM, TN, STAGES>), dim3(total), dim3(64 * WM * WN), lds, s, b);
@@ -567,6 +569,7 @@
   a.slope = v.slope;
   a.addend = v.addend;
   a.mask = v.mask;
+  a.alias = v.alias; a.addend_n = v.addend_n;
   a.prog[0].B[0] = v.B;
   a.prog[0].ktot[0] = v.ktot;
   a.prog[0].out_base[0] = v.out_base;
diff --git a/jpd-se_amd/csrc/gemm_fast.h b/jpd-se_amd/csrc/gemm_fast.h
--- a/jpd-se_amd/csrc/gemm_fast.h
+++ b/jpd-se_amd/csrc/gemm_fast.h
@@ -32,11 +32,13 @@
   int no_finish;
   long long x_extent;
   int xcd_map;
+  int alias, addend_n;
 };
 
+constexpr int kFastBatchMax = 8;
 struct FastBatch {
-  FastArgs p[4];
-  int first_tile[5];
+  FastArgs p[kFastBatchMax];
+  int first_tile[kFastBatchMax + 1];
   int n;
   int small_m;
 };
@@ -132,7 +134,7 @@
 __global__ __launch_bounds__(64 * WM * WN) void gemm_fast_kernel(const FastBatch batch) {
   int q = 0;
 #pragma unroll
-  for (int i = 1; i < 4; ++i)
+  for (int i = 1; i < kFastBatchMax; ++i)
     if (i < batch.n && (int)blockIdx.x >= batch.first_tile[i]) q = i;
   const FastArgs& a = batch.p[q];
   const int block_id = (int)blockIdx.x - batch.first_tile[q];
@@ -432,7 +434,7 @@
     const float bv = (a.bias != nullptr && live) ? a.bias[col] : 0.f;
     o[e] = live ? apply_act(acc[e] + bv, a.act, a.slope) : 0.f;
   }
-  if (a.addend != nullptr) {
+  if (a.addend != nullptr && (a.addend_n == 0 || n < a.addend_n)) {
     float ad[8];
     Vec16<bf16_t>::load(a.addend + off + c0, ad);
 #pragma unroll
@@ -440,7 +442,7 @@
   }
   if (a.mask != nullptr) {
     float mk[8];
-    Vec16<bf16_t>::load(a.mask + off + c0, mk);
+    Vec16<bf16_t>::load(a.mask + (off - (n >= a.alias ? (long long)a.alias * a.out_sn : 0)) + c0, mk);
 #pragma unroll
     for (int e = 0; e < 8; ++e) o[e] = mk[e] > 0.f ? o[e] : (a.mask_slope == 0.f ? 0.f : bf16_round(o[e]) * a.mask_slope);
   }
diff --git a/jpd-se_amd/csrc/gemm_taps.h b/jpd-se_amd/csrc/gemm_taps.h
--- a/jpd-se_amd/csrc/gemm_taps.h
+++ b/jpd-se_amd/csrc/gemm_taps.h
@@ -34,6 +34,7 @@
   float* partial;
   const bf16_t* V;
   int nblk0;
+  int alias, addend_n;
   TapsProg prog[2];
 };
 
@@ -271,13 +272,15 @@
   constexpr int PITCH = BN * 2 + 64;
   static_assert(TH * TW * PITCH <= 2 * HALO + 3 * B_STAGE, "epilogue tile fits the pipeline LDS");
   constexpr int VPR = BN / 8;
+  const bf16_t* const addend = (a.addend_n == 0 || n < a.addend_n) ? a.addend : nullptr;
+  const bf16_t* const mask = a.mask != nullptr ? a.mask - (n >= a.alias ? (long long)a.alias * a.out_sn : 0) : nullptr;
 #pragma unroll
   for (int q = 0; q < NSETS; ++q) {
     __syncthreads();
     acc_tile_to_lds<2, TN>(smem, PITCH, WROWS == 1 ? wm * 64 : wm * 64, wn * TN * 32, n0, lane, acc[q], a.bias, a.Kout, a.act, a.slope);
     __syncthreads();
     const long long blk_base = pr.out_base[q] + n * a.out_sn + (long long)oh0 * a.out_sh + (long long)ow0 * a.out_sw;
-    if (a.addend != nullptr || a.mask != nullptr) {
+    if (addend != nullptr || mask != nullptr) {
       constexpr int NV = TH * TW * VPR / 512;
       static_assert(TH * TW * VPR % 512 == 0, "every thread owns the same number of output vectors");
       u32x4 addv[NV], mskv[NV];
@@ -288,8 +291,8 @@
         const int r = row / TW, c = row - r * TW;
         const long long off = blk_base + (long long)r * a.out_sh + (long long)c * a.out_sw + n0 + v * 8;
         const bool on = n0 + v * 8 < a.Ks;
-        if (on && a.addend != nullptr) addv[it] = *reinterpret_cast<const u32x4*>(a.addend + off);
-        if (on && a.mask != nullptr) mskv[it] = *reinterpret_cast<const u32x4*>(a.mask + off);
+        if (on && addend != nullptr) addv[it] = *reinterpret_cast<const u32x4*>(addend + off);
+        if (on && mask != nullptr) mskv[it] = *reinterpret_cast<const u32x4*>(mask + off);
       }
 #pragma unroll
       for (int it = 0; it < NV; ++it) {
@@ -299,8 +302,8 @@
         const int r = row / TW, c = row - r * TW;
         const long long off = blk_base + (long long)r * a.out_sh + (long long)c * a.out_sw + n0 + v * 8;
         u32x4 val = *reinterpret_cast<const u32x4*>(smem + row * PITCH + v * 16);
-        if (a.addend != nullptr) val = add_bf16x8(val, addv[it]);
-        if (a.mask != nullptr) val = lrelu_mask8(val, mskv[it], a.mask_slope);
+        if (addend != nullptr) val = add_bf16x8(val, addv[it]);
+        if (mask != nullptr) val = lrelu_mask8(val, mskv[it], a.mask_slope);
         *reinterpret_cast<u32x4*>(a.Y + off) = val;
       }
       continue;
diff --git a/jpd-se_amd/csrc/norm.hip b/jpd-se_amd/csrc/norm.hip
--- a/jpd-se_amd/csrc/norm.hip
+++ b/jpd-se_amd/csrc/norm.hip
@@ -7,11 +7,12 @@
   int TX, TY;
   int tx_shift;
   int splits, pix_per_split;
+  int alias;
 };
 
 static MomentGeom moment_geom(int N, int HW, int Cs, int VE) {
   MomentGeom g;
-  g.N = N; g.HW = HW; g.Cs = Cs; g.cv = Cs / VE;
+  g.N = N; g.HW = HW; g.Cs = Cs; g.cv = Cs / VE; g.alias = 0;
   int tx = 1;
   while (tx < g.cv && tx < 256) tx <<= 1;
   g.TX = tx; g.TY = 256 / tx;
@@ -118,8 +119,10 @@
     } else {
       BwdMoments<T> f{x, dy, stats, act, slope};
       float mean[VE], rstd[VE];
+      const int nx = n >= g.alias ? n - g.alias : n;
+      const long long xbase = (long long)nx * g.HW * g.Cs + c0;
       {
-        const float* st = stats + ((long long)n * g.Cs + c0) * 2;
+        const float* st = stats + ((long long)nx * g.Cs + c0) * 2;
 #pragma unroll
         for (int e = 0; e < VE; ++e) { mean[e] = st[2 * e]; rstd[e] = st[2 * e + 1]; }
       }
@@ -128,16 +131,16 @@
         float v[JPDSE_NORM_ILP][VE], gr[JPDSE_NORM_ILP][VE];
 #pragma unroll
         for (int u = 0; u < JPDSE_NORM_ILP; ++u) {
-          const long long off = base + (long long)(p + u * g.TY) * g.Cs;
-          Vec16<T>::load(x + off, v[u]);
-          Vec16<T>::load(dy + off, gr[u]);
+          const long long po = (long long)(p + u * g.TY) * g.Cs;
+          Vec16<T>::load(x + xbase + po, v[u]);
+          Vec16<T>::load(dy + base + po, gr[u]);
         }
 #pragma unroll
         for (int u = 0; u < JPDSE_NORM_ILP; ++u) f.acc2(v[u], gr[u], mean, rstd, s1, s2);
       }
       for (; p < p1; p += g.TY) {
         float v[VE], gr[VE];
-        Vec16<T>::load(x + base + (long long)p * g.Cs, v);
+        Vec16<T>::load(x + xbase + (long long)p * g.Cs, v);
         Vec16<T>::load(dy + base + (long long)p * g.Cs, gr);
         f.acc2(v, gr, mean, rstd, s1, s2);
       }
@@ -295,27 +298,27 @@
   if (col >= g.cv) return;
   const int c0 = col * VE;
   float mean[VE], rstd[VE], s1[VE], s2[VE];
-  const long long sidx = ((long long)n * g.Cs + c0) * 2;
+  const int nx = n >= g.alias ? n - g.alias : n;
+  const long long sidx = ((long long)n * g.Cs + c0) * 2, xidx = ((long long)nx * g.Cs + c0) * 2;
 #pragma unroll
   for (int e = 0; e < VE; ++e) {
-    mean[e] = stats[sidx + 2 * e];
-    rstd[e] = stats[sidx + 2 * e + 1];
+    mean[e] = stats[xidx + 2 * e];
+    rstd[e] = stats[xidx + 2 * e + 1];
     s1[e] = sums[sidx + 2 * e];
     s2[e] = sums[sidx + 2 * e + 1];
   }
   const int p0 = split * g.pix_per_split;
   int p1 = p0 + g.pix_per_split;
   p1 = p1 < g.HW ? p1 : g.HW;
-  const long long base = (long long)n * g.HW * g.Cs + c0;
+  const long long base = (long long)n * g.HW * g.Cs + c0, xbase = (long long)nx * g.HW * g.Cs + c0;
   for (int p = p0 + ty; p < p1; p += JPDSE_NORM_ILP * g.TY) {
     float v[JPDSE_NORM_ILP][VE], gr[JPDSE_NORM_ILP][VE];
 #pragma unroll
     for (int u = 0; u < JPDSE_NORM_ILP; ++u) {
       const int pu = p + u * g.TY;
       if (pu < p1) {
-        const long long off = base + (long long)pu * g.Cs;
-        JPDSE_LOAD_LAST(T, x + off, v[u]);
-        JPDSE_LOAD_LAST(T, dy + off, gr[u]);
+        JPDSE_LOAD_LAST(T, x + xbase + (long long)pu * g.Cs, v[u]);
+        JPDSE_LOAD_LAST(T, dy + base + (long long)pu * g.Cs, gr[u]);
       }
     }
 #pragma unroll
@@ -350,11 +353,12 @@
   int TX, TY, tx_shift;
   int col_blocks, splits, span;
   int nv;
+  int alias;
 };
 
 static FusedGeom fused_geom(int N, int HW, int Cs, int VE, int P) {
   FusedGeom g;
-  g.N = N; g.HW = HW; g.Cs = Cs; g.cv = Cs / VE;
+  g.N = N; g.HW = HW; g.Cs = Cs; g.cv = Cs / VE; g.alias = 0;
   int tx = 1;
   while (tx < g.cv && tx < 16) tx <<= 1;
   g.TX = tx; g.TY = 256 / tx;
@@ -540,14 +544,15 @@
   const int col = cb * g.TX + tx;
   const bool on = col < g.cv;
   const int c0 = (on ? col : 0) * VE;
-  const long long base = (long long)n * g.HW * g.Cs + c0;
+  const int nx = n >= g.alias ? n - g.alias : n;
+  const long long base = (long long)n * g.HW * g.Cs + c0, xbase = (long long)nx * g.HW * g.Cs + c0;
   const int p0 = split * g.span + ty;
   u32x4 xv[P], gv[P];
 #pragma unroll
   for (int i = 0; i < P; ++i) {
     const int p = p0 + i * g.TY;
     if (on && p < g.HW) {
-      xv[i] = *reinterpret_cast<const u32x4*>(x + base + (long long)p * g.Cs);
+      xv[i] = *reinterpret_cast<const u32x4*>(x + xbase + (long long)p * g.Cs);
       gv[i] = *reinterpret_cast<const u32x4*>(dy + base + (long long)p * g.Cs);
     }
   }
@@ -555,7 +560,7 @@
 #pragma unroll
   for (int e = 0; e < 8; ++e) { s1[e] = 0.f; s2[e] = 0.f; }
   {
-    const float* st = stats + ((long long)n * g.Cs + c0) * 2;
+    const float* st = stats + ((long long)nx * g.Cs + c0) * 2;
 #pragma unroll
     for (int e = 0; e < VE; ++e) { mean[e] = st[2 * e]; rstd[e] = st[2 * e + 1]; }
   }
@@ -700,10 +705,13 @@
   void* out;
   float* stats;
   void* stream;
+  int alias;
 };
 
 static MomentGeom moment_geom(const jpdse_inorm_desc* d) {
-  return moment_geom(d->N, d->H * d->W, cpad(d->C), vec_elems(d->dtype));
+  MomentGeom g = moment_geom(d->N - d->alias, d->H * d->W, cpad(d->C), vec_elems(d->dtype));
+  g.N = d->N;
+  return g;
 }
 static dim3 moment_grid(const MomentGeom& g) { return dim3(g.N * g.splits * ((g.cv + g.TX - 1) / g.TX)); }
 static dim3 lanes8_grid(const jpdse_inorm_desc* d) { return dim3((d->N * cpad(d->C) * 8 + 255) / 256); }
@@ -719,10 +727,11 @@
 }
 
 template <typename T, int PHASE, bool BWD>
-static int launch_reg(const NormCall& c, const FusedGeom& fg, float* part, int mslots = 0) {
+static int launch_reg(const NormCall& c, FusedGeom fg, float* part, int mslots = 0) {
   static const char* const what[2][3] = {{"inorm rows fwd", "inorm apply-from-rows fwd", "inorm apply-from-slots fwd"},
                                          {"inorm rows bwd", "inorm apply-from-rows bwd", "inorm apply-from-slots bwd"}};
   const jpdse_inorm_desc* d = c.d;
+  fg.alias = BWD ? c.alias : 0;
   if constexpr (BWD)
     return launch256(what[1][PHASE - 1], inorm_reg_bwd_kernel<T, 8, PHASE>, fused_grid(fg), c.stream, cptr<T>(c.x), cptr<T>(c.in2),
                      mptr<T>(c.out), c.stats, part, (unsigned*)nullptr, d->act, d->slope, fg, mslots);
@@ -747,7 +756,8 @@
   return launch_reg<T, 3, BWD>(c, fg, const_cast<float*>(slots_in), slots);
 }
 
-template <typename T, bool BWD> static int launch_apply(const NormCall& c, const MomentGeom& g, const float* sums = nullptr) {
+template <typename T, bool BWD> static int launch_apply(const NormCall& c, MomentGeom g, const float* sums = nullptr) {
+  g.alias = BWD ? c.alias : 0;
   if constexpr (BWD)
     return launch256("inorm apply bwd", inorm_apply_bwd_kernel<T>, moment_grid(g), c.stream, cptr<T>(c.x), cptr<T>(c.in2),
                      mptr<T>(c.out), c.stats, sums, c.d->act, c.d->slope, g);
@@ -773,7 +783,8 @@
 template <typename T> static int inorm_bwd_t(const NormCall& c, void* ws) {
   if (const int r = try_reg<T, true>(c, ws); r != kNoRegForm) return r;
   const jpdse_inorm_desc* d = c.d;
-  const MomentGeom g = moment_geom(d);
+  MomentGeom g = moment_geom(d);
+  g.alias = c.alias;
   float* partial = mptr<float>(ws);
   float* sums = reinterpret_cast<float*>(mptr<char>(ws) + ws_sums_offset(d, g));
   if (int rc = launch256("inorm moment bwd", moment_kernel<T, true>, moment_grid(g), c.stream, cptr<T>(c.x), cptr<T>(c.in2),
@@ -811,6 +822,7 @@
   JPDSE_REQUIRE(d->N > 0 && d->H > 0 && d->W > 0 && d->C > 0, "inorm: non-positive shape");
   JPDSE_REQUIRE(d->act == JPDSE_ACT_NONE || d->act == JPDSE_ACT_RELU || d->act == JPDSE_ACT_LRELU,
                 "inorm: unsupported activation %d", d->act);
+  JPDSE_REQUIRE(d->alias >= 0 && 2 * (long long)d->alias <= d->N, "inorm: alias %d outside [0, N / 2 = %d / 2]", d->alias, d->N);
   return JPDSE_OK;
 }
 
@@ -851,6 +863,7 @@
 int jpdse_inorm_fwd(const jpdse_inorm_desc* d, const void* x, const void* residual, void* y, float* stats, void* ws,
                     size_t ws_bytes, void* stream) {
   if (int rc = inorm_enter("inorm_fwd", d, x && y && stats, "null pointer", &residual, WS_FULL, ws, ws_bytes)) return rc;
+  JPDSE_REQUIRE(d->alias == 0, "inorm_fwd: the descriptor's alias is for jpdse_inorm_bwd alone");
   const NormCall c = {d, x, residual, y, stats, stream};
   return timed_by_dtype(d, stream, JPDSE_HBM_INORM_FWD, d->has_residual ? 4.0 : 3.0,
                         [&](auto tag) { return inorm_fwd_t<decltype(tag)>(c, ws); });
@@ -859,7 +872,7 @@
 int jpdse_inorm_bwd(const jpdse_inorm_desc* d, const void* x, const float* stats, const void* dy, void* dx, void* ws,
                     size_t ws_bytes, void* stream) {
   if (int rc = inorm_enter("inorm_bwd", d, x && stats && dy && dx, "null pointer", nullptr, WS_FULL, ws, ws_bytes)) return rc;
-  const NormCall c = {d, x, dy, dx, const_cast<float*>(stats), stream};
+  const NormCall c = {d, x, dy, dx, const_cast<float*>(stats), stream, d->alias};
   return timed_by_dtype(d, stream, JPDSE_HBM_INORM_BWD, 5.0, [&](auto tag) { return inorm_bwd_t<decltype(tag)>(c, ws); });
 }
 
@@ -868,6 +881,7 @@
   if (int rc = inorm_enter("inorm_bwd_from_sums", d, x && stats && dy && dx && sums && slots > 0, "null pointer / no slots",
                            nullptr, WS_SUMS, ws, ws_bytes))
     return rc;
+  JPDSE_REQUIRE(d->alias == 0, "inorm_bwd_from_sums: the descriptor's alias is for jpdse_inorm_bwd alone");
   const NormCall c = {d, x, dy, dx, const_cast<float*>(stats), stream};
   return timed_by_dtype(d, stream, JPDSE_HBM_INORM_BWD, 3.0,
                         [&](auto tag) { return inorm_bwd_from_sums_t<decltype(tag)>(c, sums, slots, ws); });
@@ -878,6 +892,7 @@
   if (int rc = inorm_enter("inorm_fwd_from_moments", d, x && y && stats && moments && slots > 0, "null pointer / no slots",
                            &residual, WS_NONE, nullptr, 0))
     return rc;
+  JPDSE_REQUIRE(d->alias == 0, "inorm_fwd_from_moments: the descriptor's alias is for jpdse_inorm_bwd alone");
   const NormCall c = {d, x, residual, y, stats, stream};
   return timed_by_dtype(d, stream, JPDSE_HBM_INORM_FWD, d->has_residual ? 3.0 : 2.0,
                         [&](auto tag) { return inorm_from_moments_t<decltype(tag)>(c, moments, slots); });
diff --git a/jpd-se_amd/csrc/thin_out1.h b/jpd-se_amd/csrc/thin_out1.h
--- a/jpd-se_amd/csrc/thin_out1.h
+++ b/jpd-se_amd/csrc/thin_out1.h
@@ -14,6 +14,7 @@
   long long b_stride;
   int Lk;
   int nseg, segw;
+  int addend_n;
 };
 
 typedef float f32x2 __attribute__((ext_vector_type(2)));
@@ -70,7 +71,7 @@
 #pragma unroll
       for (int u = 0; u < R; ++u) win[v][u] = dyw[pl][u][v - 1];
     bf16_t* __restrict__ out = a.DX + (((long long)n * a.H + ih) * a.W + w0) * a.Cs + cg * 8;
-    const bf16_t* __restrict__ add = a.addend != nullptr ? a.addend + (out - a.DX) : nullptr;
+    const bf16_t* __restrict__ add = (a.addend != nullptr && (a.addend_n == 0 || n < a.addend_n)) ? a.addend + (out - a.DX) : nullptr;
     for (int i0 = 0; i0 < wn; i0 += 4) {
       u32x4 adv[4];
       if (add != nullptr) {
diff --git a/jpd-se_amd/ctu/models/pix2pixHD_model.py b/jpd-se_amd/ctu/models/pix2pixHD_model.py
--- a/jpd-se_amd/ctu/models/pix2pixHD_model.py
+++ b/jpd-se_amd/ctu/models/pix2pixHD_model.py
@@ -383,12 +383,37 @@
       self._one = torch.ones(1, dtype=torch.float32, device=dev)
     return self._one
 
-  def backward_G(self, state, w_gan, w_feat, w_vgg, w_dist):
+  d_backward_batched = True
+
+  def backward_G(self, state, w_gan, w_feat, w_vgg, w_dist, w_d=0.0):
     opt, B = self.opt, state['B']
     one = self._ones(state['fake'].t.device)
     fake, real = state['fake'], state['real']
     d_fake = None
-    if (w_gan != 0.0 or w_feat != 0.0) and state['pred'] is not None:
+    if (self.d_backward_batched and not self.grad_buckets and w_gan != 0.0 and w_d != 0.0 and state['pred'] is not None
+        and self.netD.can_bwd_batched()
+        and all(p.requires_grad for p in self.netD.parameters())):
+      dfeats, dpred = [], []
+      for i in range(opt.num_D):
+        feats = state['pred'][i]
+        row = []
+        for j, f in enumerate(feats[:-1]):
+          if w_feat == 0.0:
+            row.append(None)
+          elif state.get('d_feat') is not None and state['d_feat'][i][j] is not None:
+            row.append(state['d_feat'][i][j])
+          else:
+            row.append(ops.l1_bwd(f.batch_slice(0, B), f.batch_slice(B, 2 * B), one, w_feat / opt.num_D))
+        dfeats.append(row)
+        p = feats[-1]
+        dp = Act.empty(3 * B, p.H, p.W, p.C, p.dtype, p.t.device)
+        ops.mse_const_bwd(p.batch_slice(0, B), 1.0, one, w_gan, out=dp.batch_slice(0, B))
+        ops.mse_const_bwd(p.batch_slice(0, B), 0.0, one, w_d, out=dp.batch_slice(B, 2 * B))
+        ops.mse_const_bwd(p.batch_slice(B, 2 * B), 1.0, one, w_d, out=dp.batch_slice(2 * B, 3 * B))
+        dpred.append(dp)
+      d_fake, state['d_wgrads'] = self.netD.bwd_batched(state['d_ctx'], dfeats, dpred, B,
+                                                        (self.label_nc, self.label_nc + fake.C))
+    elif (w_gan != 0.0 or w_feat != 0.0) and state['pred'] is not None:
       dres = []
       for i in range(opt.num_D):
         row = []
@@ -449,6 +474,10 @@
   def backward_D(self, state, w_d):
     if w_d == 0.0 or state['pred'] is None:
       return False
+    if state.get('d_wgrads') is not None:
+      for call in state.pop('d_wgrads'):
+        call()
+      return True
     opt, B = self.opt, state['B']
     one = self._ones(state['fake'].t.device)
     dres = []
@@ -481,11 +510,12 @@
         ev.record()
         marks[name] = ev
 
-    did_G = self.backward_G(state, w_gan, w_feat, w_vgg, w_dist)
+    w_d = 0.0 if opt.no_d_gan_loss else 0.5
+    did_G = self.backward_G(state, w_gan, w_feat, w_vgg, w_dist, w_d)
     mark('g_bwd_end')
     if did_G and bg is not None:
       bg.launch_all()
-    did_D = self.backward_D(state, 0.0 if opt.no_d_gan_loss else 0.5)
+    did_D = self.backward_D(state, w_d)
     mark('d_bwd_end')
     if did_G:
       if bg is not None:
diff --git a/jpd-se_amd/ctu/models/pix2pixHD_networks/networks.py b/jpd-se_amd/ctu/models/pix2pixHD_networks/networks.py
--- a/jpd-se_amd/ctu/models/pix2pixHD_networks/networks.py
+++ b/jpd-se_amd/ctu/models/pix2pixHD_networks/networks.py
@@ -413,6 +413,18 @@
     return d
 
 
+  def bwd_batched(self, ctxs, dfeats, dpred, B, later, dx_channels):
+    assert self.fuse_lrelu0
+    d = dpred
+    for j in range(len(self._stages) - 1, 0, -1):
+      lrelu0 = dict(relu_input=True, input_slope=self._stages[0].slope) if j == 1 else {}
+      d = self._stages[j].bwd_batched(ctxs[j], d, B, later, addend=dfeats[j - 1], **lrelu0)
+    st0 = self._stages[0]
+    if st0.weight.requires_grad:
+      later.append(lambda: st0.bwd(ctxs[0], d.batch_slice(B, d.N), need_dx=False, need_dw=True, dy_is_dz=True))
+    return st0.bwd_input_slice(ctxs[0].slice(0, B), d.batch_slice(0, B), dx_channels[0], dx_channels[1], dy_is_dz=True)
+
+
 class MultiscaleDiscriminator(nn.Module):
 
   def __init__(self, input_nc, ndf=64, n_layers=3, norm_layer=None, use_sigmoid=False, num_D=3,
@@ -451,6 +463,19 @@
           d = ops.add_(d, ops.avgpool3s2_bwd(dx, H, W))
         dx = d
     return dx
+
+  def bwd_batched(self, ctxs, dfeats, dpred, B, dx_channels):
+    dx, later = None, []
+    for i in range(self.num_D - 1, -1, -1):
+      c, H, W = ctxs[i]
+      d = self._scales[self.num_D - 1 - i].bwd_batched(c, dfeats[i], dpred[i], B, later, dx_channels)
+      if dx is not None:
+        d = ops.add_(d, ops.avgpool3s2_bwd(dx, H, W))
+      dx = d
+    return dx, later
+
+  def can_bwd_batched(self):
+    return all(s.fuse_lrelu0 for s in self._scales)
 
   def forward(self, input, keep_input=False):
     if keep_input:
diff --git a/jpd-se_amd/jpdse_hip/__init__.py b/jpd-se_amd/jpdse_hip/__init__.py
--- a/jpd-se_amd/jpdse_hip/__init__.py
+++ b/jpd-se_amd/jpdse_hip/__init__.py
@@ -24,7 +24,8 @@
 class InormDesc(ctypes.Structure):
   _fields_ = [('dtype', ctypes.c_int32), ('N', ctypes.c_int32), ('H', ctypes.c_int32),
               ('W', ctypes.c_int32), ('C', ctypes.c_int32), ('act', ctypes.c_int32),
-              ('slope', ctypes.c_float), ('eps', ctypes.c_float), ('has_residual', ctypes.c_int32)]
+              ('slope', ctypes.c_float), ('eps', ctypes.c_float), ('has_residual', ctypes.c_int32),
+              ('alias', ctypes.c_int32)]
 
 
 class PackEntry(ctypes.Structure):
@@ -234,6 +235,7 @@
     'jpdse_conv_dgrad_relu': (_I32, [_CD, _P, _P, _P, _P, _P, _SZ, _P]),
     'jpdse_conv_dgrad_fused': (_I32, [_CD, _P, _P, _P, _P, _P, _P, _SZ, _P]),
     'jpdse_conv_dgrad_fused_lrelu': (_I32, [_CD, _P, _P, _P, _F, _P, _P, _P, _SZ, _P]),
+    'jpdse_conv_dgrad_batched': (_I32, [_CD, _P, _P, _P, _F, _P, _I32, _I32, _P, _P, _SZ, _P]),
     'jpdse_conv_dgrad_nsum_slots': (_I32, [_CD]),
     'jpdse_conv_dgrad_fused_nsums': (_I32, [_CD, _P, _P, _P, _P, _P, _P, _P, _I32, _F, _P, _P, _SZ, _P]),
     'jpdse_conv_wgrad': (_I32, [_CD, _P, _P, _P, _P, _SZ, _P]),
diff --git a/jpd-se_amd/jpdse_hip/layers.py b/jpd-se_amd/jpdse_hip/layers.py
--- a/jpd-se_amd/jpdse_hip/layers.py
+++ b/jpd-se_amd/jpdse_hip/layers.py
@@ -181,6 +181,16 @@
                                     relu_input=x if relu_input else None, addend=addend)
     return ops.conv_dgrad(d, dz, dgrad_pack, relu_input=x if relu_input else None, addend=addend, mask_slope=input_slope)
 
+  def bwd_batched(self, ctx, dy, B, later, relu_input=False, addend=None, input_slope=0.0):
+    assert not self.transposed and self.act == ACT_NONE
+    _, dgrad_pack = self.packs()
+    x, _ = ctx.items
+    assert dy.N == x.N + B
+    if self.weight.requires_grad:
+      later.append(lambda: self.bwd(ctx, dy.batch_slice(B, dy.N), need_dx=False, need_dw=True))
+    return ops.conv_dgrad_batched(self._desc(dy.N, x.H, x.W), dy, dgrad_pack, B, relu_input=x if relu_input else None,
+                                  addend=addend, mask_slope=input_slope)
+
   def bwd_input_slice(self, ctx, dy, c0, c1, dy_is_dz=False):
     assert not self.transposed
     x, y = ctx.items
@@ -399,6 +409,12 @@
     dh = self.norm.bwd(c2, dy)
     return self.conv.bwd(c1, dh, need_dx, need_dw, addend=addend, **conv_kw)
 
+  def bwd_batched(self, ctx, dy, B, later, addend=None, **conv_kw):
+    c1, c2 = ctx.items
+    x, stats = c2.items
+    dh = ops.inorm_bwd_aliased(x, stats, dy, B, self.norm.act, self.norm.slope, self.norm.eps)
+    return self.conv.bwd_batched(c1, dh, B, later, addend=addend, **conv_kw)
+
   def dy_sink(self, ctx):
     return self.norm.sink(ctx.items[1])
 
diff --git a/jpd-se_amd/jpdse_hip/ops.py b/jpd-se_amd/jpdse_hip/ops.py
--- a/jpd-se_amd/jpdse_hip/ops.py
+++ b/jpd-se_amd/jpdse_hip/ops.py
@@ -166,6 +166,17 @@
   return dx
 
 
+def conv_dgrad_batched(d, dy, dgrad_pack, alias, relu_input=None, addend=None, mask_slope=0.0):
+  dx = Act.empty(d.N, d.H, d.W, d.C, d.dtype, dy.t.device)
+  assert relu_input is None or relu_input.N == d.N - alias, (relu_input.N, d.N, alias)
+  ws, n = _conv_ws(d, dy.t.device)
+  check(lib().jpdse_conv_dgrad_batched(ctypes.byref(d), _p(dy.t), _p(dgrad_pack), _p(relu_input.t if relu_input is not None else None),
+                                       float(mask_slope), _p(addend.t if addend is not None else None), int(alias),
+                                       int(addend.N) if addend is not None else 0, _p(dx.t), _p(ws), ws.numel(), _stream()),
+        'conv_dgrad_batched')
+  return dx
+
+
 def conv_dgrad_nsum_slots(d):
   return int(lib().jpdse_conv_dgrad_nsum_slots(ctypes.byref(d)))
 
@@ -240,6 +251,17 @@
     return dx
   check(lib().jpdse_inorm_bwd(ctypes.byref(d), _p(x.t), _p(stats), _p(dy.t), _p(dx.t), _p(ws), ws.numel(), _stream()),
         'inorm_bwd')
+  return dx
+
+
+def inorm_bwd_aliased(x, stats, dy, alias, act, slope=0.2, eps=1e-5):
+  assert x.N == dy.N - alias and tuple(x.t.shape[1:]) == tuple(dy.t.shape[1:]), (tuple(x.t.shape), tuple(dy.t.shape), alias)
+  d = InormDesc(x.dtype, dy.N, x.H, x.W, x.C, act, slope, eps, 0, int(alias))
+  dx = dy.empty_like()
+  n = lib().jpdse_inorm_workspace_size(ctypes.byref(d))
+  ws = workspace(n, x.t.device)
+  check(lib().jpdse_inorm_bwd(ctypes.byref(d), _p(x.t), _p(stats), _p(dy.t), _p(dx.t), _p(ws), ws.numel(), _stream()),
+        'inorm_bwd (aliased)')
   return dx
 
 
```

Measured after the change: 159.7 images/sec (median of 6 runs). +1.8%, better.
